# BallisticLA/RandLAPACK

Hardware: AMD Instinct MI355X
Metric: GFLOP/s (sketch+factor) for RSVD rank-256 on m x n dense fp64 (higher is better)
Workload: dtype f64; 1 GPU; RSVD 200000x20000 fp64 rank 256, one QB block, p=0, CholQRQ (BASELINE configs[1]); m=200000, n=20000, k=256, parallelism=row-block x1, collectives=none, ranks_seen=1, comm_kind=none, qb_return=3, k_out=256

## Files before the change

### include/RandLAPACK_amd/rl_blaspp.hh

```
#pragma once
#include <cstdint>
#include <cmath>
#include <stdexcept>
#include <string>
#include <vector>
#include "../rlhip.h"

namespace blas {

enum class Layout : char { ColMajor = 'C', RowMajor = 'R' };
enum class Op : char { NoTrans = 'N', Trans = 'T', ConjTrans = 'C' };
enum class Side : char { Left = 'L', Right = 'R' };
enum class Diag : char { NonUnit = 'N', Unit = 'U' };
enum class Uplo : char { Upper = 'U', Lower = 'L', General = 'G' };

inline char to_char(Op v) { return (char)v; }
inline char to_char(Side v) { return (char)v; }
inline char to_char(Diag v) { return (char)v; }
inline char to_char(Uplo v) { return (char)v; }
inline char to_char(Layout v) { return (char)v; }

class Error : public std::runtime_error {
public:
    explicit Error(std::string const& m) : std::runtime_error(m) {}
};

inline void check(int rc, const char* what) {
    if (rc < 0) throw Error(std::string(what) + " failed with code " + std::to_string(rc));
}

class Queue {
    rlhip_ctx* ctx_ = nullptr;
    bool owned_ = false;
public:
    explicit Queue(int device = 0) {
        check(rlhip_create(&ctx_, device, nullptr, 1), "rlhip_create");
        owned_ = true;
    }
    explicit Queue(rlhip_ctx* ctx) : ctx_(ctx), owned_(false) {}
    struct Side {};
    Queue(Queue& parent, Side) {
        check(rlhip_create_side(parent.ctx_, &ctx_), "rlhip_create_side");
        owned_ = true;
    }
    struct CachedSide {};
    Queue(Queue& parent, CachedSide) {
        check(rlhip_side_of(parent.ctx_, &ctx_), "rlhip_side_of");
        owned_ = false;
    }
    void wait_for(Queue& other) { check(rlhip_order_after(ctx_, other.ctx_), "rlhip_order_after"); }
    void set_qrcp_cols(int cols) { check(rlhip_set_qrcp_cols(ctx_, cols), "rlhip_set_qrcp_cols"); }
    Queue(Queue const&) = delete;
    Queue& operator=(Queue const&) = delete;
    ~Queue() { if (owned_ && ctx_) rlhip_destroy(ctx_); }
    void sync() { check(rlhip_sync(ctx_), "rlhip_sync"); }

    int world() const { return local_only ? 1 : rlhip_comm_size(ctx_); }
    int rank() const { return local_only ? 0 : rlhip_comm_rank(ctx_); }
    int local_only = 0;
    struct NormRequest { const void* ptr = nullptr; int64_t rows = 0, cols = 0, ld = 0; bool done = false; double value = 0; bool defer = false, pending = false; };
    NormRequest norm_req;
    double collect_norm(bool over_ranks) {
        if (norm_req.pending) { check(rlhip_norma_collect_f64(ctx_, over_ranks ? 1 : 0, &norm_req.value), "norma_collect"); norm_req.pending = false; }
        else if (over_ranks && world() > 1) { double ssq = norm_req.value * norm_req.value; allreduce_sum_host(&ssq, 1); norm_req.value = std::sqrt(ssq); }
        return norm_req.value;
    }
    bool rows_sharded = false;
    bool reduce_over_rows() const { return rows_sharded && world() > 1; }
    void allreduce_sum(double* buf, int64_t count) { check(rlhip_allreduce_sum_f64(ctx_, buf, count), "allreduce"); }
    void allreduce_sum(float* buf, int64_t count) { check(rlhip_allreduce_sum_f32(ctx_, buf, count), "allreduce"); }
    void allreduce_sum_host(double* x, int64_t n) { check(rlhip_allreduce_sum_host_f64(ctx_, x, n), "allreduce_host"); }
    void shard_extent(int64_t m_local, int64_t& m_global, int64_t& row0) {
        const int w = world(), r = rank();
        if (w <= 1) { m_global = m_local; row0 = 0; return; }
        std::vector<double> len((size_t)w, 0.0);
        len[(size_t)r] = (double)m_local;
        allreduce_sum_host(len.data(), w);
        m_global = 0; row0 = 0;
        for (int i = 0; i < w; ++i) { if (i < r) row0 += (int64_t)len[(size_t)i]; m_global += (int64_t)len[(size_t)i]; }
    }
    void* stream() const { return rlhip_stream(ctx_); }
    rlhip_ctx* ctx() const { return ctx_; }
};

inline Queue& default_queue() {
    static Queue q0(0);
    return q0;
}

template <typename T>
T* device_malloc(int64_t n, Queue& q = blas::default_queue()) {
    void* p = nullptr;
    check(rlhip_malloc(q.ctx(), &p, (size_t)(n > 0 ? n : 1) * sizeof(T)), "device_malloc");
    return (T*)p;
}
inline void device_free(void* p, Queue& q = blas::default_queue()) { check(rlhip_free(q.ctx(), p), "device_free"); }
template <typename T>
void device_memset(T* p, int byte, int64_t n, Queue& q = blas::default_queue()) { check(rlhip_memset(q.ctx(), p, byte, (size_t)n * sizeof(T)), "memset"); }
template <typename T>
void device_copy_vector(int64_t n, T const* src, T* dst, Queue& q = blas::default_queue()) {
    check(rlhip_memcpy_d2d(q.ctx(), dst, src, (size_t)n * sizeof(T)), "device_copy_vector");
}
template <typename T>
void copy_to_host(int64_t n, T const* dev, T* host, Queue& q = blas::default_queue()) { check(rlhip_memcpy_d2h(q.ctx(), host, dev, (size_t)n * sizeof(T)), "d2h"); }
template <typename T>
void copy_to_device(int64_t n, T const* host, T* dev, Queue& q = blas::default_queue()) { check(rlhip_memcpy_h2d(q.ctx(), dev, host, (size_t)n * sizeof(T)), "h2d"); }

template <typename T>
void copy(int64_t n, T const* x, int64_t incx, T* y, int64_t incy, Queue& q = default_queue()) {
    if (incx != 1 || incy != 1) throw Error("blas::copy: unit strides only");
    device_copy_vector(n, x, y, q);
}

class RowsSharded {
    Queue& q_;
    bool prev_;
public:
    RowsSharded(Queue& q, bool on) : q_(q), prev_(q.rows_sharded) { q.rows_sharded = on; }
    ~RowsSharded() { q_.rows_sharded = prev_; }
};

class LocalOnly {
    Queue& q_;
public:
    explicit LocalOnly(Queue& q) : q_(q) { ++q.local_only; }
    ~LocalOnly() { --q_.local_only; }
};

class Range {
public:
    explicit Range(const char* name) { rlhip_range_push(name); }
    ~Range() { rlhip_range_pop(); }
    Range(Range const&) = delete;
    Range& operator=(Range const&) = delete;
};

class Phases {
    bool open_ = false;
public:
    void operator()(const char* name) { end(); rlhip_range_push(name); open_ = true; }
    void end() { if (open_) { rlhip_range_pop(); open_ = false; } }
    ~Phases() { end(); }
};

class GiveWay {
    Queue& q_;
    int prev_;
public:
    explicit GiveWay(Queue& q) : q_(q), prev_(rlhip_avoid_persistent(q.ctx(), 1)) {}
    ~GiveWay() { rlhip_avoid_persistent(q_.ctx(), prev_ > 0 ? 1 : 0); }
};

class Scratch {
    Queue& q_;
    size_t mark_;
public:
    explicit Scratch(Queue& q) : q_(q), mark_(rlhip_scratch_mark(q.ctx())) {}
    ~Scratch() { rlhip_scratch_release(q_.ctx(), mark_); }
    template <typename T>
    T* alloc(int64_t n) {
        void* p = nullptr;
        check(rlhip_scratch_alloc(q_.ctx(), &p, (size_t)(n > 0 ? n : 1) * sizeof(T)), "scratch_alloc");
        return (T*)p;
    }
    template <typename T>
    T* try_alloc(int64_t n) {
        void* p = nullptr;
        if (rlhip_scratch_alloc(q_.ctx(), &p, (size_t)(n > 0 ? n : 1) * sizeof(T)) < 0) return nullptr;
        return (T*)p;
    }
};

inline void gemm(Layout, Op ta, Op tb, int64_t m, int64_t n, int64_t k, double alpha, double const* A, int64_t lda,
                 double const* B, int64_t ldb, double beta, double* C, int64_t ldc, Queue& q = blas::default_queue()) {
    auto& nr = q.norm_req;
    if (nr.ptr == (const void*)A && !nr.done && nr.ld == lda &&
        ((ta == Op::NoTrans && nr.rows == m && nr.cols == k) || (ta != Op::NoTrans && nr.rows == k && nr.cols == m))) {
        double nrm = 0;
        check(rlhip_gemm_norma_f64(q.ctx(), (char)ta, (char)tb, m, n, k, alpha, A, lda, B, ldb, beta, C, ldc, nr.defer ? nullptr : &nrm,
                                   nullptr), "gemm_norma");
        nr.done = true;
        nr.pending = nr.defer;
        nr.value = nrm;
        return;
    }
    check(rlhip_gemm_f64(q.ctx(), (char)ta, (char)tb, m, n, k, alpha, A, lda, B, ldb, beta, C, ldc), "gemm");
}
inline void gemm(Layout, Op ta, Op tb, int64_t m, int64_t n, int64_t k, float alpha, float const* A, int64_t lda,
                 float const* B, int64_t ldb, float beta, float* C, int64_t ldc, Queue& q = blas::default_queue()) {
    check(rlhip_gemm_f32(q.ctx(), (char)ta, (char)tb, m, n, k, alpha, A, lda, B, ldb, beta, C, ldc), "gemm");
}
inline void syrk(Layout, Uplo u, Op t, int64_t n, int64_t k, double alpha, double const* A, int64_t lda, double beta,
                 double* C, int64_t ldc, Queue& q = blas::default_queue()) {
    check(rlhip_syrk_f64(q.ctx(), (char)u, (char)t, n, k, alpha, A, lda, beta, C, ldc), "syrk");
}
inline void syrk(Layout, Uplo u, Op t, int64_t n, int64_t k, float alpha, float const* A, int64_t lda, float beta,
                 float* C, int64_t ldc, Queue& q = blas::default_queue()) {
    check(rlhip_syrk_f32(q.ctx(), (char)u, (char)t, n, k, alpha, A, lda, beta, C, ldc), "syrk");
}
inline void trsm(Layout, Side s, Uplo u, Op t, Diag d, int64_t m, int64_t n, double alpha, double const* A, int64_t lda,
                 double* B, int64_t ldb, Queue& q = blas::default_queue()) {
    check(rlhip_trsm_f64(q.ctx(), (char)s, (char)u, (char)t, (char)d, m, n, alpha, A, lda, B, ldb), "trsm");
}
inline void trsm(Layout, Side s, Uplo u, Op t, Diag d, int64_t m, int64_t n, float alpha, float const* A, int64_t lda,
                 float* B, int64_t ldb, Queue& q = blas::default_queue()) {
    check(rlhip_trsm_f32(q.ctx(), (char)s, (char)u, (char)t, (char)d, m, n, alpha, A, lda, B, ldb), "trsm");
}
inline void trsm_gather(Diag d, int64_t m, int64_t n, double alpha, double const* A, int64_t lda, double const* Bsrc, int64_t ldsrc,
                        int64_t const* jpvt, double* B, int64_t ldb, Queue& q = blas::default_queue()) {
    check(rlhip_trsm_gather_f64(q.ctx(), (char)d, m, n, alpha, A, lda, Bsrc, ldsrc, jpvt, B, ldb), "trsm_gather");
}
inline void trsm_gather(Diag d, int64_t m, int64_t n, float alpha, float const* A, int64_t lda, float const* Bsrc, int64_t ldsrc,
                        int64_t const* jpvt, float* B, int64_t ldb, Queue& q = blas::default_queue()) {
    check(rlhip_trsm_gather_f32(q.ctx(), (char)d, m, n, alpha, A, lda, Bsrc, ldsrc, jpvt, B, ldb), "trsm_gather");
}
inline bool trsm_gather_range(Diag d, int64_t m, int64_t nsrc, double alpha, double const* A, int64_t lda, double const* Bsrc, int64_t ldsrc,
                              int64_t const* jpvt, double* B, int64_t ldb, int64_t col0, int64_t col1, Queue& q = blas::default_queue()) {
    const int rc = rlhip_trsm_gather_range_f64(q.ctx(), (char)d, m, nsrc, alpha, A, lda, Bsrc, ldsrc, jpvt, B, ldb, col0, col1);
    if (rc == 1) return false;
    check(rc, "trsm_gather_range");
    return true;
}
inline bool trsm_gather_range(Diag d, int64_t m, int64_t nsrc, float alpha, float const* A, int64_t lda, float const* Bsrc, int64_t ldsrc,
                              int64_t const* jpvt, float* B, int64_t ldb, int64_t col0, int64_t col1, Queue& q = blas::default_queue()) {
    const int rc = rlhip_trsm_gather_range_f32(q.ctx(), (char)d, m, nsrc, alpha, A, lda, Bsrc, ldsrc, jpvt, B, ldb, col0, col1);
    if (rc == 1) return false;
    check(rc, "trsm_gather_range");
    return true;
}
inline void trmm(Layout, Side s, Uplo u, Op t, Diag d, int64_t m, int64_t n, double alpha, double const* A, int64_t lda,
                 double* B, int64_t ldb, Queue& q = blas::default_queue()) {
    check(rlhip_trmm_f64(q.ctx(), (char)s, (char)u, (char)t, (char)d, m, n, alpha, A, lda, B, ldb), "trmm");
}
inline void trmm(Layout, Side s, Uplo u, Op t, Diag d, int64_t m, int64_t n, float alpha, float const* A, int64_t lda,
                 float* B, int64_t ldb, Queue& q = blas::default_queue()) {
    check(rlhip_trmm_f32(q.ctx(), (char)s, (char)u, (char)t, (char)d, m, n, alpha, A, lda, B, ldb), "trmm");
}

}

namespace RandLAPACK {
using blas::Layout;
using blas::Op;
using blas::Side;
using blas::Diag;
using blas::Uplo;
}
```

### include/RandLAPACK_amd/rl_lapackpp.hh

```
#pragma once
#include <cmath>
#include "rl_blaspp.hh"

namespace lapack {

using blas::Queue;
enum class Job : char { NoVec = 'N', Vec = 'V', SomeVec = 'S', AllVec = 'A' };
enum class Norm : char { One = '1', Inf = 'I', Fro = 'F', Max = 'M' };
enum class MatrixType : char { General = 'G', Lower = 'L', Upper = 'U' };
inline char to_char(Job v) { return (char)v; }
inline char to_char(Norm v) { return (char)v; }
inline char to_char(MatrixType v) { return (char)v; }

inline int64_t potrf(blas::Uplo u, int64_t n, double* A, int64_t lda, Queue& q = blas::default_queue()) {
    int rc = rlhip_potrf_f64(q.ctx(), (char)u, n, A, lda); blas::check(rc, "potrf"); return rc;
}
inline int64_t potrf(blas::Uplo u, int64_t n, float* A, int64_t lda, Queue& q = blas::default_queue()) {
    int rc = rlhip_potrf_f32(q.ctx(), (char)u, n, A, lda); blas::check(rc, "potrf"); return rc;
}
inline int cholqrq(int64_t m, int64_t k, double* A, int64_t lda, double* R, bool reduce_gram, int& info, Queue& q = blas::default_queue()) {
    const int rc = rlhip_cholqrq_f64(q.ctx(), m, k, A, lda, R, reduce_gram ? 1 : 0, &info);
    blas::check(rc, "cholqrq");
    return rc;
}
inline int cholqrq(int64_t m, int64_t k, float* A, int64_t lda, float* R, bool reduce_gram, int& info, Queue& q = blas::default_queue()) {
    const int rc = rlhip_cholqrq_f32(q.ctx(), m, k, A, lda, R, reduce_gram ? 1 : 0, &info);
    blas::check(rc, "cholqrq");
    return rc;
}
inline double lange(Norm nt, int64_t m, int64_t n, double const* A, int64_t lda, Queue& q = blas::default_queue()) {
    if (nt != Norm::Fro) throw blas::Error("lange: only Norm::Fro is on the path");
    double r = 0; blas::check(rlhip_lange_fro_f64(q.ctx(), m, n, A, lda, &r), "lange"); return r;
}
inline float lange(Norm nt, int64_t m, int64_t n, float const* A, int64_t lda, Queue& q = blas::default_queue()) {
    if (nt != Norm::Fro) throw blas::Error("lange: only Norm::Fro is on the path");
    float r = 0; blas::check(rlhip_lange_fro_f32(q.ctx(), m, n, A, lda, &r), "lange"); return r;
}
inline void lacpy(MatrixType t, int64_t m, int64_t n, double const* A, int64_t lda, double* B, int64_t ldb, Queue& q = blas::default_queue()) {
    blas::check(rlhip_lacpy_f64(q.ctx(), (char)t, m, n, A, lda, B, ldb), "lacpy");
}
inline void lacpy(MatrixType t, int64_t m, int64_t n, float const* A, int64_t lda, float* B, int64_t ldb, Queue& q = blas::default_queue()) {
    blas::check(rlhip_lacpy_f32(q.ctx(), (char)t, m, n, A, lda, B, ldb), "lacpy");
}
inline void laset(MatrixType t, int64_t m, int64_t n, double offd, double diag, double* A, int64_t lda, Queue& q = blas::default_queue()) {
    blas::check(rlhip_laset_f64(q.ctx(), (char)t, m, n, offd, diag, A, lda), "laset");
}
inline void laset(MatrixType t, int64_t m, int64_t n, float offd, float diag, float* A, int64_t lda, Queue& q = blas::default_queue()) {
    blas::check(rlhip_laset_f32(q.ctx(), (char)t, m, n, offd, diag, A, lda), "laset");
}
inline void add_diag(int64_t n, double alpha, double* A, int64_t lda, Queue& q = blas::default_queue()) {
    blas::check(rlhip_add_diag_f64(q.ctx(), n, alpha, A, lda), "add_diag");
}
inline void add_diag(int64_t n, float alpha, float* A, int64_t lda, Queue& q = blas::default_queue()) {
    blas::check(rlhip_add_diag_f32(q.ctx(), n, alpha, A, lda), "add_diag");
}
inline int64_t geqp3(int64_t m, int64_t n, double* A, int64_t lda, int64_t* jpvt, double* tau, Queue& q = blas::default_queue()) {
    int rc = rlhip_geqp3_f64(q.ctx(), m, n, A, lda, jpvt, tau); blas::check(rc, "geqp3"); return rc;
}
inline int64_t geqp3(int64_t m, int64_t n, float* A, int64_t lda, int64_t* jpvt, float* tau, Queue& q = blas::default_queue()) {
    int rc = rlhip_geqp3_f32(q.ctx(), m, n, A, lda, jpvt, tau); blas::check(rc, "geqp3"); return rc;
}
inline void get_diag(int64_t n, double const* A, int64_t lda, double* diag_host, Queue& q = blas::default_queue()) {
    blas::check(rlhip_get_diag_f64(q.ctx(), n, A, lda, diag_host), "get_diag");
}
inline void get_diag(int64_t n, float const* A, int64_t lda, float* diag_host, Queue& q = blas::default_queue()) {
    blas::check(rlhip_get_diag_f32(q.ctx(), n, A, lda, diag_host), "get_diag");
}
inline bool any_abs_gt(int64_t n, double const* x, double thr, Queue& q = blas::default_queue()) { int a = 0; blas::check(rlhip_any_abs_gt_f64(q.ctx(), n, x, thr, &a), "any_abs_gt"); return a != 0; }
inline bool any_abs_gt(int64_t n, float const* x, float thr, Queue& q = blas::default_queue()) { int a = 0; blas::check(rlhip_any_abs_gt_f32(q.ctx(), n, x, thr, &a), "any_abs_gt"); return a != 0; }
inline void orhr_col(int64_t m, int64_t n, int64_t nb, double* A, int64_t lda, double* T, int64_t ldt, double* D, Queue& q = blas::default_queue()) { blas::check(rlhip_orhr_col_f64(q.ctx(), m, n, nb, A, lda, T, ldt, D), "orhr_col"); }
inline void orhr_col(int64_t m, int64_t n, int64_t nb, float* A, int64_t lda, float* T, int64_t ldt, float* D, Queue& q = blas::default_queue()) { blas::check(rlhip_orhr_col_f32(q.ctx(), m, n, nb, A, lda, T, ldt, D), "orhr_col"); }
inline void gemqrt(blas::Side s, blas::Op t, int64_t m, int64_t n, int64_t k, int64_t nb, double const* V, int64_t ldv, double const* T, int64_t ldt, double* C, int64_t ldc, Queue& q = blas::default_queue()) { blas::check(rlhip_gemqrt_f64(q.ctx(), (char)s, (char)t, m, n, k, nb, V, ldv, T, ldt, C, ldc), "gemqrt"); }
inline void gemqrt(blas::Side s, blas::Op t, int64_t m, int64_t n, int64_t k, int64_t nb, float const* V, int64_t ldv, float const* T, int64_t ldt, float* C, int64_t ldc, Queue& q = blas::default_queue()) { blas::check(rlhip_gemqrt_f32(q.ctx(), (char)s, (char)t, m, n, k, nb, V, ldv, T, ldt, C, ldc), "gemqrt"); }
inline void gemqrt_head(int64_t m, int64_t n, int64_t k, double const* V, int64_t ldv, double const* T, int64_t ldt, double* C, int64_t ldc, double* W2, Queue& q = blas::default_queue()) { blas::check(rlhip_gemqrt_head_f64(q.ctx(), m, n, k, V, ldv, T, ldt, C, ldc, W2), "gemqrt_head"); }
inline void gemqrt_head(int64_t m, int64_t n, int64_t k, float const* V, int64_t ldv, float const* T, int64_t ldt, float* C, int64_t ldc, float* W2, Queue& q = blas::default_queue()) { blas::check(rlhip_gemqrt_head_f32(q.ctx(), m, n, k, V, ldv, T, ldt, C, ldc, W2), "gemqrt_head"); }
inline void gemqrt_tail(int64_t m, int64_t n, int64_t k, double const* V, int64_t ldv, double const* W2, double* C, int64_t ldc, Queue& q = blas::default_queue()) { blas::check(rlhip_gemqrt_tail_f64(q.ctx(), m, n, k, V, ldv, W2, C, ldc), "gemqrt_tail"); }
inline void gemqrt_tail(int64_t m, int64_t n, int64_t k, float const* V, int64_t ldv, float const* W2, float* C, int64_t ldc, Queue& q = blas::default_queue()) { blas::check(rlhip_gemqrt_tail_f32(q.ctx(), m, n, k, V, ldv, W2, C, ldc), "gemqrt_tail"); }
inline void larft(int64_t m, int64_t k, double const* V, int64_t ldv, double const* tau, double* T, int64_t ldt, Queue& q = blas::default_queue()) { blas::check(rlhip_larft_f64(q.ctx(), m, k, V, ldv, tau, T, ldt), "larft"); }
inline void larft(int64_t m, int64_t k, float const* V, int64_t ldv, float const* tau, float* T, int64_t ldt, Queue& q = blas::default_queue()) { blas::check(rlhip_larft_f32(q.ctx(), m, k, V, ldv, tau, T, ldt), "larft"); }
inline void row_sign(int64_t n, double* R, int64_t ldr, double const* D, Queue& q = blas::default_queue()) { blas::check(rlhip_row_sign_f64(q.ctx(), n, R, ldr, D), "row_sign"); }
inline void row_sign(int64_t n, float* R, int64_t ldr, float const* D, Queue& q = blas::default_queue()) { blas::check(rlhip_row_sign_f32(q.ctx(), n, R, ldr, D), "row_sign"); }
inline void tau_from_t(int64_t k, int64_t nb, double const* T, int64_t ldt, double* tau, Queue& q = blas::default_queue()) { blas::check(rlhip_tau_from_t_f64(q.ctx(), k, nb, T, ldt, tau), "tau_from_t"); }
inline void tau_from_t(int64_t k, int64_t nb, float const* T, int64_t ldt, float* tau, Queue& q = blas::default_queue()) { blas::check(rlhip_tau_from_t_f32(q.ctx(), k, nb, T, ldt, tau), "tau_from_t"); }
inline int64_t geqrf(int64_t m, int64_t n, double* A, int64_t lda, double* tau, Queue& q = blas::default_queue()) { int rc = rlhip_geqrf_f64(q.ctx(), m, n, A, lda, tau); blas::check(rc, "geqrf"); return rc; }
inline int64_t geqrf(int64_t m, int64_t n, float* A, int64_t lda, float* tau, Queue& q = blas::default_queue()) { int rc = rlhip_geqrf_f32(q.ctx(), m, n, A, lda, tau); blas::check(rc, "geqrf"); return rc; }
inline bool geqrf_q(int64_t m, int64_t n, double* A, int64_t lda, double* R, int64_t ldr, Queue& q = blas::default_queue()) { int rc = rlhip_geqrf_q_f64(q.ctx(), m, n, A, lda, R, ldr); blas::check(rc, "geqrf_q"); return rc == 0; }
inline bool geqrf_q(int64_t m, int64_t n, float* A, int64_t lda, float* R, int64_t ldr, Queue& q = blas::default_queue()) { int rc = rlhip_geqrf_q_f32(q.ctx(), m, n, A, lda, R, ldr); blas::check(rc, "geqrf_q"); return rc == 0; }
inline void ungqr(int64_t m, int64_t n, int64_t k, double* A, int64_t lda, double const* tau, Queue& q = blas::default_queue()) { blas::check(rlhip_ungqr_f64(q.ctx(), m, n, k, A, lda, tau), "ungqr"); }
inline void ungqr(int64_t m, int64_t n, int64_t k, float* A, int64_t lda, float const* tau, Queue& q = blas::default_queue()) { blas::check(rlhip_ungqr_f32(q.ctx(), m, n, k, A, lda, tau), "ungqr"); }
inline int64_t getrf(int64_t m, int64_t n, double* A, int64_t lda, int64_t* ipiv, Queue& q = blas::default_queue()) { int rc = rlhip_getrf_f64(q.ctx(), m, n, A, lda, ipiv); blas::check(rc, "getrf"); return rc; }
inline int64_t getrf(int64_t m, int64_t n, float* A, int64_t lda, int64_t* ipiv, Queue& q = blas::default_queue()) { int rc = rlhip_getrf_f32(q.ctx(), m, n, A, lda, ipiv); blas::check(rc, "getrf"); return rc; }
inline int64_t getrf_pivots(int64_t m, int64_t n, double* A, int64_t lda, int64_t* ipiv, Queue& q = blas::default_queue()) { int rc = rlhip_getrf_piv_f64(q.ctx(), m, n, A, lda, ipiv); blas::check(rc, "getrf_piv"); return rc; }
inline int64_t getrf_pivots(int64_t m, int64_t n, float* A, int64_t lda, int64_t* ipiv, Queue& q = blas::default_queue()) { int rc = rlhip_getrf_piv_f32(q.ctx(), m, n, A, lda, ipiv); blas::check(rc, "getrf_piv"); return rc; }
inline void laswp(int64_t n, double* A, int64_t lda, int64_t k1, int64_t k2, int64_t const* ipiv, int64_t incx, Queue& q = blas::default_queue()) {
    if (incx != 1) throw blas::Error("laswp: only incx = 1 is on the path");
    blas::check(rlhip_laswp_f64(q.ctx(), n, A, lda, k1, k2, ipiv), "laswp");
}
inline void laswp(int64_t n, float* A, int64_t lda, int64_t k1, int64_t k2, int64_t const* ipiv, int64_t incx, Queue& q = blas::default_queue()) {
    if (incx != 1) throw blas::Error("laswp: only incx = 1 is on the path");
    blas::check(rlhip_laswp_f32(q.ctx(), n, A, lda, k1, k2, ipiv), "laswp");
}
template <typename T>
inline void geqrt(int64_t m, int64_t n, int64_t nb, T* A, int64_t lda, T* Tm, int64_t ldt, T* tau_scratch, Queue& q = blas::default_queue()) {
    geqrf(m, n, A, lda, tau_scratch, q);
    for (int64_t i = 0; i < n; i += nb) {
        const int64_t ib = std::min(nb, n - i);
        larft(m - i, ib, A + i + i * lda, lda, tau_scratch + i, Tm + i * ldt, ldt, q);
    }
}
template <typename T>
inline void ormqr(blas::Side s, blas::Op t, int64_t m, int64_t n, int64_t k, T const* V, int64_t ldv, T const* tau, T* C, int64_t ldc, T* T_scratch, Queue& q = blas::default_queue()) {
    if (k == 0 || n == 0) return;
    larft(m, k, V, ldv, tau, T_scratch, k, q);
    gemqrt(s, t, m, n, k, k, V, ldv, T_scratch, k, C, ldc, q);
}
template <typename T>
inline T lansy(Norm nt, blas::Uplo u, int64_t n, T const* A, int64_t lda, Queue& q = blas::default_queue()) {
    if (nt != Norm::Fro) throw blas::Error("lansy: only Norm::Fro is on the path");
    if (n <= 0) return (T)0;
    blas::Scratch ws(q);
    T* W = ws.alloc<T>(n * n);
    laset(MatrixType::General, n, n, (T)0, (T)0, W, n, q);
    lacpy(u == blas::Uplo::Upper ? MatrixType::Upper : MatrixType::Lower, n, n, A, lda, W, n, q);
    const T tri = lange(Norm::Fro, n, n, W, n, q);
    std::vector<T> dg((size_t)n);
    get_diag(n, A, lda, dg.data(), q);
    double dd = 0;
    for (T v : dg) dd += (double)v * (double)v;
    const double s2 = 2.0 * (double)tri * (double)tri - dd;
    return (T)std::sqrt(s2 > 0 ? s2 : 0.0);
}
inline void qrp_partial(int64_t m, int64_t n, int64_t steps, double* A, int64_t lda, int64_t* jpvt, double* tau, Queue& q = blas::default_queue()) { blas::check(rlhip_qrp_partial_f64(q.ctx(), m, n, steps, A, lda, jpvt, tau), "qrp_partial"); }
inline void qrp_partial(int64_t m, int64_t n, int64_t steps, float* A, int64_t lda, int64_t* jpvt, float* tau, Queue& q = blas::default_queue()) { blas::check(rlhip_qrp_partial_f32(q.ctx(), m, n, steps, A, lda, jpvt, tau), "qrp_partial"); }
inline void geqp3_steps(int64_t m, int64_t n, int64_t steps, double* A, int64_t lda, int64_t* jpvt, double* tau, Queue& q = blas::default_queue()) { blas::check(rlhip_geqp3_steps_f64(q.ctx(), m, n, steps, A, lda, jpvt, tau), "geqp3_steps"); }
inline void geqp3_steps(int64_t m, int64_t n, int64_t steps, float* A, int64_t lda, int64_t* jpvt, float* tau, Queue& q = blas::default_queue()) { blas::check(rlhip_geqp3_steps_f32(q.ctx(), m, n, steps, A, lda, jpvt, tau), "geqp3_steps"); }
inline void vrows_explicit(int64_t br, int64_t toff, int64_t tcnt, double const* Vtop, int64_t ldv, double* out, int64_t ldo, Queue& q = blas::default_queue()) { blas::check(rlhip_vrows_explicit_f64(q.ctx(), br, toff, tcnt, Vtop, ldv, out, ldo), "vrows_explicit"); }
inline void vrows_explicit(int64_t br, int64_t toff, int64_t tcnt, float const* Vtop, int64_t ldv, float* out, int64_t ldo, Queue& q = blas::default_queue()) { blas::check(rlhip_vrows_explicit_f32(q.ctx(), br, toff, tcnt, Vtop, ldv, out, ldo), "vrows_explicit"); }
inline void luqrcp_piv(int64_t sd, int64_t cols, int64_t const* ipiv, int64_t* J, Queue& q = blas::default_queue()) { blas::check(rlhip_luqrcp_piv(q.ctx(), sd, cols, ipiv, J), "luqrcp_piv"); }
inline int64_t gesdd(Job job, int64_t m, int64_t n, double* A, int64_t lda, double* S, double* U, int64_t ldu,
                     double* VT, int64_t ldvt, Queue& q = blas::default_queue()) {
    if (job != Job::SomeVec) throw blas::Error("gesdd: only Job::SomeVec is on the path");
    int rc = rlhip_gesdd_f64(q.ctx(), m, n, A, lda, S, U, ldu, VT, ldvt, nullptr); blas::check(rc, "gesdd"); return rc;
}
inline int64_t gesdd(Job job, int64_t m, int64_t n, float* A, int64_t lda, float* S, float* U, int64_t ldu,
                     float* VT, int64_t ldvt, Queue& q = blas::default_queue()) {
    if (job != Job::SomeVec) throw blas::Error("gesdd: only Job::SomeVec is on the path");
    int rc = rlhip_gesdd_f32(q.ctx(), m, n, A, lda, S, U, ldu, VT, ldvt, nullptr); blas::check(rc, "gesdd"); return rc;
}
inline int64_t gesvdj(int64_t m, int64_t n, double* A, int64_t lda, double* S, double* VT, int64_t ldvt, Queue& q = blas::default_queue()) {
    int rc = rlhip_gesvdj_f64(q.ctx(), m, n, A, lda, S, VT, ldvt, nullptr); blas::check(rc, "gesvdj"); return rc;
}
inline int64_t gesvdj(int64_t m, int64_t n, float* A, int64_t lda, float* S, float* VT, int64_t ldvt, Queue& q = blas::default_queue()) {
    int rc = rlhip_gesvdj_f32(q.ctx(), m, n, A, lda, S, VT, ldvt, nullptr); blas::check(rc, "gesvdj"); return rc;
}

}

namespace RandLAPACK {
using lapack::Job;
using lapack::MatrixType;
using lapack::Norm;
}
```

### include/RandLAPACK_amd/rl_qb.hh

```
#pragma once
#include <algorithm>
#include <cmath>
#include <limits>
#include "rl_rf.hh"

namespace RandLAPACK {

template <typename T, typename RNG>
class QBalg {
public:
    virtual ~QBalg() {}
    virtual int call(int64_t m, int64_t n, T* A, int64_t& k, int64_t b_sz, T tol, T*& Q, T*& BT,
                     RandBLAS::RNGState<RNG>& state) = 0;
};

template <typename T, typename RNG>
class QB : public QBalg<T, RNG> {
public:
    QB(RangeFinder<T, RNG>& rf_obj, Stabilization<T>& orth_obj, bool verb, bool orth) : QB(blas::default_queue(), rf_obj, orth_obj, verb, orth) {}
    QB(blas::Queue& queue, RangeFinder<T, RNG>& rf_obj, Stabilization<T>& orth_obj, bool verb, bool orth)
        : q(queue), rf(rf_obj), orth(orth_obj) {
        verbose = verb;
        orth_check = orth;
    }

    int call(int64_t m, int64_t n, T* A, int64_t& k, int64_t b_sz, T tol, T*& Q, T*& BT,
             RandBLAS::RNGState<RNG>& state) override {
        int64_t curr_sz = 0, next_sz = 0;
        tol = std::max(tol, 100 * std::numeric_limits<T>::epsilon());
        T norm_B = 0, prev_err = 0, approx_err = 0;
        if (Q) blas::device_free(Q, q);
        if (BT) blas::device_free(BT, q);
        const int64_t k_in = k;
        Q = blas::device_malloc<T>(m * k_in, q);
        BT = blas::device_malloc<T>(n * k_in, q);
        blas::Scratch ws(q);
        T* QtQi = ws.alloc<T>(k_in * std::max<int64_t>(1, std::min(b_sz, k_in)));
        const bool single_block = (b_sz >= k_in);
        T* A_cpy = A;
        T* A_own = nullptr;
        T norm_A = 0;
        bool have_norm = false;
        if (!single_block) {
            A_own = blas::device_malloc<T>(m * n, q);
            lapack::lacpy(MatrixType::General, m, n, A, m, A_own, m, q);
            A_cpy = A_own;
        }
        if constexpr (sizeof(T) == 8) {
            q.norm_req = blas::Queue::NormRequest();
            q.norm_req.ptr = A_cpy; q.norm_req.rows = m; q.norm_req.cols = n; q.norm_req.ld = m;
            q.norm_req.defer = true;
        }
        blas::RowsSharded sh(q, true);
        auto done = [&](int code) {
            q.norm_req = blas::Queue::NormRequest();
            if (A_own) blas::device_free(A_own, q);
            const int64_t kept = std::max<int64_t>(std::min(k, k_in), 0);
            if (kept < k_in) {
                blas::device_memset(Q + m * kept, 0, m * (k_in - kept), q);
                blas::device_memset(BT + n * kept, 0, n * (k_in - kept), q);
            }
            return code;
        };

        while (curr_sz < k) {
            b_sz = std::min(b_sz, k - curr_sz);
            next_sz = curr_sz + b_sz;
            T* Q_i = Q + m * curr_sz;
            T* BT_i = BT + n * curr_sz;
            if (rf.call(m, n, A_cpy, b_sz, Q_i, state)) { k = curr_sz; q.norm_req = blas::Queue::NormRequest(); return done(6); }
            const bool norm_rides = !have_norm && q.norm_req.done;
            if (!have_norm && !norm_rides) norm_A = lapack::lange(Norm::Fro, m, n, A_cpy, m, q);
            if (orth_check && util::orthogonality_check(m, b_sz, Q_i, verbose, q)) { k = curr_sz; return done(4); }
            if (curr_sz != 0) {
                blas::gemm(Layout::ColMajor, Op::Trans, Op::NoTrans, curr_sz, b_sz, m, T(1), Q, m, Q_i, m, T(0), QtQi, next_sz, q);
                if (q.world() > 1) q.allreduce_sum(QtQi, next_sz * b_sz);
                blas::gemm(Layout::ColMajor, Op::NoTrans, Op::NoTrans, m, b_sz, curr_sz, T(-1), Q, m, QtQi, next_sz, T(1), Q_i, m, q);
                orth.call(m, b_sz, Q_i);
            }
            blas::gemm(Layout::ColMajor, Op::Trans, Op::NoTrans, n, b_sz, m, T(1), A_cpy, m, Q_i, m, T(0), BT_i, n, q);
            if (q.world() > 1) q.allreduce_sum(BT_i, n * b_sz);
            T norm_B_i = lapack::lange(Norm::Fro, n, b_sz, BT_i, n, q);
            if (!have_norm) {
                if (norm_rides) norm_A = (T)q.collect_norm(true);
                else if (q.world() > 1) {
                    double ssq = (double)norm_A * (double)norm_A;
                    q.allreduce_sum_host(&ssq, 1);
                    norm_A = (T)std::sqrt(ssq);
                }
                q.norm_req = blas::Queue::NormRequest();
                have_norm = true;
            }
            norm_B = std::hypot(norm_B, norm_B_i);
            prev_err = approx_err;
            approx_err = std::sqrt(std::abs(norm_A - norm_B)) * (std::sqrt(norm_A + norm_B) / norm_A);
            if ((curr_sz > 0) && (approx_err > prev_err)) { k = curr_sz; return done(2); }
            if (orth_check && util::orthogonality_check(m, next_sz, Q, verbose, q)) { k = curr_sz; return done(5); }
            curr_sz += b_sz;
            if (approx_err < tol) { k = curr_sz; return done(0); }
            if (curr_sz < k)
                blas::gemm(Layout::ColMajor, Op::NoTrans, Op::Trans, m, n, b_sz, T(-1), Q_i, m, BT_i, n, T(1), A_cpy, m, q);
        }
        return done(3);
    }

    blas::Queue& q;
    RangeFinder<T, RNG>& rf;
    Stabilization<T>& orth;
    bool verbose;
    bool orth_check;
};

}
```

### include/RandLAPACK_amd/rl_rsvd.hh

```
#pragma once
#include "rl_exceptions.hh"
#include "rl_qb.hh"

namespace RandLAPACK {

template <typename T, typename RNG>
class RSVDalg {
public:
    virtual ~RSVDalg() {}
    virtual int call(int64_t m, int64_t n, T* A, int64_t& k, T tol, T*& U, T*& S, T*& V,
                     RandBLAS::RNGState<RNG>& state) = 0;
};

template <typename T, typename RNG>
class RSVD : public RSVDalg<T, RNG> {
public:
    RSVD(QBalg<T, RNG>& qb_obj, int64_t b_sz) : RSVD(blas::default_queue(), qb_obj, b_sz) {}
    RSVD(blas::Queue& queue, QBalg<T, RNG>& qb_obj, int64_t b_sz) : q(queue), QB_Obj(qb_obj) { block_sz = b_sz; }

    int call(int64_t m, int64_t n, T* A, int64_t& k, T tol, T*& U, T*& S, T*& V,
             RandBLAS::RNGState<RNG>& state) override {
        randlapack_require(m >= 0) << "m=" << m << " must be >= 0";
        randlapack_require(n >= 0) << "n=" << n << " must be >= 0";
        randlapack_require(k > 0) << "target rank k=" << k << " must be > 0";
        randlapack_require(tol >= (T)0) << "tol=" << tol << " must be >= 0";
        randlapack_require(!(A == nullptr && m > 0 && n > 0))
            << "A buffer is null but m=" << m << " and n=" << n << " imply a nonempty matrix";

        T* Q = nullptr;
        T* BT = nullptr;
        qb_return = QB_Obj.call(m, n, A, k, block_sz, tol, Q, BT, state);

        const int64_t kk = std::max<int64_t>(k, 1);
        U = blas::device_malloc<T>(m * kk, q);
        S = blas::device_malloc<T>(kk, q);
        V = blas::device_malloc<T>(n * kk, q);
        if (k > 0) {
            blas::Scratch ws(q);
            T* UT_buf = ws.alloc<T>(k * k);
            svd_info = lapack::gesdd(Job::SomeVec, n, k, BT, n, S, V, n, UT_buf, k, q);
            blas::gemm(Layout::ColMajor, Op::NoTrans, Op::Trans, m, k, k, T(1), Q, m, UT_buf, k, T(0), U, m, q);
        }
        blas::device_free(Q, q);
        blas::device_free(BT, q);
        return 0;
    }

    blas::Queue& q;
    QBalg<T, RNG>& QB_Obj;
    int64_t block_sz;
    int qb_return = 0;
    int64_t svd_info = 0;
};

}
```

### include/rlhip.h

```cpp
#ifndef RLHIP_H
#define RLHIP_H
#include <stddef.h>
#include <stdint.h>

#ifdef __cplusplus
extern "C" {
#endif

typedef struct rlhip_ctx rlhip_ctx;

int rlhip_create(rlhip_ctx** ctx, int device, void* hip_stream, int own_stream);
int rlhip_create_side(rlhip_ctx* parent, rlhip_ctx** out);
int rlhip_order_after(rlhip_ctx* waiter, rlhip_ctx* signaler);
int rlhip_destroy(rlhip_ctx* ctx);
enum rlhip_option {
    RLHIP_OPT_CHOLQRQ_ONE_STREAM = 0,
    RLHIP_OPT_GESDD_GRAM = 1,
    RLHIP_OPT_JACOBI_PERSIST = 2,
    RLHIP_OPT_TRSM_XASM = 3,
    RLHIP_OPT_SASO_MODE = 4,
    RLHIP_OPT_HQRRP_TALL_PANEL = 5,
    RLHIP_OPT_DRV_BQRRP_LOOKAHEAD_MIN_ELEMS = 6,
    RLHIP_OPT_DRV_BQRRP_CHOLQR_FALLBACK = 7,
    RLHIP_OPT_DRV_CQRRPT_FOLD_PIVOTING = 8,
    RLHIP_OPT_DRV_CQRRPT_SPLIT_QRCP = 9,
    RLHIP_OPT_DRV_SPARSE_SKETCH_DENSIFY = 10,
    RLHIP_OPT_JACOBI_CLOCK_HOLDERS = 11,
    RLHIP_OPT_LSQ_NORMAL_FUSED = 12,
    RLHIP_OPT_SPMV_LANES = 13,
    RLHIP_OPT_RBF_FUSED = 14,
    RLHIP_OPT_COUNT = 15
};
int rlhip_set_option(rlhip_ctx* ctx, int option, int64_t value);
int64_t rlhip_get_option(rlhip_ctx* ctx, int option);
int rlhip_sync(rlhip_ctx* ctx);
void* rlhip_stream(rlhip_ctx* ctx);
int rlhip_malloc(rlhip_ctx* ctx, void** dev_ptr, size_t bytes);
int rlhip_free(rlhip_ctx* ctx, void* dev_ptr);
int rlhip_trim(rlhip_ctx* ctx);
int rlhip_malloc_host(rlhip_ctx* ctx, void** host_ptr, size_t bytes);
int rlhip_free_host(rlhip_ctx* ctx, void* host_ptr);
int rlhip_memcpy_h2d(rlhip_ctx* ctx, void* dst_dev, const void* src_host, size_t bytes);
int rlhip_memcpy_d2h(rlhip_ctx* ctx, void* dst_host, const void* src_dev, size_t bytes);
int rlhip_memcpy_d2d(rlhip_ctx* ctx, void* dst_dev, const void* src_dev, size_t bytes);
int rlhip_memset(rlhip_ctx* ctx, void* dst_dev, int byte, size_t bytes);
int rlhip_reserve_workspace(rlhip_ctx* ctx, size_t bytes);
size_t rlhip_workspace_highwater(rlhip_ctx* ctx);
const char* rlhip_version(void);

size_t rlhip_scratch_mark(rlhip_ctx* ctx);
int rlhip_scratch_alloc(rlhip_ctx* ctx, void** dev_ptr, size_t bytes);
int rlhip_scratch_release(rlhip_ctx* ctx, size_t mark);

int rlhip_timer_start(rlhip_ctx* ctx);
int rlhip_timer_stop_ms(rlhip_ctx* ctx, float* ms_host);

int rlhip_philox4x32_10(rlhip_ctx* ctx, int64_t nblocks, uint32_t* out_dev, const uint32_t ctr_host[4],
                        const uint32_t key_host[2]);
int rlhip_fill_dense_f64(rlhip_ctx* ctx, int dist, int64_t rows, int64_t cols, double* buf,
                         const uint32_t ctr_host[4], const uint32_t key_host[2], uint32_t next_ctr_host[4]);
int rlhip_fill_dense_f32(rlhip_ctx* ctx, int dist, int64_t rows, int64_t cols, float* buf,
                         const uint32_t ctr_host[4], const uint32_t key_host[2], uint32_t next_ctr_host[4]);
int rlhip_fill_dense_rows_f64(rlhip_ctx* ctx, int dist, int64_t glob_rows, int64_t cols, int64_t row0, int64_t loc_rows,
                              double* buf, int64_t ld, const uint32_t ctr[4], const uint32_t key[2], uint32_t next_ctr[4]);
int rlhip_fill_dense_rows_f32(rlhip_ctx* ctx, int dist, int64_t glob_rows, int64_t cols, int64_t row0, int64_t loc_rows,
                              float* buf, int64_t ld, const uint32_t ctr[4], const uint32_t key[2], uint32_t next_ctr[4]);

int rlhip_gemm_f64(rlhip_ctx* ctx, char transa, char transb, int64_t m, int64_t n, int64_t k, double alpha,
                   const double* A, int64_t lda, const double* B, int64_t ldb, double beta, double* C,
                   int64_t ldc);
int rlhip_gemm_f32(rlhip_ctx* ctx, char transa, char transb, int64_t m, int64_t n, int64_t k, float alpha,
                   const float* A, int64_t lda, const float* B, int64_t ldb, float beta, float* C,
                   int64_t ldc);
int rlhip_gemm_norma_f64(rlhip_ctx* ctx, char transa, char transb, int64_t m, int64_t n, int64_t k, double alpha,
                         const double* A, int64_t lda, const double* B, int64_t ldb, double beta, double* C,
                         int64_t ldc, double* norm_a_host, int* fused_host);
int rlhip_norma_collect_f64(rlhip_ctx* ctx, int over_ranks, double* norm_a_host);
int rlhip_syrk_f64(rlhip_ctx* ctx, char uplo, char trans, int64_t n, int64_t k, double alpha, const double* A,
                   int64_t lda, double beta, double* C, int64_t ldc);
int rlhip_syrk_f32(rlhip_ctx* ctx, char uplo, char trans, int64_t n, int64_t k, float alpha, const float* A,
                   int64_t lda, float beta, float* C, int64_t ldc);
int rlhip_trsm_f64(rlhip_ctx* ctx, char side, char uplo, char trans, char diag, int64_t m, int64_t n,
                   double alpha, const double* A, int64_t lda, double* B, int64_t ldb);
int rlhip_trsm_f32(rlhip_ctx* ctx, char side, char uplo, char trans, char diag, int64_t m, int64_t n,
                   float alpha, const float* A, int64_t lda, float* B, int64_t ldb);
int rlhip_trsm_gather_f64(rlhip_ctx* ctx, char diag, int64_t m, int64_t n, double alpha, const double* A, int64_t lda,
                          const double* Bsrc, int64_t ldsrc, const int64_t* jpvt_dev, double* B, int64_t ldb);
int rlhip_trsm_gather_f32(rlhip_ctx* ctx, char diag, int64_t m, int64_t n, float alpha, const float* A, int64_t lda,
                          const float* Bsrc, int64_t ldsrc, const int64_t* jpvt_dev, float* B, int64_t ldb);
int rlhip_trsm_gather_range_f64(rlhip_ctx* ctx, char diag, int64_t m, int64_t nsrc, double alpha, const double* A, int64_t lda,
                                const double* Bsrc, int64_t ldsrc, const int64_t* jpvt, double* B, int64_t ldb, int64_t col0, int64_t col1);
int rlhip_trsm_gather_range_f32(rlhip_ctx* ctx, char diag, int64_t m, int64_t nsrc, float alpha, const float* A, int64_t lda,
                                const float* Bsrc, int64_t ldsrc, const int64_t* jpvt, float* B, int64_t ldb, int64_t col0, int64_t col1);
int rlhip_trmm_f64(rlhip_ctx* ctx, char side, char uplo, char trans, char diag, int64_t m, int64_t n,
                   double alpha, const double* A, int64_t lda, double* B, int64_t ldb);
int rlhip_trmm_f32(rlhip_ctx* ctx, char side, char uplo, char trans, char diag, int64_t m, int64_t n,
                   float alpha, const float* A, int64_t lda, float* B, int64_t ldb);

int rlhip_potrf_f64(rlhip_ctx* ctx, char uplo, int64_t n, double* A, int64_t lda);
int rlhip_potrf_f32(rlhip_ctx* ctx, char uplo, int64_t n, float* A, int64_t lda);
int rlhip_cholqrq_f64(rlhip_ctx* ctx, int64_t m, int64_t k, double* A, int64_t lda, double* R, int reduce_gram, int* info_host);
int rlhip_cholqrq_f32(rlhip_ctx* ctx, int64_t m, int64_t k, float* A, int64_t lda, float* R, int reduce_gram, int* info_host);
int rlhip_lange_fro_f64(rlhip_ctx* ctx, int64_t m, int64_t n, const double* A, int64_t lda, double* result_host);
int rlhip_lange_fro_f32(rlhip_ctx* ctx, int64_t m, int64_t n, const float* A, int64_t lda, float* result_host);
int rlhip_lacpy_f64(rlhip_ctx* ctx, char uplo, int64_t m, int64_t n, const double* A, int64_t lda, double* B,
                    int64_t ldb);
int rlhip_lacpy_f32(rlhip_ctx* ctx, char uplo, int64_t m, int64_t n, const float* A, int64_t lda, float* B,
                    int64_t ldb);
int rlhip_laset_f64(rlhip_ctx* ctx, char uplo, int64_t m, int64_t n, double offdiag, double diag, double* A,
                    int64_t lda);
int rlhip_laset_f32(rlhip_ctx* ctx, char uplo, int64_t m, int64_t n, float offdiag, float diag, float* A,
                    int64_t lda);
int rlhip_gesvdj_f64(rlhip_ctx* ctx, int64_t m, int64_t n, double* A, int64_t lda, double* S, double* VT,
                     int64_t ldvt, int* sweeps_host);
int rlhip_gesvdj_f32(rlhip_ctx* ctx, int64_t m, int64_t n, float* A, int64_t lda, float* S, float* VT,
                     int64_t ldvt, int* sweeps_host);

int rlhip_add_diag_f64(rlhip_ctx* ctx, int64_t n, double alpha, double* A, int64_t lda);
int rlhip_add_diag_f32(rlhip_ctx* ctx, int64_t n, float alpha, float* A, int64_t lda);
int rlhip_gesdd_f64(rlhip_ctx* ctx, int64_t m, int64_t n, double* A, int64_t lda, double* S, double* U, int64_t ldu,
                    double* VT, int64_t ldvt, int* sweeps_host);
int rlhip_gesdd_f32(rlhip_ctx* ctx, int64_t m, int64_t n, float* A, int64_t lda, float* S, float* U, int64_t ldu,
                    float* VT, int64_t ldvt, int* sweeps_host);
int rlhip_transpose_f64(rlhip_ctx* ctx, int64_t m, int64_t n, const double* A, int64_t lda, double* AT,
                        int64_t ldat, int upper_only);
int rlhip_transpose_f32(rlhip_ctx* ctx, int64_t m, int64_t n, const float* A, int64_t lda, float* AT, int64_t ldat,
                        int upper_only);

typedef struct rlhip_saso rlhip_saso;
int rlhip_saso_create(rlhip_ctx* ctx, int64_t d, int64_t m, int nnz, const uint32_t ctr_host[4],
                      const uint32_t key_host[2], uint32_t next_ctr_host[4], rlhip_saso** S);
int rlhip_saso_create_mode(rlhip_ctx* ctx, int64_t d, int64_t m, int nnz, int mode, const uint32_t ctr_host[4],
                           const uint32_t key_host[2], uint32_t next_ctr_host[4], rlhip_saso** S);
int rlhip_saso_destroy(rlhip_ctx* ctx, rlhip_saso* S);
int rlhip_saso_apply_f64(rlhip_ctx* ctx, const rlhip_saso* S, int64_t n, double alpha, const double* A, int64_t lda,
                         double beta, double* B, int64_t ldb);
int rlhip_saso_apply_f32(rlhip_ctx* ctx, const rlhip_saso* S, int64_t n, float alpha, const float* A, int64_t lda,
                         float beta, float* B, int64_t ldb);
int rlhip_saso_apply_rows_f64(rlhip_ctx* ctx, const rlhip_saso* S, int64_t n, double alpha, const double* A_loc, int64_t lda,
                              int64_t row0, int64_t mloc, double beta, double* B, int64_t ldb);
int rlhip_saso_apply_rows_f32(rlhip_ctx* ctx, const rlhip_saso* S, int64_t n, float alpha, const float* A_loc, int64_t lda,
                              int64_t row0, int64_t mloc, float beta, float* B, int64_t ldb);
int rlhip_saso_apply_csr_f64(rlhip_ctx* ctx, const rlhip_saso* S, int64_t n, double alpha, const int64_t* rowptrT, const int64_t* colidxT,
                             const double* valsT, double beta, double* B, int64_t ldb, int64_t row0);
int rlhip_saso_apply_csr_f32(rlhip_ctx* ctx, const rlhip_saso* S, int64_t n, float alpha, const int64_t* rowptrT, const int64_t* colidxT,
                             const float* valsT, float beta, float* B, int64_t ldb, int64_t row0);
int rlhip_saso_apply_csr_ordered_f64(rlhip_ctx* ctx, const rlhip_saso* S, int64_t n, double alpha, const int64_t* rowptrT, const int64_t* colidxT,
                                     const double* valsT, double beta, double* B, int64_t ldb);
int rlhip_saso_apply_csr_ordered_f32(rlhip_ctx* ctx, const rlhip_saso* S, int64_t n, float alpha, const int64_t* rowptrT, const int64_t* colidxT,
                                     const float* valsT, float beta, float* B, int64_t ldb);
int rlhip_saso_dense_f64(rlhip_ctx* ctx, const rlhip_saso* S, double* dense_d_by_m);
int rlhip_saso_dense_f32(rlhip_ctx* ctx, const rlhip_saso* S, float* dense_d_by_m);
int rlhip_col_swap_f64(rlhip_ctx* ctx, int64_t m, int64_t n, int64_t k, double* A, int64_t lda, const int64_t* idx);
int rlhip_col_swap_f32(rlhip_ctx* ctx, int64_t m, int64_t n, int64_t k, float* A, int64_t lda, const int64_t* idx);
int rlhip_col_swap_i64(rlhip_ctx* ctx, int64_t n, int64_t k, int64_t* A, const int64_t* idx);
int rlhip_geqp3_f64(rlhip_ctx* ctx, int64_t m, int64_t n, double* A, int64_t lda, int64_t* jpvt, double* tau);
int rlhip_geqp3_f32(rlhip_ctx* ctx, int64_t m, int64_t n, float* A, int64_t lda, int64_t* jpvt, float* tau);
int rlhip_get_diag_f64(rlhip_ctx* ctx, int64_t n, const double* A, int64_t lda, double* diag_host);
int rlhip_get_diag_f32(rlhip_ctx* ctx, int64_t n, const float* A, int64_t lda, float* diag_host);

int rlhip_getrf_f64(rlhip_ctx* ctx, int64_t m, int64_t n, double* A, int64_t lda, int64_t* ipiv);
int rlhip_getrf_piv_f64(rlhip_ctx* ctx, int64_t m, int64_t n, double* A, int64_t lda, int64_t* ipiv);
int rlhip_getrf_piv_f32(rlhip_ctx* ctx, int64_t m, int64_t n, float* A, int64_t lda, int64_t* ipiv);
int rlhip_getrf_f32(rlhip_ctx* ctx, int64_t m, int64_t n, float* A, int64_t lda, int64_t* ipiv);
int rlhip_geqrf_q_f64(rlhip_ctx* ctx, int64_t m, int64_t n, double* A, int64_t lda, double* R, int64_t ldr);
int rlhip_geqrf_q_f32(rlhip_ctx* ctx, int64_t m, int64_t n, float* A, int64_t lda, float* R, int64_t ldr);
int rlhip_geqrf_f64(rlhip_ctx* ctx, int64_t m, int64_t n, double* A, int64_t lda, double* tau);
int rlhip_geqrf_f32(rlhip_ctx* ctx, int64_t m, int64_t n, float* A, int64_t lda, float* tau);
int rlhip_ungqr_f64(rlhip_ctx* ctx, int64_t m, int64_t n, int64_t k, double* A, int64_t lda, const double* tau);
int rlhip_ungqr_f32(rlhip_ctx* ctx, int64_t m, int64_t n, int64_t k, float* A, int64_t lda, const float* tau);
int rlhip_laswp_f64(rlhip_ctx* ctx, int64_t n, double* A, int64_t lda, int64_t k1, int64_t k2, const int64_t* ipiv);
int rlhip_laswp_f32(rlhip_ctx* ctx, int64_t n, float* A, int64_t lda, int64_t k1, int64_t k2, const int64_t* ipiv);
int rlhip_luqrcp_piv(rlhip_ctx* ctx, int64_t sd, int64_t cols, const int64_t* ipiv, int64_t* J);

int rlhip_orhr_col_f64(rlhip_ctx* ctx, int64_t m, int64_t n, int64_t nb, double* A, int64_t lda, double* T, int64_t ldt,
                       double* D);
int rlhip_orhr_col_f32(rlhip_ctx* ctx, int64_t m, int64_t n, int64_t nb, float* A, int64_t lda, float* T, int64_t ldt,
                       float* D);
int rlhip_gemqrt_f64(rlhip_ctx* ctx, char side, char trans, int64_t m, int64_t n, int64_t k, int64_t nb, const double* V,
                     int64_t ldv, const double* T, int64_t ldt, double* C, int64_t ldc);
int rlhip_gemqrt_f32(rlhip_ctx* ctx, char side, char trans, int64_t m, int64_t n, int64_t k, int64_t nb, const float* V,
                     int64_t ldv, const float* T, int64_t ldt, float* C, int64_t ldc);
int rlhip_gemqrt_head_f64(rlhip_ctx* ctx, int64_t m, int64_t n, int64_t k, const double* V, int64_t ldv, const double* T, int64_t ldt, double* C, int64_t ldc, double* W2);
int rlhip_gemqrt_head_f32(rlhip_ctx* ctx, int64_t m, int64_t n, int64_t k, const float* V, int64_t ldv, const float* T, int64_t ldt, float* C, int64_t ldc, float* W2);
int rlhip_gemqrt_tail_f64(rlhip_ctx* ctx, int64_t m, int64_t n, int64_t k, const double* V, int64_t ldv, const double* W2, double* C, int64_t ldc);
int rlhip_gemqrt_tail_f32(rlhip_ctx* ctx, int64_t m, int64_t n, int64_t k, const float* V, int64_t ldv, const float* W2, float* C, int64_t ldc);
int rlhip_qrp_partial_f64(rlhip_ctx* ctx, int64_t m, int64_t n, int64_t steps, double* A, int64_t lda, int64_t* jpvt, double* tau);
int rlhip_qrp_partial_f32(rlhip_ctx* ctx, int64_t m, int64_t n, int64_t steps, float* A, int64_t lda, int64_t* jpvt, float* tau);
int rlhip_geqp3_steps_f64(rlhip_ctx* ctx, int64_t m, int64_t n, int64_t steps, double* A, int64_t lda, int64_t* jpvt, double* tau);
int rlhip_geqp3_steps_f32(rlhip_ctx* ctx, int64_t m, int64_t n, int64_t steps, float* A, int64_t lda, int64_t* jpvt, float* tau);
int rlhip_side_of(rlhip_ctx* parent, rlhip_ctx** out);
int rlhip_set_qrcp_cols(rlhip_ctx* ctx, int cols);
int rlhip_vrows_explicit_f64(rlhip_ctx* ctx, int64_t br, int64_t toff, int64_t tcnt, const double* Vtop, int64_t ldv, double* out, int64_t ldo);
int rlhip_vrows_explicit_f32(rlhip_ctx* ctx, int64_t br, int64_t toff, int64_t tcnt, const float* Vtop, int64_t ldv, float* out, int64_t ldo);
int rlhip_larft_f64(rlhip_ctx* ctx, int64_t m, int64_t k, const double* V, int64_t ldv, const double* tau, double* T, int64_t ldt);
int rlhip_larft_f32(rlhip_ctx* ctx, int64_t m, int64_t k, const float* V, int64_t ldv, const float* tau, float* T, int64_t ldt);
int rlhip_row_sign_f64(rlhip_ctx* ctx, int64_t n, double* R, int64_t ldr, const double* D);
int rlhip_row_sign_f32(rlhip_ctx* ctx, int64_t n, float* R, int64_t ldr, const float* D);
int rlhip_tau_from_t_f64(rlhip_ctx* ctx, int64_t k, int64_t nb, const double* T, int64_t ldt, double* tau);
int rlhip_tau_from_t_f32(rlhip_ctx* ctx, int64_t k, int64_t nb, const float* T, int64_t ldt, float* tau);
int rlhip_any_abs_gt_f64(rlhip_ctx* ctx, int64_t n, const double* x, double thr, int* any_host);
int rlhip_any_abs_gt_f32(rlhip_ctx* ctx, int64_t n, const float* x, float thr, int* any_host);

int rlhip_scal_cols_f64(rlhip_ctx* ctx, int64_t m, int64_t n, double* A, int64_t lda, const double* s_dev);
int rlhip_scal_cols_f32(rlhip_ctx* ctx, int64_t m, int64_t n, float* A, int64_t lda, const float* s_dev);
int rlhip_scal_rows_idx_f64(rlhip_ctx* ctx, int64_t cnt, const int64_t* idx_dev, int64_t n, double* A, int64_t lda, double alpha);
int rlhip_scal_rows_idx_f32(rlhip_ctx* ctx, int64_t cnt, const int64_t* idx_dev, int64_t n, float* A, int64_t lda, float alpha);
int rlhip_gen_kahan_f64(rlhip_ctx* ctx, int64_t m, int64_t n, double* A, int64_t lda, double theta, double perturb);
int rlhip_gen_kahan_f32(rlhip_ctx* ctx, int64_t m, int64_t n, float* A, int64_t lda, float theta, float perturb);

int rlhip_symmetrize_f64(rlhip_ctx* ctx, char uplo, int64_t n, const double* A, int64_t lda, double* F, int64_t ldf);
int rlhip_symmetrize_f32(rlhip_ctx* ctx, char uplo, int64_t n, const float* A, int64_t lda, float* F, int64_t ldf);
int rlhip_axpby_f64(rlhip_ctx* ctx, int64_t n, double alpha, const double* x, double beta, double* y);
int rlhip_axpby_f32(rlhip_ctx* ctx, int64_t n, float alpha, const float* x, float beta, float* y);

int rlhip_csr_spmm_f64(rlhip_ctx* ctx, char layout, int64_t m, int64_t n, int64_t k, double alpha, const int64_t* rowptr,
                       const int64_t* colidx, const double* vals, const double* B, int64_t ldb, double beta, double* C, int64_t ldc);
int rlhip_csr_spmm_f32(rlhip_ctx* ctx, char layout, int64_t m, int64_t n, int64_t k, float alpha, const int64_t* rowptr,
                       const int64_t* colidx, const float* vals, const float* B, int64_t ldb, float beta, float* C, int64_t ldc);
int rlhip_csr_transpose_f64(rlhip_ctx* ctx, int64_t m, int64_t k, const int64_t* rowptr, const int64_t* colidx, const double* vals,
                            int64_t* rowptrT, int64_t* colidxT, double* valsT);
int rlhip_csr_transpose_f32(rlhip_ctx* ctx, int64_t m, int64_t k, const int64_t* rowptr, const int64_t* colidx, const float* vals,
                            int64_t* rowptrT, int64_t* colidxT, float* valsT);
int rlhip_csr_densify_cols_f64(rlhip_ctx* ctx, int64_t m, const int64_t* rowptrT, const int64_t* colidxT, const double* valsT,
                               int64_t c0, int64_t b, double* out, int64_t ldo);
int rlhip_csr_densify_cols_f32(rlhip_ctx* ctx, int64_t m, const int64_t* rowptrT, const int64_t* colidxT, const float* valsT,
                               int64_t c0, int64_t b, float* out, int64_t ldo);

int rlhip_sqexp_columns_f64(rlhip_ctx* ctx, int64_t rows_x, int64_t n, const double* X, int64_t ldx, int64_t nidx, const int64_t* idx_dev,
                            double bandwidth, double reg, double* out, int64_t ldo);
int rlhip_sqexp_columns_f32(rlhip_ctx* ctx, int64_t rows_x, int64_t n, const float* X, int64_t ldx, int64_t nidx, const int64_t* idx_dev,
                            float bandwidth, float reg, float* out, int64_t ldo);
int rlhip_sq_colnorms_f64(rlhip_ctx* ctx, int64_t rows_x, int64_t cols_x, const double* X, int64_t ldx, double* sq_colnorms_x);
int rlhip_sq_colnorms_f32(rlhip_ctx* ctx, int64_t rows_x, int64_t cols_x, const float* X, int64_t ldx, float* sq_colnorms_x);
int rlhip_sqexp_submatrix_f64(rlhip_ctx* ctx, int64_t rows_x, int64_t cols_x, const double* X, int64_t ldx, const double* sq_colnorms_x,
                              int64_t rows_ksub, int64_t cols_ksub, double* Ksub, int64_t ldk, int64_t ro_ksub, int64_t co_ksub, double bandwidth);
int rlhip_sqexp_submatrix_f32(rlhip_ctx* ctx, int64_t rows_x, int64_t cols_x, const float* X, int64_t ldx, const float* sq_colnorms_x,
                              int64_t rows_ksub, int64_t cols_ksub, float* Ksub, int64_t ldk, int64_t ro_ksub, int64_t co_ksub, float bandwidth);
int rlhip_rbf_apply_f64(rlhip_ctx* ctx, int64_t rows_x, int64_t dim, const double* X, int64_t ldx, double bandwidth, const double* regs_host,
                        int64_t num_ops, int eval_includes_reg, int64_t n, double alpha, const double* B, int64_t ldb, double beta, double* C,
                        int64_t ldc);
int rlhip_rbf_apply_f32(rlhip_ctx* ctx, int64_t rows_x, int64_t dim, const float* X, int64_t ldx, float bandwidth, const float* regs_host,
                        int64_t num_ops, int eval_includes_reg, int64_t n, float alpha, const float* B, int64_t ldb, float beta, float* C,
                        int64_t ldc);
#define RLHIP_PDK_SQEXP 0
#define RLHIP_PDK_MATERN32 1
#define RLHIP_PDK_MATERN52 2
int rlhip_pdk_columns_f64(rlhip_ctx* ctx, int64_t rows_x, int64_t n, const double* X, int64_t ldx, int64_t nidx, const int64_t* idx_dev, int kernel,
                          double bandwidth, double reg, double* out, int64_t ldo);
int rlhip_pdk_columns_f32(rlhip_ctx* ctx, int64_t rows_x, int64_t n, const float* X, int64_t ldx, int64_t nidx, const int64_t* idx_dev, int kernel,
                          float bandwidth, float reg, float* out, int64_t ldo);
int rlhip_pdk_submatrix_f64(rlhip_ctx* ctx, int64_t rows_x, int64_t cols_x, const double* X, int64_t ldx, const double* sq_colnorms_x,
                            int64_t rows_ksub, int64_t cols_ksub, double* Ksub, int64_t ldk, int64_t ro_ksub, int64_t co_ksub, int kernel,
                            double bandwidth);
int rlhip_pdk_submatrix_f32(rlhip_ctx* ctx, int64_t rows_x, int64_t cols_x, const float* X, int64_t ldx, const float* sq_colnorms_x,
// ... 167 lines not shown
```

### randlapack_amd/_lib.py

```python
from __future__ import annotations

import ctypes as C
import os
from pathlib import Path

_HERE = Path(__file__).resolve().parent
LIB_PATH = _HERE / "librlhip.so"

c_i64 = C.c_int64
c_int = C.c_int
c_char = C.c_char
c_dbl = C.c_double
c_flt = C.c_float
c_vp = C.c_void_p
c_sz = C.c_size_t
u32p = C.POINTER(C.c_uint32)


def _blas3(T):
    return {
        "gemm": [c_vp, c_char, c_char, c_i64, c_i64, c_i64, T, c_vp, c_i64, c_vp, c_i64, T, c_vp, c_i64],
        "syrk": [c_vp, c_char, c_char, c_i64, c_i64, T, c_vp, c_i64, T, c_vp, c_i64],
        "trsm": [c_vp, c_char, c_char, c_char, c_char, c_i64, c_i64, T, c_vp, c_i64, c_vp, c_i64],
        "trmm": [c_vp, c_char, c_char, c_char, c_char, c_i64, c_i64, T, c_vp, c_i64, c_vp, c_i64],
# ... 154 lines not shown
    "rlhip_drv_abrik_linop_timed_f64": (c_int, [c_vp, _ldp, c_i64, c_dbl, c_i64, dpp, dpp, dpp, u32p, C.POINTER(c_i64), C.POINTER(c_i64),
                                                C.POINTER(c_dbl), c_int, C.POINTER(C.c_long)]),
    "rlhip_linop_apply_f64": (c_int, [c_vp, _ldp, _ldp, c_char, c_char, c_i64, c_i64, c_i64, c_dbl, c_vp, c_i64, c_dbl, c_vp, c_i64]),
    "rlhip_linop_apply_view_f64": (c_int, [c_vp, _ldp, _ldp, c_int, C.POINTER(c_i64), c_char, c_char, c_i64, c_i64, c_i64, c_dbl, c_vp, c_i64, c_dbl, c_vp, c_i64]),
    "rlhip_regsym_apply_f64": (c_int, [c_vp, c_i64, c_vp, c_i64, C.POINTER(c_dbl), c_i64, c_int, c_i64, c_dbl, c_vp, c_i64, c_dbl, c_vp, c_i64]),
})
SIGNATURES["rlhip_drv_revd2_f64"] = (c_int, [c_vp, c_char, c_i64, c_vp, C.POINTER(c_i64), c_dbl, c_i64, c_i64, c_int, c_int, dpp, dpp, u32p,
                                               C.POINTER(c_dbl)])
SIGNATURES["rlhip_drv_syrf_f64"] = (c_int, [c_vp, c_char, c_i64, c_vp, c_i64, c_i64, c_i64, c_int, c_vp, u32p])
SIGNATURES["rlhip_drv_mat_gen_f64"] = (c_int, [c_vp, c_int, c_i64, c_i64, c_i64, c_dbl, c_dbl, c_dbl, c_int, c_dbl, c_dbl, c_dbl, c_int, c_vp, u32p,
                                                 C.POINTER(c_i64)])
for _name in ("stab", "rsvd", "cqrrpt", "hqrrp", "bqrrp", "qr_linops", "mat_gen"):
    _rt, _args = SIGNATURES[f"rlhip_drv_{_name}_f64"]
    SIGNATURES[f"rlhip_drv_{_name}_f32"] = (_rt, [c_flt if a is c_dbl else a for a in _args])
for _suf, _T in (("f64", c_dbl), ("f32", c_flt)):
    for _name, _args in _blas3(_T).items():
        SIGNATURES[f"rlhip_{_name}_{_suf}"] = (c_int, _args)

i64p = C.POINTER(c_i64)
intp = C.POINTER(c_int)
for _suf, _T in (("f64", c_dbl), ("f32", c_flt)):
    SIGNATURES.update({
        f"rlhip_sqexp_columns_{_suf}": (c_int, [c_vp, c_i64, c_i64, c_vp, c_i64, c_i64, c_vp, _T, _T, c_vp, c_i64]),
        f"rlhip_sq_colnorms_{_suf}": (c_int, [c_vp, c_i64, c_i64, c_vp, c_i64, c_vp]),
        f"rlhip_sqexp_submatrix_{_suf}": (c_int, [c_vp, c_i64, c_i64, c_vp, c_i64, c_vp, c_i64, c_i64, c_vp, c_i64, c_i64, c_i64, _T]),
        f"rlhip_rbf_apply_{_suf}": (c_int, [c_vp, c_i64, c_i64, c_vp, c_i64, _T, C.POINTER(_T), c_i64, c_int, c_i64, _T, c_vp, c_i64, _T, c_vp,
                                            c_i64]),
        f"rlhip_sample_indices_iid_{_suf}": (c_int, [c_vp, c_i64, c_vp, c_i64, c_int, u32p, u32p, u32p, c_vp, i64p, i64p, intp]),
        f"rlhip_rpchol_panel_finish_{_suf}": (c_int, [c_vp, c_i64, c_i64, c_vp, c_i64, c_vp, c_i64, c_vp, c_vp]),
        f"rlhip_gather_rows_{_suf}": (c_int, [c_vp, c_i64, c_vp, c_i64, c_vp, c_i64, c_vp, c_i64]),
        f"rlhip_gather_cols_{_suf}": (c_int, [c_vp, c_i64, c_i64, c_vp, c_vp, c_i64, c_vp, c_i64]),
        f"rlhip_drv_rpchol_rbf_{_suf}": (c_int, [c_vp, c_vp, c_i64, c_i64, c_i64, _T, _T, i64p, c_i64, i64p, c_vp, c_i64, u32p, intp]),
        f"rlhip_drv_rpchol_dense_{_suf}": (c_int, [c_vp, c_i64, c_vp, c_i64, i64p, c_i64, i64p, c_vp, c_i64, u32p, intp]),
        f"rlhip_drv_rpchol_pc_data_rbf_{_suf}": (c_int, [c_vp, c_vp, c_i64, c_i64, c_i64, _T, _T, i64p, c_i64, c_vp, c_vp, u32p]),
    })

f64p = C.POINTER(c_dbl)
SIGNATURES["rlhip_pcg_path_count"] = (c_i64, [c_vp, c_int])
for _suf, _T in (("f64", c_dbl), ("f32", c_flt)):
    _Tp = C.POINTER(_T)
    SIGNATURES.update({
        f"rlhip_posm_square_{_suf}": (c_int, [c_vp, c_i64, c_vp, c_vp, c_int, c_vp]),
        f"rlhip_pcg_update_xr_{_suf}": (c_int, [c_vp, c_i64, c_i64, c_vp, c_vp, c_i64, c_vp, c_i64, c_vp, c_i64, c_vp, c_i64, c_vp]),
        f"rlhip_pcg_update_p_{_suf}": (c_int, [c_vp, c_i64, c_i64, c_vp, c_vp, c_i64, c_vp, c_i64]),
        f"rlhip_pcg_colnorm2_{_suf}": (c_int, [c_vp, c_i64, c_i64, c_vp, c_i64, c_vp]),
        f"rlhip_spectral_precond_apply_{_suf}": (c_int, [c_vp, c_i64, c_i64, c_vp, c_i64, c_vp, c_i64, c_i64, _T, c_vp, c_i64, _T, c_vp, c_i64, c_vp,
                                                         c_vp]),
        f"rlhip_drv_pcg_dense_{_suf}": (c_int, [c_vp, c_i64, c_vp, c_i64, _Tp, c_i64, c_vp, c_i64, c_vp, c_i64, c_vp, c_vp, c_i64, _T, c_i64, i64p,
                                                _Tp]),
        f"rlhip_drv_pcg_rbf_{_suf}": (c_int, [c_vp, c_vp, c_i64, c_i64, c_i64, _T, _Tp, c_i64, c_vp, c_i64, c_vp, c_i64, c_vp, c_vp, c_i64, _T, c_i64,
                                              i64p, _Tp]),
        f"rlhip_drv_krill_full_rpchol_rbf_{_suf}": (c_int, [c_vp, c_vp, c_i64, c_i64, c_i64, _T, _Tp, c_i64, c_vp, c_vp, c_i64, _T, c_i64, i64p, c_i64,
                                                            u32p, i64p, _Tp]),
        f"rlhip_drv_posm_square_{_suf}": (c_int, [c_vp, c_i64, c_vp, c_vp, c_int, i64p]),
    })

SIGNATURES["rlhip_lsq_path_count"] = (c_i64, [c_vp, c_int])
for _suf, _T in (("f64", c_dbl), ("f32", c_flt)):
    SIGNATURES.update({
        f"rlhip_gemv_{_suf}": (c_int, [c_vp, c_char, c_i64, c_i64, _T, c_vp, c_i64, c_vp, _T, c_vp]),
        f"rlhip_normal_matvec_{_suf}": (c_int, [c_vp, c_i64, c_i64, c_vp, c_i64, c_vp, _T, c_vp, c_vp, c_vp, c_i64]),
        f"rlhip_pcg_saddle_step_xr_{_suf}": (c_int, [c_vp, c_i64, c_vp, c_vp, c_vp, c_vp, c_vp, c_vp]),
        f"rlhip_pcg_saddle_step_refresh_{_suf}": (c_int, [c_vp, c_i64, c_vp, c_vp, _T, c_vp, c_vp]),
        f"rlhip_pcg_saddle_step_d_{_suf}": (c_int, [c_vp, c_i64, c_vp, c_vp, c_vp, c_vp, c_vp]),
        f"rlhip_drv_pcg_saddle_{_suf}": (c_int, [c_vp, c_i64, c_i64, c_vp, c_i64, c_vp, c_vp, _T, c_i64, c_vp, _T, c_i64, c_vp, c_i64, c_vp, c_vp, c_vp,
                                                 i64p]),
        f"rlhip_drv_rpc_data_svd_saso_{_suf}": (c_int, [c_vp, c_i64, c_i64, c_i64, c_i64, c_vp, c_i64, c_vp, c_vp, u32p]),
        f"rlhip_drv_make_right_orthogonalizer_{_suf}": (c_int, [c_vp, c_i64, c_vp, c_vp, _T, c_i64, i64p]),
        f"rlhip_drv_sap_lstsq_{_suf}": (c_int, [c_vp, c_i64, c_i64, c_vp, c_i64, c_vp, c_vp, _T, _T, c_i64, _T, c_i64, c_vp, c_vp, c_vp, u32p, i64p,
                                                i64p]),
    })

SIGNATURES["rlhip_spmv_path_count"] = (c_i64, [c_vp, c_int])
for _suf, _T in (("f64", c_dbl), ("f32", c_flt)):
    SIGNATURES.update({
        f"rlhip_csr_spmv_{_suf}": (c_int, [c_vp, c_i64, c_i64, c_i64, c_vp, c_vp, c_vp, _T, c_vp, _T, c_vp]),
        f"rlhip_csr_normal_matvec_{_suf}": (c_int, [c_vp, c_i64, c_i64, c_i64, c_vp, c_vp, c_vp, c_vp, c_vp, c_vp, c_vp, _T, c_vp, c_vp, c_vp, c_i64]),
        f"rlhip_drv_pcg_saddle_linop_{_suf}": (c_int, [c_vp, _ldp, _ldp, c_vp, c_vp, _T, c_i64, c_vp, _T, c_i64, c_vp, c_i64, c_vp, c_vp, c_vp, i64p]),
        f"rlhip_drv_rpc_data_svd_saso_linop_{_suf}": (c_int, [c_vp, _ldp, _ldp, c_i64, c_i64, c_vp, c_vp, u32p]),
        f"rlhip_drv_sap_lstsq_linop_{_suf}": (c_int, [c_vp, _ldp, _ldp, c_vp, c_vp, _T, _T, c_i64, _T, c_i64, c_vp, c_vp, c_vp, u32p, i64p, i64p]),
    })

SIGNATURES["rlhip_rbf_path_count"] = (c_i64, [c_vp, c_int])
SIGNATURES["rlhip_rbf_split_chunks"] = (c_i64, [c_i64, c_i64])
SIGNATURES["rlhip_rbf_split_count"] = (c_i64, [c_vp])
for _suf, _T in (("f64", c_dbl), ("f32", c_flt)):
    SIGNATURES.update({
        f"rlhip_sqexp_cross_submatrix_{_suf}": (c_int, [c_vp, c_i64, c_i64, c_vp, c_i64, c_vp, c_i64, c_vp, c_i64, c_vp, c_i64, c_i64, c_vp, c_i64, c_i64,
                                                        c_i64, _T]),
        f"rlhip_rbf_cross_apply_{_suf}": (c_int, [c_vp, c_i64, c_i64, c_vp, c_i64, c_i64, c_vp, c_i64, _T, c_i64, _T, c_vp, c_i64, _T, c_vp, c_i64]),
        f"rlhip_drv_rbf_kernel_apply_{_suf}": (c_int, [c_vp, c_vp, c_i64, c_i64, c_i64, _T, C.POINTER(_T), c_i64, c_int, c_int, c_i64, _T, c_vp, c_i64, _T,
                                                       c_vp, c_i64]),
        f"rlhip_drv_krr_predict_{_suf}": (c_int, [c_vp, c_i64, c_i64, c_vp, c_i64, c_i64, c_vp, c_i64, _T, c_i64, c_vp, c_i64, c_vp, c_i64]),
    })

for _suf, _T in (("f64", c_dbl), ("f32", c_flt)):
    for _new, _old in (("rlhip_pdk_columns", "rlhip_sqexp_columns"), ("rlhip_pdk_submatrix", "rlhip_sqexp_submatrix"), ("rlhip_pdk_apply", "rlhip_rbf_apply"),
                       ("rlhip_pdk_cross_submatrix", "rlhip_sqexp_cross_submatrix"), ("rlhip_pdk_cross_apply", "rlhip_rbf_cross_apply"),
                       ("rlhip_drv_rpchol_pdk", "rlhip_drv_rpchol_rbf"), ("rlhip_drv_krill_full_rpchol_pdk", "rlhip_drv_krill_full_rpchol_rbf"),
                       ("rlhip_drv_krr_predict_pdk", "rlhip_drv_krr_predict"), ("rlhip_drv_pdk_kernel_apply", "rlhip_drv_rbf_kernel_apply")):
        _rt, _args = SIGNATURES[f"{_old}_{_suf}"]
        _at = _args.index(_T)
        SIGNATURES[f"{_new}_{_suf}"] = (_rt, _args[:_at] + [c_int] + _args[_at:])

for _suf, _T in (("f64", c_dbl), ("f32", c_flt)):
    _Tp = C.POINTER(_T)
    SIGNATURES.update({
        f"rlhip_ridge_filter_{_suf}": (c_int, [c_vp, c_i64, c_i64, c_vp, c_vp, c_i64, _T, c_vp, c_i64]),
        f"rlhip_drv_krill_restricted_rpchol_pdk_{_suf}": (c_int, [c_vp, c_vp, c_i64, c_i64, c_i64, c_int, _T, _Tp, c_i64, c_vp, c_i64, c_i64, i64p, c_i64,
                                                                  i64p, c_vp, c_i64, u32p, intp]),
        f"rlhip_drv_krill_restricted_pdk_{_suf}": (c_int, [c_vp, c_vp, c_i64, c_i64, c_i64, c_int, _T, _Tp, c_i64, c_vp, c_i64, c_i64, c_i64, i64p, c_vp,
                                                           c_i64, i64p]),
        f"rlhip_drv_krr_predict_restricted_pdk_{_suf}": (c_int, [c_vp, c_i64, c_i64, c_vp, c_i64, c_i64, c_vp, c_i64, c_int, _T, c_i64, i64p, c_i64, c_vp,
                                                                 c_i64, c_vp, c_i64]),
    })

for _suf, _T in (("f64", c_dbl), ("f32", c_flt)):
    _Tp, _dp = C.POINTER(_T), C.POINTER(c_dbl)
    SIGNATURES.update({
        f"rlhip_ridge_loo_{_suf}": (c_int, [c_vp, c_i64, c_i64, c_i64, c_i64, c_vp, c_i64, c_vp, c_vp, c_i64, c_vp, c_i64, c_vp, _T, c_vp, c_vp]),
        f"rlhip_drv_krill_restricted_rpchol_cv_pdk_{_suf}": (c_int, [c_vp, c_vp, c_i64, c_i64, c_i64, c_int, _T, _Tp, c_i64, c_int, c_vp, c_i64, c_i64, i64p,
                                                                     c_i64, i64p, c_vp, c_i64, u32p, intp, _dp, _dp, _dp, i64p, _dp]),
        f"rlhip_drv_krill_restricted_cv_pdk_{_suf}": (c_int, [c_vp, c_vp, c_i64, c_i64, c_i64, c_int, _T, _Tp, c_i64, c_int, c_vp, c_i64, c_i64, c_i64, i64p,
                                                              c_vp, c_i64, i64p, _dp, _dp, _dp, i64p, _dp]),
    })

SIGNATURES["rlhip_pdk_var_fused"] = (c_int, [c_i64, c_i64, c_i64])
SIGNATURES["rlhip_pdk_var_path_count"] = (c_i64, [c_vp, c_int])
SIGNATURES["rlhip_pdk_var_set_fused"] = (c_int, [c_vp, c_int])
for _suf, _T in (("f64", c_dbl), ("f32", c_flt)):
    _Tp = C.POINTER(_T)
    _fit, _given = (SIGNATURES[f"rlhip_drv_krill_restricted_{_n}pdk_{_suf}"] for _n in ("rpchol_", ""))
    SIGNATURES.update({
        f"rlhip_pdk_cross_var_{_suf}": (c_int, [c_vp, c_i64, c_i64, c_vp, c_i64, c_i64, c_vp, c_i64, c_int, _T, c_vp, c_i64, c_vp, c_i64, c_vp, c_i64, _T,
                                                c_vp, c_i64]),
        f"rlhip_drv_krill_restricted_rpchol_gp_pdk_{_suf}": (_fit[0], _fit[1] + [c_vp, c_i64, c_vp]),
        f"rlhip_drv_krill_restricted_gp_pdk_{_suf}": (_given[0], _given[1] + [c_vp, c_i64, c_vp]),
        f"rlhip_drv_krr_predict_restricted_var_pdk_{_suf}": (c_int, [c_vp, c_i64, c_i64, c_vp, c_i64, c_i64, c_vp, c_i64, c_int, _T, c_i64, i64p, c_vp,
                                                                     c_i64, c_vp, c_i64, _Tp, c_i64, c_vp, c_i64, c_int]),
    })

SIGNATURES["rlhip_pdk_grad_fused"] = (c_int, [c_i64, c_i64])
SIGNATURES["rlhip_pdk_grad_path_count"] = (c_i64, [c_vp, c_int])
SIGNATURES["rlhip_pdk_grad_set_fused"] = (c_int, [c_vp, c_int])
for _suf, _T in (("f64", c_dbl), ("f32", c_flt)):
    SIGNATURES.update({
        f"rlhip_pdk_cross_grad_{_suf}": (c_int, [c_vp, c_i64, c_i64, c_vp, c_i64, c_i64, c_vp, c_i64, c_int, _T, c_i64, _T, c_vp, c_i64, c_vp, c_i64]),
        f"rlhip_drv_krr_predict_grad_pdk_{_suf}": SIGNATURES[f"rlhip_drv_krr_predict_pdk_{_suf}"],
        f"rlhip_drv_krr_predict_restricted_grad_pdk_{_suf}": SIGNATURES[f"rlhip_drv_krr_predict_restricted_pdk_{_suf}"],
    })

SIGNATURES["rlhip_lu_path_count"] =(c_i64, [c_vp, c_int])
SIGNATURES["rlhip_tri_path_count"] = (c_i64, [c_vp, c_int])

_lib = None


def load():
    global _lib
    if _lib is not None:
        return _lib
    if not LIB_PATH.exists():
        raise RuntimeError(
            f"{LIB_PATH} is missing: build it with `python -c 'import __graft_entry__ as g; g.build()'` "
            "(hipcc --offload-arch=gfx950). randlapack_amd has no CPU fallback."
        )
    lib = C.CDLL(str(LIB_PATH), mode=os.RTLD_GLOBAL if hasattr(os, "RTLD_GLOBAL") else C.DEFAULT_MODE)
    for name, (res, args) in SIGNATURES.items():
        fn = getattr(lib, name)
        fn.restype = res
        fn.argtypes = args
    _lib = lib
    return lib


class RlhipError(RuntimeError):
    pass


def check(rc: int, what: str) -> int:
    if rc < 0:
        raise RlhipError(f"{what} failed with code {rc}")
    return rc


def lib_sha256() -> str:
    import hashlib

    h = hashlib.sha256()
    with open(LIB_PATH, "rb") as f:
        for chunk in iter(lambda: f.read(1 << 20), b""):
            h.update(chunk)
    return h.hexdigest()
```

### randlapack_amd/csrc/capi.hip

```cpp
#include "rlhip_internal.h"
#include <cstring>
#include <cstdlib>
#include <dlfcn.h>

static inline size_t align_up(size_t x, size_t a) { return (x + a - 1) / a * a; }

static size_t seg_vstart(const rlhip_ctx* c, int k) {
    size_t v = 0;
    for (int i = 0; i < k; ++i) v += c->segs[i].size;
    return v;
}

static int rlhip_poison() {
    static int v = -1;
    if (v < 0) { const char* e = getenv("RLHIP_POISON"); v = (e && e[0] == '1') ? 1 : 0; }
    return v;
}

void* rlhip_ws_alloc(rlhip_ctx* c, size_t bytes) {
    bytes = align_up(bytes ? bytes : 1, 256);
    for (;;) {
        if (c->cur_seg < c->nsegs && c->cur_used + bytes <= c->segs[c->cur_seg].size) {
            void* p = c->segs[c->cur_seg].base + c->cur_used;
            c->cur_used += bytes;
// ... 29 lines not shown
    void* p = nullptr;
    hipError_t e;
    if (kind == 1) e = hipExtMallocWithFlags(&p, bytes, hipDeviceMallocFinegrained);
    else if (kind == 2) e = hipExtMallocWithFlags(&p, bytes, hipDeviceMallocUncached);
    else e = hipMalloc(&p, bytes);
    if (e != hipSuccess && kind != 0) { (void)hipGetLastError(); e = hipMalloc(&p, bytes); }
    if (e != hipSuccess) { (void)hipGetLastError(); return nullptr; }
    c->xchg = p; c->xchg_bytes = bytes;
    return p;
}

void* rlhip_xloc_buffer(rlhip_ctx* c, size_t bytes) {
    if (bytes <= c->xloc_bytes) return c->xloc;
    if (c->xloc) { rlhip_stream_sync(c); hipFree(c->xloc); c->xloc = nullptr; c->xloc_bytes = 0; }
    bytes = (bytes + ((size_t)1 << 20) - 1) & ~(((size_t)1 << 20) - 1);
    void* p = nullptr;
    if (hipMalloc(&p, bytes) != hipSuccess) { (void)hipGetLastError(); return nullptr; }
    c->xloc = p; c->xloc_bytes = bytes;
    return p;
}

size_t rlhip_ws_mark(rlhip_ctx* c) { return c->nsegs ? seg_vstart(c, c->cur_seg) + c->cur_used : 0; }

void rlhip_ws_release(rlhip_ctx* c, size_t mark) {
    size_t v = 0;
    int k = 0;
    for (; k < c->nsegs; ++k) {
        if (mark <= v + c->segs[k].size) break;
        v += c->segs[k].size;
    }
    if (k >= c->nsegs) k = c->nsegs ? c->nsegs - 1 : 0;
    c->cur_seg = k;
    c->cur_used = (c->nsegs && mark >= v) ? (mark - v) : 0;
    if (mark == 0 && c->nsegs > 1) {
        rlhip_stream_sync(c);
        for (int i = 0; i < c->nsegs; ++i) hipFree(c->segs[i].base);
        c->nsegs = 0; c->cur_seg = 0; c->cur_used = 0;
        size_t want = align_up(c->ws_highwater + (c->ws_highwater >> 3), 1 << 20);
        char* p = nullptr;
        if (hipMalloc((void**)&p, want) == hipSuccess) { c->segs[0].base = p; c->segs[0].size = want; c->nsegs = 1; }
    }
}

__global__ void rlhip_zero_f64_kernel(double* p) { *p = 0.0; }

extern "C" {

const char* rlhip_version(void) { return "rlhip 0.1 (gfx950)"; }

int rlhip_create(rlhip_ctx** out, int device, void* hip_stream, int own_stream) {
    if (!out) return -1;
    int ndev = 0;
    hipError_t e = hipGetDeviceCount(&ndev);
    if (e != hipSuccess || ndev <= 0) {
        fprintf(stderr, "[rlhip] no HIP device visible (%s)\n", hipGetErrorString(e));
        return RLHIP_ERR_HIP(e == hipSuccess ? hipErrorNoDevice : e);
    }
    if (device < 0 || device >= ndev) return -2;
    RLHIP_CHECK(hipSetDevice(device));
    rlhip_ctx* c = new rlhip_ctx();
    c->device = device;
    {
        int ncu = 0;
        if (hipDeviceGetAttribute(&ncu, hipDeviceAttributeMultiprocessorCount, device) == hipSuccess && ncu > 0) c->num_cu = ncu;
    }
    if (!own_stream) {
        c->stream = (hipStream_t)hip_stream;
        c->owns_stream = false;
    } else {
        RLHIP_CHECK(hipStreamCreateWithFlags(&c->stream, hipStreamNonBlocking));
        c->owns_stream = true;
    }
    RLHIP_CHECK(hipHostMalloc((void**)&c->h_mail, MAIL_WORDS * sizeof(int64_t), hipHostMallocDefault));
    RLHIP_CHECK(hipMalloc((void**)&c->d_mail, MAIL_WORDS * sizeof(int64_t)));
    RLHIP_CHECK(hipEventCreate(&c->ev0));
    RLHIP_CHECK(hipEventCreate(&c->ev1));
    RLHIP_CHECK(hipEventCreateWithFlags(&c->ev_flag, hipEventDisableTiming));
    {
        char* p = nullptr;
        RLHIP_CHECK(hipMalloc((void**)&p, (size_t)64 << 20));
        c->segs[0].base = p; c->segs[0].size = (size_t)64 << 20; c->nsegs = 1;
    }
    {
        size_t fr = 0, tot = 0;
        c->pool_cap_bytes = (hipMemGetInfo(&fr, &tot) == hipSuccess) ? tot / 8 : ((size_t)8 << 30);
    }
    *out = c;
    return 0;
}

int rlhip_create_side(rlhip_ctx* parent, rlhip_ctx** out) {
    if (!parent || !out) return -1;
    RLHIP_CHECK(hipSetDevice(parent->device));
    int lo = 0, hi = 0;
    RLHIP_CHECK(hipDeviceGetStreamPriorityRange(&lo, &hi));
    hipStream_t st = nullptr;
    RLHIP_CHECK(hipStreamCreateWithPriority(&st, hipStreamNonBlocking, hi));
    const int rc = rlhip_create(out, parent->device, (void*)st, 0);
    if (rc) { hipStreamDestroy(st); return rc; }
    (*out)->owns_stream = true;
    for (int i = 0; i < RLHIP_OPT_COUNT; ++i) (*out)->opt[i] = parent->opt[i];
    (*out)->avoid_persistent = 1;
    return 0;
}

int rlhip_side_of(rlhip_ctx* parent, rlhip_ctx** out) {
    if (!parent || !out) return -1;
    if (!parent->side_ctx) {
        const int rc = rlhip_create_side(parent, &parent->side_ctx);
        if (rc) { parent->side_ctx = nullptr; return rc; }
    }
    *out = parent->side_ctx;
    return 0;
}

int rlhip_set_qrcp_cols(rlhip_ctx* c, int cols) {
    if (!c || cols < 0) return -1;
    c->qrcp_cols_per_wg = cols;
    return 0;
}

int rlhip_set_option(rlhip_ctx* c, int option, int64_t value) {
    if (!c || option < 0 || option >= RLHIP_OPT_COUNT) return -1;
    c->opt[option] = value;
    if (c->side_ctx) c->side_ctx->opt[option] = value;
    return 0;
}
int64_t rlhip_get_option(rlhip_ctx* c, int option) {
    if (!c || option < 0 || option >= RLHIP_OPT_COUNT) return INT64_MIN;
    return c->opt[option];
}

int rlhip_order_after(rlhip_ctx* waiter, rlhip_ctx* signaler) {
    if (!waiter || !signaler) return -1;
    if (waiter->stream == signaler->stream) return 0;
    hipEvent_t ev = nullptr;
    RLHIP_CHECK(hipEventCreateWithFlags(&ev, hipEventDisableTiming));
    hipError_t e = hipEventRecord(ev, signaler->stream);
    if (e == hipSuccess) e = hipStreamWaitEvent(waiter->stream, ev, 0);
    hipEventDestroy(ev);
    return e == hipSuccess ? 0 : RLHIP_ERR_HIP(e);
}

int rlhip_destroy(rlhip_ctx* c) {
    if (!c) return 0;
    rlhip_comm_destroy(c);
    hipSetDevice(c->device);
    rlhip_stream_sync(c);
    for (int i = 0; i < c->npool; ++i) hipFree(c->pool[i].p);
    for (int i = 0; i < c->nsegs; ++i) hipFree(c->segs[i].base);
    if (c->d_mail) hipFree(c->d_mail);
    if (c->xchg) hipFree(c->xchg);
    if (c->xloc) hipFree(c->xloc);
    if (c->h_mail) hipHostFree(c->h_mail);
    if (c->ev0) hipEventDestroy(c->ev0);
    if (c->ev1) hipEventDestroy(c->ev1);
    if (c->ev_flag) hipEventDestroy(c->ev_flag);
    if (c->side_ctx) { rlhip_destroy(c->side_ctx); c->side_ctx = nullptr; hipSetDevice(c->device); }
    if (c->side) hipStreamDestroy(c->side);
    if (c->owns_stream) hipStreamDestroy(c->stream);
    delete c;
    return 0;
}

int rlhip_sync(rlhip_ctx* c) { RLHIP_CHECK(rlhip_stream_sync(c)); return 0; }
void* rlhip_stream(rlhip_ctx* c) { return (void*)c->stream; }

static void pool_drop(rlhip_ctx* c, int i) {
    hipFree(c->pool[i].p);
    c->pool_idle_bytes -= c->pool[i].bytes;
    c->pool[i] = c->pool[--c->npool];
}
int rlhip_malloc_host(rlhip_ctx* c, void** p, size_t bytes) {
    RLHIP_CHECK(hipSetDevice(c->device));
    RLHIP_CHECK(hipHostMalloc(p, bytes ? bytes : 1, hipHostMallocMapped | hipHostMallocPortable));
    return 0;
}
int rlhip_free_host(rlhip_ctx* c, void* p) {
    if (!p) return 0;
    RLHIP_CHECK(rlhip_stream_sync(c));
    RLHIP_CHECK(hipHostFree(p));
    return 0;
}
int rlhip_trim(rlhip_ctx* c) {
    RLHIP_CHECK(rlhip_stream_sync(c));
    for (int i = c->npool - 1; i >= 0; --i)
        if (!c->pool[i].in_use) pool_drop(c, i);
    return 0;
}
int rlhip_malloc(rlhip_ctx* c, void** p, size_t bytes) {
    RLHIP_CHECK(hipSetDevice(c->device));
    bytes = bytes ? ((bytes + 255) & ~(size_t)255) : 256;
    for (int i = 0; i < c->npool; ++i)
        if (!c->pool[i].in_use && c->pool[i].bytes == bytes) {
            c->pool[i].in_use = true;
            c->pool_idle_bytes -= bytes;
            *p = c->pool[i].p;
            if (rlhip_poison()) (void)hipMemsetAsync(*p, 0xFF, bytes, c->stream);
            return 0;
        }
    static int trace = -1;
    if (trace < 0) { const char* t = getenv("RLHIP_POOL_TRACE"); trace = t ? atoi(t) : 0; }
    if (trace) fprintf(stderr, "[rlhip pool] miss: %zu bytes (%d blocks, %zu idle bytes)\n", bytes, c->npool, c->pool_idle_bytes);
    hipError_t e = hipMalloc(p, bytes);
    if (e != hipSuccess) {
        (void)hipGetLastError();
        rlhip_trim(c);
        e = hipMalloc(p, bytes);
        if (e != hipSuccess) { (void)hipGetLastError(); return RLHIP_ERR_HIP(e); }
    }
    if (c->npool >= 256) {
        int lru = -1;
        for (int j = 0; j < c->npool; ++j)
            if (!c->pool[j].in_use && (lru < 0 || c->pool[j].stamp < c->pool[lru].stamp)) lru = j;
        if (lru >= 0) { (void)rlhip_stream_sync(c); pool_drop(c, lru); }
    }
    if (c->npool < 256) c->pool[c->npool++] = {*p, bytes, true, 0};
    if (rlhip_poison()) (void)hipMemsetAsync(*p, 0xFF, bytes, c->stream);
    return 0;
}
int rlhip_free(rlhip_ctx* c, void* p) {
    if (!p) return 0;
    for (int i = 0; i < c->npool; ++i)
        if (c->pool[i].p == p) {
            c->pool[i].in_use = false;
            c->pool[i].stamp = ++c->pool_clock;
            c->pool_idle_bytes += c->pool[i].bytes;
            if (c->pool_idle_bytes > c->pool_cap_bytes) {
                RLHIP_CHECK(rlhip_stream_sync(c));
                while (c->pool_idle_bytes > c->pool_cap_bytes) {
                    int lru = -1;
                    for (int j = 0; j < c->npool; ++j)
                        if (!c->pool[j].in_use && (lru < 0 || c->pool[j].stamp < c->pool[lru].stamp)) lru = j;
                    if (lru < 0) break;
                    pool_drop(c, lru);
                }
            }
            return 0;
        }
    RLHIP_CHECK(rlhip_stream_sync(c));
    RLHIP_CHECK(hipFree(p));
    return 0;
}
int rlhip_memcpy_h2d(rlhip_ctx* c, void* dst, const void* src, size_t bytes) {
    RLHIP_CHECK(hipMemcpyAsync(dst, src, bytes, hipMemcpyHostToDevice, c->stream));
    RLHIP_CHECK(rlhip_stream_sync(c));
    return 0;
}
int rlhip_memcpy_d2h(rlhip_ctx* c, void* dst, const void* src, size_t bytes) {
    RLHIP_CHECK(hipMemcpyAsync(dst, src, bytes, hipMemcpyDeviceToHost, c->stream));
    RLHIP_CHECK(rlhip_stream_sync(c));
    return 0;
}
int rlhip_memcpy_d2d(rlhip_ctx* c, void* dst, const void* src, size_t bytes) {
    RLHIP_CHECK(hipMemcpyAsync(dst, src, bytes, hipMemcpyDeviceToDevice, c->stream));
    return 0;
}
int rlhip_memset(rlhip_ctx* c, void* dst, int byte, size_t bytes) {
    RLHIP_CHECK(hipMemsetAsync(dst, byte, bytes, c->stream));
    return 0;
}
int rlhip_reserve_workspace(rlhip_ctx* c, size_t bytes) {
    if (rlhip_ws_mark(c) != 0) return -2;
    size_t total = 0;
    for (int i = 0; i < c->nsegs; ++i) total += c->segs[i].size;
    if (c->nsegs == 1 && bytes <= total) return 0;
    RLHIP_CHECK(rlhip_stream_sync(c));
    for (int i = 0; i < c->nsegs; ++i) hipFree(c->segs[i].base);
    c->nsegs = 0; c->cur_seg = 0; c->cur_used = 0;
    bytes = align_up(bytes > total ? bytes : total, 1 << 20);
    char* p = nullptr;
    RLHIP_CHECK(hipMalloc((void**)&p, bytes));
    c->segs[0].base = p; c->segs[0].size = bytes; c->nsegs = 1;
    return 0;
}
size_t rlhip_workspace_highwater(rlhip_ctx* c) { return c->ws_highwater; }

size_t rlhip_scratch_mark(rlhip_ctx* c) { return rlhip_ws_mark(c); }
int rlhip_scratch_alloc(rlhip_ctx* c, void** p, size_t bytes) {
    *p = rlhip_ws_alloc(c, bytes);
    return *p ? 0 : RLHIP_ERR_HIP(hipErrorOutOfMemory);
}
int rlhip_scratch_release(rlhip_ctx* c, size_t mark) { rlhip_ws_release(c, mark); return 0; }

int rlhip_timer_start(rlhip_ctx* c) { RLHIP_CHECK(hipEventRecord(c->ev0, c->stream)); return 0; }
int rlhip_timer_stop_ms(rlhip_ctx* c, float* ms) {
    RLHIP_CHECK(hipEventRecord(c->ev1, c->stream));
    RLHIP_CHECK(hipEventSynchronize(c->ev1));
    RLHIP_CHECK(hipEventElapsedTime(ms, c->ev0, c->ev1));
    return 0;
}

int rlhip_philox4x32_10(rlhip_ctx* c, int64_t nblocks, uint32_t* out_dev, const uint32_t ctr[4],
                        const uint32_t key[2]) {
    return rlhip::philox_raw(c, nblocks, out_dev, ctr, key);
}
int rlhip_fill_dense_f64(rlhip_ctx* c, int dist, int64_t rows, int64_t cols, double* buf, const uint32_t ctr[4],
                         const uint32_t key[2], uint32_t next_ctr[4]) {
    return rlhip::fill_dense<double>(c, dist, rows, cols, buf, ctr, key, next_ctr);
}
int rlhip_fill_dense_rows_f64(rlhip_ctx* c, int dist, int64_t glob_rows, int64_t cols, int64_t row0, int64_t loc_rows, double* buf,
                              int64_t ld, const uint32_t ctr[4], const uint32_t key[2], uint32_t next_ctr[4]) {
    return rlhip::fill_dense_rows<double>(c, dist, glob_rows, cols, row0, loc_rows, buf, ld, ctr, key, next_ctr);
}
int rlhip_fill_dense_rows_f32(rlhip_ctx* c, int dist, int64_t glob_rows, int64_t cols, int64_t row0, int64_t loc_rows, float* buf,
                              int64_t ld, const uint32_t ctr[4], const uint32_t key[2], uint32_t next_ctr[4]) {
// ... 217 lines not shown
    if (op_flag(ta, &fa)) return -2;
    if (op_flag(tb, &fb)) return -3;
    double* d_ssq = (double*)(c->d_mail + MAIL_NORMA_SSQ);
    hipLaunchKernelGGL(rlhip_zero_f64_kernel, dim3(1), dim3(1), 0, c->stream, d_ssq);
    int done = 0;
    int rc = rlhip::gemm_impl<double>(c, fa, fb, m, n, k, alpha, A, lda, B, ldb, beta, C, ldc, 0, d_ssq, &done);
    if (rc) return rc;
    if (fused_host) *fused_host = done ? 1 : 0;
    const int64_t arows = fa ? k : m, acols = fa ? m : k;
    c->norma_state = 0;
    c->norma_reduced = 0;
    if (done == 2 && norm_a_host == nullptr) {
        RLHIP_CHECK(hipMemcpyAsync(c->h_mail + MAIL_NORMA_SSQ, d_ssq, sizeof(double), hipMemcpyDeviceToHost, c->stream));
        c->norma_state = 1;
        c->norma_epoch = c->sync_epoch;
        return 0;
    }
    double result = 0;
    if (!done) {
        rc = rlhip::lange_fro<double>(c, arows, acols, A, lda, &result);
        if (rc) return rc;
    } else {
        double ssq_main = 0, rest = 0;
        RLHIP_CHECK(hipMemcpyAsync(c->h_mail + MAIL_NORMA_SSQ, d_ssq, sizeof(double), hipMemcpyDeviceToHost, c->stream));
        RLHIP_CHECK(rlhip_stream_sync(c));
        ssq_main = *(double*)(c->h_mail + MAIL_NORMA_SSQ);
        const int64_t m_main = (m / 128) * 128;
        if (m_main < m && done != 2) {
            const double* A2 = fa ? (A + m_main * lda) : (A + m_main);
            rc = rlhip::lange_fro<double>(c, fa ? k : (m - m_main), fa ? (m - m_main) : k, A2, lda, &rest);
            if (rc) return rc;
        }
        result = sqrt(ssq_main + rest * rest);
    }
    if (norm_a_host) *norm_a_host = result;
    else { c->norma_value = result; c->norma_state = 2; }
    return 0;
}

int rlhip_norma_collect_f64(rlhip_ctx* c, int over_ranks, double* norm_a_host) {
    if (!norm_a_host) return -3;
    double ssq = 0;
    bool global = false;
    if (c->norma_state == 1) {
        if (c->sync_epoch == c->norma_epoch) RLHIP_CHECK(rlhip_stream_sync(c));
        if (over_ranks && c->norma_reduced) { ssq = *(double*)(c->h_mail + MAIL_NORMA_SSQ_RANKS); global = true; }
        else ssq = *(double*)(c->h_mail + MAIL_NORMA_SSQ);
    } else if (c->norma_state == 2) {
        ssq = c->norma_value * c->norma_value;
    } else {
        return -4;
    }
    c->norma_state = 0;
    c->norma_reduced = 0;
    if (over_ranks && !global && rlhip_comm_size(c) > 1) {
        const int rc = rlhip_allreduce_sum_host_f64(c, &ssq, 1);
        if (rc) return rc;
    }
    *norm_a_host = sqrt(ssq);
    return 0;
}

RLHIP_DEFINE_BLAS3(f64, double)
RLHIP_DEFINE_BLAS3(f32, float)

}

namespace {
typedef double d4_t __attribute__((ext_vector_type(4)));
typedef float f4_t __attribute__((ext_vector_type(4)));

__global__ __launch_bounds__(256) void mfma_peak_f64_kernel(int iters, double* out) {
    d4_t a0 = {0, 0, 0, 0}, a1 = a0, a2 = a0, a3 = a0, a4 = a0, a5 = a0, a6 = a0, a7 = a0;
    double x = 1.0 + threadIdx.x * 1e-9, y = 1.0 - threadIdx.x * 1e-9;
    for (int i = 0; i < iters; ++i) {
        a0 = __builtin_amdgcn_mfma_f64_16x16x4f64(x, y, a0, 0, 0, 0);
        a1 = __builtin_amdgcn_mfma_f64_16x16x4f64(x, y, a1, 0, 0, 0);
        a2 = __builtin_amdgcn_mfma_f64_16x16x4f64(x, y, a2, 0, 0, 0);
        a3 = __builtin_amdgcn_mfma_f64_16x16x4f64(x, y, a3, 0, 0, 0);
        a4 = __builtin_amdgcn_mfma_f64_16x16x4f64(x, y, a4, 0, 0, 0);
        a5 = __builtin_amdgcn_mfma_f64_16x16x4f64(x, y, a5, 0, 0, 0);
        a6 = __builtin_amdgcn_mfma_f64_16x16x4f64(x, y, a6, 0, 0, 0);
        a7 = __builtin_amdgcn_mfma_f64_16x16x4f64(x, y, a7, 0, 0, 0);
    }
    d4_t s = a0 + a1 + a2 + a3 + a4 + a5 + a6 + a7;
    if (s[0] == 12345.678) out[0] = s[1] + s[2] + s[3];
}
__global__ __launch_bounds__(256) void mfma_peak_f32_kernel(int iters, float* out) {
    f4_t a0 = {0, 0, 0, 0}, a1 = a0, a2 = a0, a3 = a0, a4 = a0, a5 = a0, a6 = a0, a7 = a0;
    float x = 1.0f + threadIdx.x * 1e-6f, y = 1.0f - threadIdx.x * 1e-6f;
    for (int i = 0; i < iters; ++i) {
        a0 = __builtin_amdgcn_mfma_f32_16x16x4f32(x, y, a0, 0, 0, 0);
        a1 = __builtin_amdgcn_mfma_f32_16x16x4f32(x, y, a1, 0, 0, 0);
        a2 = __builtin_amdgcn_mfma_f32_16x16x4f32(x, y, a2, 0, 0, 0);
        a3 = __builtin_amdgcn_mfma_f32_16x16x4f32(x, y, a3, 0, 0, 0);
        a4 = __builtin_amdgcn_mfma_f32_16x16x4f32(x, y, a4, 0, 0, 0);
        a5 = __builtin_amdgcn_mfma_f32_16x16x4f32(x, y, a5, 0, 0, 0);
        a6 = __builtin_amdgcn_mfma_f32_16x16x4f32(x, y, a6, 0, 0, 0);
        a7 = __builtin_amdgcn_mfma_f32_16x16x4f32(x, y, a7, 0, 0, 0);
    }
    f4_t s = a0 + a1 + a2 + a3 + a4 + a5 + a6 + a7;
    if (s[0] == 12345.678f) out[0] = s[1] + s[2] + s[3];
}
__global__ __launch_bounds__(256) void hbm_read_kernel(const double2* __restrict__ p, size_t n16, double* out) {
    double acc = 0;
    size_t stride = (size_t)gridDim.x * blockDim.x;
    for (size_t i = (size_t)blockIdx.x * blockDim.x + threadIdx.x; i < n16; i += stride) {
        double2 v = p[i];
        acc += v.x + v.y;
    }
    if (acc == 12345.678) out[0] = acc;
}
__global__ __launch_bounds__(256) void dvfs_burn_kernel(int mode, long long ticks, double* out) {
    const long long t0 = wall_clock64();
    d4_t a0 = {0, 0, 0, 0}, a1 = a0, a2 = a0, a3 = a0;
    double x = 1.0 + threadIdx.x * 1e-9, y = 1.0 - threadIdx.x * 1e-9, z = 0.5;
    while (wall_clock64() - t0 < ticks) {
        if (mode == 0) {
            __builtin_amdgcn_s_sleep(64);
        } else if (mode == 1) {
#pragma unroll
            for (int i = 0; i < 64; ++i) z = fma(z, x, y);
        } else {
#pragma unroll
            for (int i = 0; i < 8; ++i) {
                a0 = __builtin_amdgcn_mfma_f64_16x16x4f64(x, y, a0, 0, 0, 0);
                a1 = __builtin_amdgcn_mfma_f64_16x16x4f64(x, y, a1, 0, 0, 0);
                a2 = __builtin_amdgcn_mfma_f64_16x16x4f64(x, y, a2, 0, 0, 0);
                a3 = __builtin_amdgcn_mfma_f64_16x16x4f64(x, y, a3, 0, 0, 0);
            }
        }
    }
    d4_t s = a0 + a1 + a2 + a3;
    if (s[0] + z == 12345.678) out[0] = s[1];
}
}

extern "C" int rlhip_dvfs_burn(rlhip_ctx* c, int blocks, int mode, int usec, int side) {
    if (blocks <= 0 || usec <= 0) return 0;
    hipStream_t st = c->stream;
    if (side) {
        if (!c->side) RLHIP_CHECK(hipStreamCreateWithFlags(&c->side, hipStreamNonBlocking));
        st = c->side;
    }
    hipLaunchKernelGGL(dvfs_burn_kernel, dim3((unsigned)blocks), dim3(256), 0, st, mode, (long long)usec * 100, (double*)(c->d_mail + MAIL_DVFS_SINK));
    RLHIP_LAUNCH_CHECK();
    return 0;
}

extern "C" int64_t rlhip_path_count(rlhip_ctx* c, int which) {
    return (c && which >= 0 && which < RLHIP_NPATH) ? c->path_count[which] : -1;
}
extern "C" int64_t rlhip_lu_path_count(rlhip_ctx* c, int which) { return (c && which >= 60 && which <= 66) ? c->lu_path_count[which - 60] : -1; }
extern "C" int64_t rlhip_tri_path_count(rlhip_ctx* c, int which) { return (c && which >= 67 && which <= 73) ? c->tri_path_count[which - 67] : -1; }
extern "C" int rlhip_path_note(rlhip_ctx* c, int which, int64_t delta) {
    if (!c || which < 0 || which >= RLHIP_NPATH) return -1;
    c->path_count[which] += delta;
    return 0;
}

namespace {
typedef int (*fn_roctx_push)(const char*);
typedef int (*fn_roctx_pop)(void);
struct Roctx { int state = 0; fn_roctx_push push = nullptr; fn_roctx_pop pop = nullptr; };
Roctx g_roctx;
void roctx_bind() {
    g_roctx.state = -1;
    const char* names[] = {"librocprofiler-sdk-roctx.so.1", "librocprofiler-sdk-roctx.so", "libroctx64.so.4", "libroctx64.so"};
    void* h = nullptr;
    const char* want = getenv("RLHIP_ROCTX");
    if (want && want[0] == '0') return;
    for (const char* n : names) { h = dlopen(n, RTLD_NOW | RTLD_NOLOAD); if (h) break; }
    if (!h && want && want[0] == '1')
        for (const char* n : names) { h = dlopen(n, RTLD_NOW); if (h) break; }
    if (!h) return;
    g_roctx.push = (fn_roctx_push)dlsym(h, "roctxRangePushA");
    g_roctx.pop = (fn_roctx_pop)dlsym(h, "roctxRangePop");
    if (g_roctx.push && g_roctx.pop) g_roctx.state = 1;
}
}
extern "C" int rlhip_range_push(const char* name) {
    if (g_roctx.state == 0) roctx_bind();
    if (g_roctx.state == 1 && name) g_roctx.push(name);
    return 0;
}
extern "C" int rlhip_range_pop(void) {
    if (g_roctx.state == 1) g_roctx.pop();
    return 0;
}
extern "C" int rlhip_avoid_persistent(rlhip_ctx* c, int on) {
    if (!c) return -1;
    const int prev = c->avoid_persistent;
    c->avoid_persistent = on ? 1 : 0;
    return prev;
}

extern "C" int rlhip_mfma_peak(rlhip_ctx* c, int is_f64, int iters, double* tflops) {
    const int blocks = 256 * 8, threads = 256;
    double* d = (double*)(c->d_mail + MAIL_SCALAR);
    for (int rep = 0; rep < 2; ++rep) {
        RLHIP_CHECK(hipEventRecord(c->ev0, c->stream));
        if (is_f64)
            hipLaunchKernelGGL(mfma_peak_f64_kernel, dim3(blocks), dim3(threads), 0, c->stream, iters, d);
        else
            hipLaunchKernelGGL(mfma_peak_f32_kernel, dim3(blocks), dim3(threads), 0, c->stream, iters, (float*)d);
        RLHIP_LAUNCH_CHECK();
        RLHIP_CHECK(hipEventRecord(c->ev1, c->stream));
        RLHIP_CHECK(hipEventSynchronize(c->ev1));
    }
    float ms = 0;
    RLHIP_CHECK(hipEventElapsedTime(&ms, c->ev0, c->ev1));
    double flops = (double)blocks * (threads / 64) * (double)iters * 8.0 * (2.0 * 16 * 16 * 4);
    *tflops = flops / (ms * 1e-3) / 1e12;
    return 0;
}

extern "C" int rlhip_hbm_read_peak(rlhip_ctx* c, const void* buf, size_t bytes, double* gbps) {
    size_t n16 = bytes / 16;
    double* d = (double*)(c->d_mail + MAIL_SCALAR);
    for (int rep = 0; rep < 2; ++rep) {
        RLHIP_CHECK(hipEventRecord(c->ev0, c->stream));
        hipLaunchKernelGGL(hbm_read_kernel, dim3(256 * 16), dim3(256), 0, c->stream, (const double2*)buf, n16, d);
        RLHIP_LAUNCH_CHECK();
        RLHIP_CHECK(hipEventRecord(c->ev1, c->stream));
        RLHIP_CHECK(hipEventSynchronize(c->ev1));
    }
    float ms = 0;
    RLHIP_CHECK(hipEventElapsedTime(&ms, c->ev0, c->ev1));
    *gbps = (double)(n16 * 16) / (ms * 1e-3) / 1e9;
    return 0;
}
```

### randlapack_amd/csrc/rlhip_internal.h

```cpp
#pragma once
#include <mutex>
#include <utility>
#include <vector>
#include <hip/hip_runtime.h>
#include <cstdint>
#include <cstddef>
#include <cstdio>
#include "rlhip.h"

#define RLHIP_ERR_HIP(e) (-1000 - (int)(e))

#define RLHIP_CHECK(expr)                                                     \
    do {                                                                      \
        hipError_t _e = (expr);                                               \
        if (_e != hipSuccess) {                                               \
            fprintf(stderr, "[rlhip] %s:%d: %s -> %s\n", __FILE__, __LINE__,  \
                    #expr, hipGetErrorString(_e));                            \
            return RLHIP_ERR_HIP(_e);                                         \
        }                                                                     \
    } while (0)

#define RLHIP_LAUNCH_CHECK() RLHIP_CHECK(hipGetLastError())

#define RLHIP_FUNC_LDS(c, func, bytes)                                                                                     \
    do {                                                                                                                   \
        static bool _rlhip_lds_done[64] = {};                                                                              \
        const int _d = (c)->device & 63;                                                                                   \
        if (!_rlhip_lds_done[_d]) {                                                                                        \
            RLHIP_CHECK(hipSetDevice((c)->device));                                                                        \
            RLHIP_CHECK(hipFuncSetAttribute((const void*)(func), hipFuncAttributeMaxDynamicSharedMemorySize, (int)(bytes))); \
            _rlhip_lds_done[_d] = true;                                                                                    \
        }                                                                                                                  \
    } while (0)

#define RLHIP_FUNC_LDS_DYN(c, func, bytes)                                                                                 \
    do {                                                                                                                   \
        static std::mutex _rlhip_lds_mu;                                                                                   \
        static std::vector<std::pair<int, const void*>> _rlhip_lds_seen;                                                   \
        std::lock_guard<std::mutex> _rlhip_lds_lock(_rlhip_lds_mu);                                                        \
        const std::pair<int, const void*> _key((c)->device, (const void*)(func));                                          \
        bool _found = false;                                                                                               \
        for (auto const& _e : _rlhip_lds_seen) _found = _found || (_e == _key);                                            \
        if (!_found) {                                                                                                     \
            RLHIP_CHECK(hipSetDevice((c)->device));                                                                        \
            RLHIP_CHECK(hipFuncSetAttribute(_key.second, hipFuncAttributeMaxDynamicSharedMemorySize, (int)(bytes)));       \
            _rlhip_lds_seen.push_back(_key);                                                                               \
        }                                                                                                                  \
    } while (0)

constexpr int MAIL_WORDS = 64;
constexpr int MAIL_SCALAR = 0;
constexpr int MAIL_ABSMAX = 1;
constexpr int MAIL_POTRF_INFO = 8;
constexpr int MAIL_JACOBI = 16;
constexpr int MAIL_TRSM_VERDICT = 16;
constexpr int MAIL_TRSM_VERDICT_WORDS = 17;
constexpr int MAIL_SVD_RATIO = 24;
constexpr int MAIL_SVD_GRAM_DEV = 25;
constexpr int MAIL_SVD_GRAM = 32;
constexpr int MAIL_SVD_GRAM_WORDS = 5;
constexpr int MAIL_SVD_GRAM_DEFECT = MAIL_SVD_GRAM + 4;
constexpr int MAIL_HOST_REDUCE = 32;
constexpr int MAIL_HOST_REDUCE_WORDS = 16;
constexpr int MAIL_DVFS_SINK = 32;
constexpr int MAIL_NORMA_SSQ = 40;
constexpr int MAIL_NORMA_SSQ_RANKS = 41;
constexpr int MAIL_GEQRF_CHOLQR = 44;
constexpr int MAIL_CHOLQRQ = 44;
constexpr int MAIL_CHOLQRQ_WORDS = 20;
constexpr int MAIL_ANY_FLAG = 48;
constexpr int MAIL_CSR_NNZ = 50;
constexpr int MAIL_CSR_BAD = 51;
constexpr int MAIL_CSR_MAXLEN = MAIL_CSR_BAD + 1;
constexpr int MAIL_PANEL_INFO = 56;
constexpr int MAIL_SAMPLE_HDR = 60;
constexpr int MAIL_SAMPLE_HDR_WORDS = 4;
constexpr bool mail_disjoint(int a, int na, int b, int nb) { return a + na <= b || b + nb <= a; }
static_assert(MAIL_TRSM_VERDICT + MAIL_TRSM_VERDICT_WORDS <= MAIL_WORDS && MAIL_SVD_GRAM + MAIL_SVD_GRAM_WORDS <= MAIL_WORDS &&
              MAIL_HOST_REDUCE + MAIL_HOST_REDUCE_WORDS <= MAIL_WORDS && MAIL_CHOLQRQ + MAIL_CHOLQRQ_WORDS <= MAIL_WORDS &&
              MAIL_CSR_BAD + 2 <= MAIL_WORDS && MAIL_SAMPLE_HDR + MAIL_SAMPLE_HDR_WORDS <= MAIL_WORDS, "a mailbox extent ends within the mailbox");
static_assert(mail_disjoint(MAIL_TRSM_VERDICT, MAIL_TRSM_VERDICT_WORDS, MAIL_NORMA_SSQ, 2) && mail_disjoint(MAIL_SVD_GRAM, MAIL_SVD_GRAM_WORDS, MAIL_NORMA_SSQ, 2) &&
              mail_disjoint(MAIL_JACOBI, 4, MAIL_NORMA_SSQ, 2) && mail_disjoint(MAIL_CHOLQRQ, MAIL_CHOLQRQ_WORDS, MAIL_NORMA_SSQ, 2),
              "a transient h_mail range covers the deferred norm");

constexpr int RLHIP_NPATH = 43;
struct rlhip_ctx {
    int device = 0;
    int num_cu = 256;
    hipStream_t stream = nullptr;
    bool owns_stream = false;
    struct Seg { char* base; size_t size; };
    Seg segs[32];
    int nsegs = 0;
    int cur_seg = 0;
    size_t cur_used = 0;
    size_t ws_highwater = 0;
    int64_t* h_mail = nullptr;
    int64_t* d_mail = nullptr;
    void* xchg = nullptr;
    size_t xchg_bytes = 0;
    void* xloc = nullptr;
    size_t xloc_bytes = 0;
    hipEvent_t ev0 = nullptr, ev1 = nullptr;
    hipEvent_t ev_flag = nullptr;
    int norma_state = 0;
    double norma_value = 0;
    int norma_reduced = 0;
    unsigned long norma_epoch = 0;
    unsigned long sync_epoch = 0;
    int avoid_persistent = 0;
    int qrcp_cols_per_wg = 0;
    int64_t opt[RLHIP_OPT_COUNT] = {-1, -1, -1, -1, -1, -1, -1, -1, -1, -1, -1, -1, -1, -1, -1};
    rlhip_ctx* side_ctx = nullptr;
    hipStream_t side = nullptr;
    void* comm = nullptr;
    struct PoolBlk { void* p; size_t bytes; bool in_use; unsigned long stamp; };
    PoolBlk pool[256];
    int npool = 0;
    size_t pool_idle_bytes = 0, pool_cap_bytes = 0;
    unsigned long pool_clock = 0;
    int64_t path_count[RLHIP_NPATH] = {};
    int64_t pcg_path_count[3] = {};
    int64_t lsq_path_count[4] = {};
    int64_t spmv_path_count[5] = {};
    int64_t rbf_path_count[3] = {};
    int64_t rbf_split_count = 0;
    int64_t var_path_count[2] = {};
    int64_t lu_path_count[7] = {};
    int64_t tri_path_count[7] = {};
    int var_fused = 0;
    int64_t grad_path_count[2] = {};
    int grad_fused = 0;
};

static inline hipError_t rlhip_stream_sync(rlhip_ctx* c) {
    const hipError_t e = hipStreamSynchronize(c->stream);
    if (e == hipSuccess) ++c->sync_epoch;
    return e;
}

void* rlhip_ws_alloc(rlhip_ctx* c, size_t bytes);
size_t rlhip_ws_mark(rlhip_ctx* c);
void rlhip_ws_release(rlhip_ctx* c, size_t mark);

template <typename T>
static inline T* ws_alloc(rlhip_ctx* c, size_t n) { return (T*)rlhip_ws_alloc(c, n * sizeof(T)); }

struct ws_scope {
    rlhip_ctx* const c;
    const size_t mark;
    explicit ws_scope(rlhip_ctx* ctx) : c(ctx), mark(rlhip_ws_mark(ctx)) {}
    ~ws_scope() { rlhip_ws_release(c, mark); }
    ws_scope(const ws_scope&) = delete;
    ws_scope& operator=(const ws_scope&) = delete;
    template <typename T>
    T* alloc(size_t n) { return ws_alloc<T>(c, n); }
};
void* rlhip_xchg_buffer(rlhip_ctx* c, size_t bytes);
void* rlhip_xloc_buffer(rlhip_ctx* c, size_t bytes);

namespace rlhip {

enum Op : int { NoTrans = 0, Trans = 1 };
enum Uplo : int { Upper = 0, Lower = 1 };
enum Diag : int { NonUnit = 0, Unit = 1 };
enum Dist : int { Gaussian = 0, UniformPM1 = 1 };

template <typename T>
int gemm(rlhip_ctx* c, int transA, int transB, int64_t m, int64_t n, int64_t k, T alpha, const T* A,
         int64_t lda, const T* B, int64_t ldb, T beta, T* C, int64_t ldc);

template <typename T>
int syrk(rlhip_ctx* c, int uplo, int trans, int64_t n, int64_t k, T alpha, const T* A, int64_t lda,
         T beta, T* C, int64_t ldc);

template <typename T>
int potrf_upper(rlhip_ctx* c, int64_t n, T* A, int64_t lda, int* info_host);

template <typename T>
int trsm_right_upper_oop(rlhip_ctx* c, int diag, int64_t m, int64_t n, T alpha, const T* A, int64_t lda, const T* Bsrc, int64_t ldsrc,
                         const int64_t* perm_dev, T* B, int64_t ldb);
template <typename T>
int trsm_right_upper_oop_range(rlhip_ctx* c, int diag, int64_t m, int64_t nsrc, T alpha, const T* A, int64_t lda, const T* Bsrc, int64_t ldsrc,
                               const int64_t* perm_dev, T* B, int64_t ldb, int64_t col0, int64_t col1);
template <typename T>
int trsm_right_upper(rlhip_ctx* c, int diag, int64_t m, int64_t n, T alpha, const T* A, int64_t lda,
                     T* B, int64_t ldb);

template <typename T>
int trmm_right_upper(rlhip_ctx* c, int diag, int64_t m, int64_t n, T alpha, const T* A, int64_t lda,
                     T* B, int64_t ldb);

template <typename T>
int trmm_left_upper(rlhip_ctx* c, int trans, int diag, int64_t m, int64_t n, T alpha, const T* A, int64_t lda, T* B, int64_t ldb);

template <typename T>
int fill_dense(rlhip_ctx* c, int dist, int64_t rows, int64_t cols, T* buf, const uint32_t ctr[4],
               const uint32_t key[2], uint32_t next_ctr[4]);

template <typename T>
int lange_fro(rlhip_ctx* c, int64_t m, int64_t n, const T* A, int64_t lda, T* result_host);

template <typename T>
int lacpy(rlhip_ctx* c, int uplo , int64_t m, int64_t n, const T* A,
          int64_t lda, T* B, int64_t ldb);

template <typename T>
int laset(rlhip_ctx* c, int uplo , int64_t m, int64_t n, T offdiag, T diag,
          T* A, int64_t lda);

template <typename T>
int gesvdj(rlhip_ctx* c, int64_t m, int64_t n, T* A, int64_t lda, T* S, T* VT, int64_t ldvt,
           int* sweeps_host);


template <typename T>
int gesvdj_core(rlhip_ctx* c, int64_t m, int64_t n, T* A, int64_t lda, T* S, T* VT, int64_t ldvt, int* sweeps_host);
template <typename T>
int svd_guard_begin(rlhip_ctx* c, int64_t m, int64_t n, T* A, int64_t lda, unsigned long long* w);
template <typename T>
int svd_guard_end(rlhip_ctx* c, int64_t n, T* S, const unsigned long long* w);

template <typename T>
int add_diag(rlhip_ctx* c, int64_t n, T alpha, T* A, int64_t lda);

template <typename T>
int transpose(rlhip_ctx* c, int64_t m, int64_t n, const T* A, int64_t lda, T* AT, int64_t ldat, int upper_only);

template <typename T>
int gesdd_tall(rlhip_ctx* c, int64_t m, int64_t n, T* A, int64_t lda, T* S, T* U, int64_t ldu, T* VT,
               int64_t ldvt, int* sweeps_host);

template <typename T>
int gemm_impl(rlhip_ctx* c, int transA, int transB, int64_t m, int64_t n, int64_t k, T alpha, const T* A, int64_t lda,
              const T* B, int64_t ldb, T beta, T* C, int64_t ldc, int tri, double* ssqA_dev = nullptr, int* ssq_done = nullptr);

template <typename T>
int gemm_streamk(rlhip_ctx* c, int transA, int transB, int64_t m, int64_t n, int64_t k, T alpha, const T* A, int64_t lda, const T* B,
                 int64_t ldb, T beta, T* C, int64_t ldc, double* ssqA_dev, int tri);

template <typename T>
int fill_dense_rows(rlhip_ctx* c, int dist, int64_t glob_rows, int64_t cols, int64_t row0, int64_t loc_rows, T* buf, int64_t ld,
                    const uint32_t ctr[4], const uint32_t key[2], uint32_t next_ctr[4]);
int philox_raw(rlhip_ctx* c, int64_t nblk, uint32_t* out_dev, const uint32_t ctr[4], const uint32_t key[2]);

template <typename T>
int potrf_upper_enqueue(rlhip_ctx* c, int64_t n, T* A, int64_t lda, int* info_dev);

template <typename T>
int cholqrq(rlhip_ctx* c, int64_t m, int64_t k, T* A, int64_t lda, T* R, int reduce_gram, int* info_host);

template <typename T>
int jacobi_enqueue_rt(rlhip_ctx* c, int n, const T* R, int64_t ldr, int trans_upper, float norm_ratio_lim, const int* skip_dev, int* out_dev,
                      const T** X_out);

struct SasoOp;
int saso_build(rlhip_ctx* c, int64_t d, int64_t m, int nnz, int mode, const uint32_t ctr[4], const uint32_t key[2],
               uint32_t next_ctr[4], SasoOp** out);
int saso_destroy(rlhip_ctx* c, SasoOp* op);
template <typename T>
int saso_dense(rlhip_ctx* c, const SasoOp* op, T* S );
template <typename T>
int saso_apply_rows(rlhip_ctx* c, const SasoOp* op, int64_t n, T alpha, const T* A, int64_t lda, int64_t row0, int64_t mloc, T beta,
                    T* B, int64_t ldb);
template <typename T>
int saso_apply(rlhip_ctx* c, const SasoOp* op, int64_t n, T alpha, const T* A, int64_t lda, T beta, T* B, int64_t ldb);
template <typename T>
int saso_apply_csr(rlhip_ctx* c, const SasoOp* op, int64_t n, T alpha, const int64_t* rowptrT, const int64_t* colidxT, const T* valsT, T beta,
                   T* B, int64_t ldb, int64_t row0);
template <typename T>
int saso_apply_csr_ordered(rlhip_ctx* c, const SasoOp* op, int64_t n, T alpha, const int64_t* rowptrT, const int64_t* colidxT, const T* valsT, T beta,
                           T* B, int64_t ldb);
template <typename T>
int col_swap(rlhip_ctx* c, int64_t m, int64_t n, int64_t k, T* A, int64_t lda, const int64_t* idx_dev);
int col_swap_i64(rlhip_ctx* c, int64_t n, int64_t k, int64_t* A, const int64_t* idx_dev);

template <typename T>
int geqp3(rlhip_ctx* c, int64_t m, int64_t n, T* A, int64_t lda, int64_t* jpvt_dev, T* tau_dev);
template <typename T>
int qrp_partial(rlhip_ctx* c, int64_t m, int64_t n, int64_t steps, T* A, int64_t lda, int64_t* jpvt_dev, T* tau_dev);
template <typename T>
int geqp3_steps(rlhip_ctx* c, int64_t m, int64_t n, int64_t steps, T* A, int64_t lda, int64_t* jpvt_dev, T* tau_dev);
template <typename T>
int geqrf(rlhip_ctx* c, int64_t m, int64_t n, T* A, int64_t lda, T* tau_dev);
template <typename T>
int ungqr(rlhip_ctx* c, int64_t m, int64_t n, T* A, int64_t lda, const T* tau_dev);

template <typename T>
int geqrf_blk(rlhip_ctx* c, int64_t m, int64_t n, T* A, int64_t lda, T* tau_dev);
template <typename T>
int lunp_blk(rlhip_ctx* c, int64_t n, T* A, int64_t lda, T* D);

template <typename T>
int orhr_col(rlhip_ctx* c, int64_t m, int64_t n, int64_t nb, T* A, int64_t lda, T* Tm, int64_t ldt, T* D);
template <typename T>
int gemqrt_lt(rlhip_ctx* c, int64_t m, int64_t n, int64_t k, int64_t nb, const T* V, int64_t ldv, const T* Tm, int64_t ldt,
              T* C, int64_t ldc);
template <typename T>
int gemqrt_lt_head(rlhip_ctx* c, int64_t m, int64_t n, int64_t k, const T* V, int64_t ldv, const T* Tm, int64_t ldt, T* C, int64_t ldc, T* W2);
template <typename T>
int gemqrt_lt_tail(rlhip_ctx* c, int64_t m, int64_t n, int64_t k, const T* V, int64_t ldv, const T* W2, T* C, int64_t ldc);
template <typename T>
int gemqrt_rn(rlhip_ctx* c, int64_t m, int64_t n, int64_t k, const T* V, int64_t ldv, const T* Tm, int64_t ldt, T* C, int64_t ldc);
template <typename T>
int larft_gram(rlhip_ctx* c, int64_t m, int64_t k, const T* V, int64_t ldv, const T* tau, T* Tm, int64_t ldt);
template <typename T>
int row_sign(rlhip_ctx* c, int64_t n, T* R, int64_t ldr, const T* D);
template <typename T>
int tau_from_t(rlhip_ctx* c, int64_t k, int64_t nb, const T* Tm, int64_t ldt, T* tau);
template <typename T>
int any_abs_gt(rlhip_ctx* c, int64_t n, const T* x, T thr, int* any_host);
template <typename T>
int geqrf_cholqr(rlhip_ctx* c, int64_t m, int64_t n, T* A, int64_t lda, T* tau, int* done);
template <typename T>
int geqrf_q(rlhip_ctx* c, int64_t m, int64_t n, T* A, int64_t lda, T* R, int64_t ldr, int* done);
template <typename T>
int vrows_explicit(rlhip_ctx* c, int64_t br, int64_t toff, int64_t tcnt, const T* Vtop, int64_t ldv, T* out, int64_t ldo);

template <typename T>
int getrf(rlhip_ctx* c, int64_t m, int64_t n, T* A, int64_t lda, int64_t* ipiv_dev, int* info_host, int pivots_only);
template <typename T>
int laswp(rlhip_ctx* c, int64_t n, T* A, int64_t lda, int64_t k1, int64_t k2, const int64_t* ipiv_dev);
int luqrcp_piv(rlhip_ctx* c, int64_t sd, int64_t cols, const int64_t* ipiv_dev, int64_t* J_dev);

template <typename T>
int gemv(rlhip_ctx* c, int trans, int64_t m, int64_t n, T alpha, const T* A, int64_t lda, const T* x, T beta, T* y);
template <typename T>
int dot_dev(rlhip_ctx* c, int64_t n, const T* x, const T* y, T* out_dev);

template <typename T>
struct PdkFn {
    bool matern;
    T scale, third;
    bool weight = false;
};
inline bool pdk_kind_ok(int kernel) { return kernel >= RLHIP_PDK_SQEXP && kernel <= RLHIP_PDK_MATERN52; }
template <typename T>
PdkFn<T> pdk_fn(int kernel, T bandwidth) {
    const double l = (double)bandwidth;
    if (kernel == RLHIP_PDK_SQEXP) return {false, (T)(-1.0 / (2.0 * l * l)), T(0)};
    if (kernel == RLHIP_PDK_MATERN32) return {true, (T)(1.7320508075688772 / l), T(0)};
    return {true, (T)(2.23606797749979 / l), (T)(1.0 / 3.0)};
}
template <typename T>
PdkFn<T> pdk_weight_fn(int kernel, T bandwidth, T* w0) {
    const double l = (double)bandwidth;
    if (kernel == RLHIP_PDK_SQEXP) { *w0 = (T)(-1.0 / (l * l)); return {false, (T)(-1.0 / (2.0 * l * l)), T(0), false}; }
    if (kernel == RLHIP_PDK_MATERN32) { *w0 = (T)(-3.0 / (l * l)); return {true, (T)(1.7320508075688772 / l), T(0), true}; }
    *w0 = (T)(-5.0 / (3.0 * l * l));
    return {true, (T)(2.23606797749979 / l), T(1), true};
}
template <typename T>
int sqexp_colnorms(rlhip_ctx* c, int64_t rows_x, int64_t cols, const T* X, int64_t ldx, T* nr);
template <typename T>
int pdk_epilogue(rlhip_ctx* c, int64_t rows, int64_t cols, const T* nr_rows, const T* nr_cols, PdkFn<T> f, T* K, int64_t ldk);

template <typename T>
int pdk_cross_apply_fn(rlhip_ctx* c, int64_t rows_x, int64_t mz, const T* Z, int64_t ldz, int64_t nx, const T* X, int64_t ldx, PdkFn<T> f, int64_t n,
                       T alpha, const T* B, int64_t ldb, T beta, T* C, int64_t ldc);

}
```

### randlapack_amd/csrc/tri.hip

```cpp
#include <cstdlib>
#include "rlhip_device.h"
#include <cstdio>

namespace {

using namespace rlhip_dev;

constexpr int SB = 32;
constexpr int RW = 256;
constexpr int BW = 256;

template <typename T>
__global__ void pack_upper_rows_kernel(int nb, int ldp, int unit, const T* __restrict__ U, int64_t ldu,
                                       T* __restrict__ Ut) {
    int idx = blockIdx.x * blockDim.x + threadIdx.x;
    if (idx >= ldp * ldp) return;
    int c = idx % ldp, l = idx / ldp;
    T v = 0;
    if (l < nb && c < nb) {
        if (l < c) v = U[l + (int64_t)c * ldu];
        else if (l == c) v = unit ? T(1) : T(1) / U[l + (int64_t)c * ldu];
    } else if (l == c) {
        v = 1;
    }
// ... 463 lines not shown
#pragma unroll
                for (int r = 0; r < 4; ++r) {
                    T* dst = bj + (int64_t)(16 * (2 * s + u) + CS * r) * ldb + loff;
                    *(live ? dst : dl) = acc[2 * s + u][r];
                }
        };
        auto retire_load = [&](int s) {
            const int64_t cbn = has_next ? col0 + 256 : col0;
#pragma unroll
            for (int u = 0; u < 2; ++u)
#pragma unroll
                for (int r = 0; r < 4; ++r) acc[2 * s + u][r] = load_raw(cbn, 2 * s + u, r);
        };
        auto retire_tiles = [&](int s) { retire_store(s); retire_load(s); };
        {
            auto dpair = [&](auto s_c) {
                constexpr int s = decltype(s_c)::value;
                wait_vm<(s >= 2) ? DW : 0>();
                __builtin_amdgcn_s_barrier();
                const T* sU = reinterpret_cast<const T*>(tf_smem + ring * HPB);
                solve_sub(s);
                T y[NQ];
#pragma unroll
                for (int q = 0; q < NQ; ++q) y[q] = M::operand(acc[2 * s], 4 * q, lane);
                panel_mma(IntC<2 * s + 2>{}, acc, sU, y, [&]() {
                    if (s >= 1) retire_store(s - 1);
                    issue_panel((s + 1 < 7) ? panel_ptr(J, ntoff + 2 * (s + 1)) : (has_next ? panel_ptr(J + 1, 0) : panel_ptr(J, 0)), ring ^ 1);
                    issue_dinv((int64_t)J * 8 + s + 1);
                    if (s >= 1) retire_load(s - 1);
                });
#pragma unroll
                for (int q = 0; q < NQ; ++q) y[q] = M::operand(acc[2 * s + 1], 4 * q, lane);
                panel_mma(IntC<2 * s + 2>{}, acc, sU + 16 * FSTR, y, [&]() {});
                ring ^= 1;
                TF_MARK(1 + 2 * s)
            };
            dpair(IntC<0>{}); dpair(IntC<1>{}); dpair(IntC<2>{}); dpair(IntC<3>{}); dpair(IntC<4>{}); dpair(IntC<5>{}); dpair(IntC<6>{});
            wait_vm<DW>();
            __builtin_amdgcn_s_barrier();
            solve_sub(7);
            retire_tiles(6);
            retire_tiles(7);
            TF_MARK(15)
            if (has_next) {
                issue_dinv((int64_t)(J + 1) * 8);
                xissue(B + (int64_t)K0blk * 256 * ldb, xc);
            }
        }
    }
#ifdef RLHIP_TF_PROF
    if (blockIdx.x == gridDim.x / 2 && threadIdx.x == 0) for (int i = 0; i < 16; ++i) ((long long*)(dump + 512))[i] = tfp[i];
#endif
}

__global__ void perm_check_kernel(int64_t n, const int64_t* __restrict__ perm, int64_t pbase, unsigned* __restrict__ seen, int* __restrict__ bad, int64_t nsrc) {
    const int64_t i = (int64_t)blockIdx.x * blockDim.x + threadIdx.x;
    if (i >= n) return;
    const int64_t sidx = perm[i] - pbase;
    if (sidx < 0 || sidx >= nsrc) { atomicExch(bad, 1); return; }
    const unsigned bit = 1u << (sidx & 31);
    if (atomicOr(seen + (sidx >> 5), bit) & bit) atomicExch(bad, 1);
}

template <typename T>
__global__ __launch_bounds__(256) void gather_cols_kernel(int64_t m, int64_t n, const T* __restrict__ src, int64_t lds_, const int64_t* __restrict__ perm,
                                                          int64_t pbase, T* __restrict__ dst, int64_t ldd) {
    const int64_t c = blockIdx.y;
    const int64_t sc = perm ? perm[c] - pbase : c;
    for (int64_t i = (int64_t)blockIdx.x * 256 + threadIdx.x; i < m; i += (int64_t)gridDim.x * 256) dst[i + c * ldd] = src[i + sc * lds_];
}


#ifndef RLHIP_TF_XASM_DEFAULT
#define RLHIP_TF_XASM_DEFAULT 1
#endif
constexpr int64_t TF_MIN_ROWS = 16384;
inline bool tf_xasm(const rlhip_ctx* c) {
    const int64_t o = c->opt[RLHIP_OPT_TRSM_XASM];
    return o < 0 ? (RLHIP_TF_XASM_DEFAULT != 0) : (o != 0);
}
inline bool tf_offsets_fit(int64_t ld, int64_t m) { return (4 * ld + m) < ((int64_t)1 << 28); }

constexpr int TF_HPR = 32;
constexpr double TF_KAPPA2_LIMIT = 1.0e6;
constexpr int TF_MAX_BLOCKS = 32;
constexpr int TF_PIVOT_WORD = TF_MAX_BLOCKS;
constexpr int TF_VERDICT_WORDS = TF_PIVOT_WORD + 1;
constexpr int TF_VERDICT_ALLOC = 40;
static_assert(TF_VERDICT_WORDS <= TF_VERDICT_ALLOC && TF_VERDICT_WORDS * sizeof(int) <= MAIL_TRSM_VERDICT_WORDS * sizeof(int64_t) &&
              TF_VERDICT_ALLOC * sizeof(int) <= MAIL_CHOLQRQ_WORDS * sizeof(int64_t), "the verdict words fit their mailbox ranges");

template <typename T>
hipError_t tf_enqueue_blk_pack(rlhip_ctx* c, int64_t n, int64_t nblk, int diag, const T* A, int64_t lda, T* Upk_all, T* Dinv_all, int* bad) {
    hipLaunchKernelGGL(trsm_blk_pack_kernel<T>, dim3(BW / 32 + 24, (unsigned)nblk), dim3(256), 0, c->stream, n, diag, A, lda, Upk_all, Dinv_all, bad,
                       TF_KAPPA2_LIMIT);
    return hipGetLastError();
}
template <typename T>
hipError_t tf_enqueue_neg_pack(rlhip_ctx* c, int64_t n, int64_t n_pad, const T* A, int64_t lda, T* Uneg) {
    hipLaunchKernelGGL(trsm_neg_pack_kernel<T>, dim3((unsigned)(n_pad / 32), (unsigned)(n_pad / 32)), dim3(256), 0, c->stream, n, n_pad, A, lda, Uneg);
    return hipGetLastError();
}
inline hipError_t tf_enqueue_perm_check(rlhip_ctx* c, int64_t n, const int64_t* perm, int64_t nsrc, unsigned* seen, int* bad, bool clear_bad) {
    hipError_t e = hipMemsetAsync(seen, 0, ((size_t)nsrc + 31) / 32 * sizeof(unsigned), c->stream);
    if (e == hipSuccess && clear_bad) e = hipMemsetAsync(bad, 0, sizeof(int), c->stream);
    if (e != hipSuccess) return e;
    hipLaunchKernelGGL(perm_check_kernel, dim3((unsigned)((n + 255) / 256)), dim3(256), 0, c->stream, n, perm, (int64_t)1, seen, bad, nsrc);
    return hipGetLastError();
}

template <typename T>
struct TfArgs {
    int64_t m, n, n_pad;
    T alpha;
    const T* Uneg;
    const T* Dinv;
    T* B;
    int64_t ldb;
    int J0, J1, K0blk;
    T* dump;
    const T* Bsrc = nullptr;
    int64_t ldsrc = 0;
    const int64_t* perm = nullptr;
    int64_t pbase = 0;
    const int* gate = nullptr;
    int ngate = 0;
};

template <typename T, int NW, int OOP, bool XASM>
int tf_launch_one(rlhip_ctx* c, const TfArgs<T>& a) {
    constexpr int lds = fused_lds_bytes<T, TF_HPR>();
    RLHIP_FUNC_LDS(c, (trsm_fused_kernel<T, NW, TF_HPR, OOP, XASM>), lds);
    hipLaunchKernelGGL((trsm_fused_kernel<T, NW, TF_HPR, OOP, XASM>), dim3((unsigned)((a.m + 16 * NW - 1) / (16 * NW))), dim3(64 * NW), lds, c->stream, a.m, a.n,
                       a.n_pad, a.alpha, a.Uneg, a.Dinv, a.B, a.ldb, a.J0, a.J1, a.K0blk, a.dump, a.Bsrc, a.ldsrc, a.perm, a.pbase, a.gate, a.ngate);
    RLHIP_LAUNCH_CHECK();
    return 0;
}

template <typename T, int OOP>
int tf_launch(rlhip_ctx* c, const TfArgs<T>& a) {
    const bool xasm = tf_xasm(c);
    if constexpr (sizeof(T) == 4 && OOP == 0) {
        const int64_t ncu = c->num_cu > 0 ? c->num_cu : 256;
        auto cost = [&](int64_t nw) { const int64_t wg = (a.m + 16 * nw - 1) / (16 * nw); return ((wg + ncu - 1) / ncu) * nw; };
        if (cost(12) < cost(8)) {
            const int rc = xasm ? tf_launch_one<T, 12, OOP, true>(c, a) : tf_launch_one<T, 12, OOP, false>(c, a);
            if (!rc) c->tri_path_count[2]++;
            return rc;
        }
    }
    return xasm ? tf_launch_one<T, 8, OOP, true>(c, a) : tf_launch_one<T, 8, OOP, false>(c, a);
}

}

namespace rlhip {

template <typename T>
int trsm_right_upper(rlhip_ctx* c, int diag, int64_t m, int64_t n, T alpha, const T* A, int64_t lda, T* B,
                     int64_t ldb) {
    if (m < 0) return -6;
    if (n < 0) return -7;
    if (lda < (n > 1 ? n : 1)) return -10;
    if (ldb < (m > 1 ? m : 1)) return -12;
    if (m == 0 || n == 0) return 0;
    ws_scope ws(c);
    T* Ut = ws.alloc<T>((size_t)SB * SB);
    if (!Ut) return RLHIP_ERR_HIP(hipErrorOutOfMemory);
    const int64_t nblk = (n + BW - 1) / BW;
    const bool try_blk = m >= 16 && n >= 128 && nblk <= TF_MAX_BLOCKS;
    T* Upk_all = try_blk ? ws.alloc<T>((size_t)nblk * BW * BW) : nullptr;
    T* Dinv_all = try_blk ? ws.alloc<T>((size_t)nblk * (BW / 32) * 1024) : nullptr;
    int* bad_dev = try_blk ? ws.alloc<int>(TF_MAX_BLOCKS) : nullptr;
    int bad_host[TF_MAX_BLOCKS];
    for (int i = 0; i < TF_MAX_BLOCKS; ++i) bad_host[i] = 1;
    if (try_blk) {
        if (!Upk_all || !Dinv_all || !bad_dev) return RLHIP_ERR_HIP(hipErrorOutOfMemory);
        RLHIP_CHECK(hipMemsetAsync(bad_dev, 0, TF_MAX_BLOCKS * sizeof(int), c->stream));
        RLHIP_CHECK(tf_enqueue_blk_pack<T>(c, n, nblk, diag, A, lda, Upk_all, Dinv_all, bad_dev));
        RLHIP_CHECK(hipMemcpyAsync(c->h_mail + MAIL_TRSM_VERDICT, bad_dev, TF_MAX_BLOCKS * sizeof(int), hipMemcpyDeviceToHost, c->stream));
        RLHIP_CHECK(rlhip_stream_sync(c));
        for (int i = 0; i < TF_MAX_BLOCKS; ++i) bad_host[i] = ((const int*)(c->h_mail + MAIL_TRSM_VERDICT))[i];
    }
    const bool use_fused = try_blk && m >= TF_MIN_ROWS && n >= BW && tf_offsets_fit(ldb, m);
    const int64_t n_pad = nblk * BW;
    T* Uneg = nullptr;
    T* fdump = nullptr;
    if (use_fused) {
        bool any_good = false;
        for (int64_t b = 0; (b + 1) * BW <= n; ++b) any_good |= !bad_host[b];
        if (any_good) {
            Uneg = ws.alloc<T>((size_t)n_pad * n_pad);
            if (!Uneg) return RLHIP_ERR_HIP(hipErrorOutOfMemory);
            RLHIP_CHECK(tf_enqueue_neg_pack<T>(c, n, n_pad, A, lda, Uneg));
            fdump = ws.alloc<T>(512 + 64);
            if (!fdump) return RLHIP_ERR_HIP(hipErrorOutOfMemory);
        }
    }
    for (int64_t j0 = 0; j0 < n; j0 += BW) {
        const int nb = (int)((n - j0 < BW) ? (n - j0) : BW);
        T a = alpha;
        if (Uneg && !bad_host[j0 / BW] && j0 + BW <= n) {
            const int Jb = (int)(j0 / BW);
            int Je = Jb;
            while (Je < nblk && !bad_host[Je] && (int64_t)(Je + 1) * BW <= n) ++Je;
            const int64_t jend = (Je * (int64_t)BW < n) ? Je * (int64_t)BW : n;
            if (j0 > 0) {
                int rc = gemm_impl<T>(c, 0, 0, m, jend - j0, j0, T(-1), B, ldb, A + j0 * lda, lda, alpha, B + j0 * ldb, ldb, 0);
                if (rc) return rc;
                a = T(1);
            }
            {
                const int lrc = tf_launch<T, 0>(c, TfArgs<T>{m, n, n_pad, a, Uneg, Dinv_all, B, ldb, Jb, Je, Jb, fdump});
                if (lrc) return lrc;
            }
#ifdef RLHIP_TF_PROF
            {
                long long pf[16];
                rlhip_stream_sync(c);
                hipMemcpy(pf, fdump + 512, sizeof(pf), hipMemcpyDeviceToHost);
                fprintf(stderr, "[trsm prof, one workgroup, us over %d blocks] off-diagonal %.1f | diag steps", Je - Jb, pf[0] / 100.0);
                for (int i = 1; i <= 14; ++i) fprintf(stderr, " %.1f", pf[i] / 100.0);
                fprintf(stderr, " | tail %.1f\n", pf[15] / 100.0);
            }
#endif
            c->path_count[2]++;
            j0 = (int64_t)(Je - 1) * BW;
            continue;
        }
        if (j0 > 0) {
            int rc = gemm_impl<T>(c, 0, 0, m, nb, j0, T(-1), B, ldb, A + j0 * lda, lda, alpha, B + j0 * ldb, ldb, 0);
            if (rc) return rc;
            a = T(1);
        }
        if (try_blk && !bad_host[j0 / BW]) {
            const T* Upk_b = Upk_all + (j0 / BW) * (int64_t)BW * BW;
            const T* Dinv_b = Dinv_all + (j0 / BW) * (int64_t)(BW / 32) * 1024;
            if (m >= 65536)
                hipLaunchKernelGGL((trsm_blk_kernel<T, 2>), dim3((unsigned)((m + 127) / 128)), dim3(256), 0, c->stream, m, nb, a, Upk_b, Dinv_b, B + j0 * ldb, ldb, 0, 0);
            else
                hipLaunchKernelGGL((trsm_blk_kernel<T, 1>), dim3((unsigned)((m + 63) / 64)), dim3(256), 0, c->stream, m, nb, a, Upk_b, Dinv_b, B + j0 * ldb, ldb, 0, 0);
            RLHIP_LAUNCH_CHECK();
            c->tri_path_count[m >= 65536 ? 1 : 0]++;
            continue;
        }
        for (int s0 = 0; s0 < nb; s0 += SB) {
            const int sbw = (nb - s0 < SB) ? (nb - s0) : SB;
            const int64_t jc = j0 + s0;
            T a2 = a;
            if (s0 > 0) {
                int rc = gemm_impl<T>(c, 0, 0, m, sbw, s0, T(-1), B + j0 * ldb, ldb, A + j0 + jc * lda, lda, a, B + jc * ldb,
                                      ldb, 0);
                if (rc) return rc;
                a2 = T(1);
            }
            hipLaunchKernelGGL(pack_upper_rows_kernel<T>, dim3((SB * SB + 255) / 256), dim3(256), 0, c->stream, sbw, SB, diag,
                               A + jc + jc * lda, lda, Ut);
            hipLaunchKernelGGL(trsm_diag_kernel<T>, dim3((unsigned)((m + RW - 1) / RW)), dim3(RW), 0, c->stream, m, sbw, SB, a2,
                               Ut, B + jc * ldb, ldb);
            RLHIP_LAUNCH_CHECK();
            c->path_count[3]++;
        }
    }
    return 0;
}

template <typename T>
static int trsm_oop_fused(rlhip_ctx* c, int diag, int64_t m, int64_t nsrc, T alpha, const T* A, int64_t lda, const T* Bsrc, int64_t ldsrc,
                          const int64_t* perm_dev, T* B, int64_t ldb, int64_t col0, int64_t col1, bool may_ident, bool* perm_checked) {
    const int64_t n = col1, nblk = (n + BW - 1) / BW;
    if (m < TF_MIN_ROWS || n < BW || n % BW != 0 || nblk > TF_MAX_BLOCKS || !tf_offsets_fit(ldb, m)) return 1;
    ws_scope ws(c);
    T* Upk_all = ws.alloc<T>((size_t)nblk * BW * BW);
    T* Dinv_all = ws.alloc<T>((size_t)nblk * (BW / 32) * 1024);
    int* bad_dev = ws.alloc<int>(TF_VERDICT_ALLOC);
    unsigned* seen = ws.alloc<unsigned>((size_t)nsrc / 32 + 2);
    T* Uneg = ws.alloc<T>((size_t)n * n);
    T* fdump = ws.alloc<T>(512);
    if (!Upk_all || !Dinv_all || !bad_dev || !seen || !Uneg || !fdump) return RLHIP_ERR_HIP(hipErrorOutOfMemory);
    RLHIP_CHECK(hipMemsetAsync(bad_dev, 0, TF_VERDICT_WORDS * sizeof(int), c->stream));
    RLHIP_CHECK(tf_enqueue_blk_pack<T>(c, n, nblk, diag, A, lda, Upk_all, Dinv_all, bad_dev));
    if (perm_dev) {
        RLHIP_CHECK(tf_enqueue_perm_check(c, n, perm_dev, nsrc, seen, bad_dev + TF_PIVOT_WORD, false));
        *perm_checked = true;
    }
    const int* verdict = (const int*)(c->h_mail + MAIL_TRSM_VERDICT);
    RLHIP_CHECK(hipMemcpyAsync(c->h_mail + MAIL_TRSM_VERDICT, bad_dev, TF_VERDICT_WORDS * sizeof(int), hipMemcpyDeviceToHost, c->stream));
    RLHIP_CHECK(hipEventRecord(c->ev_flag, c->stream));
    RLHIP_CHECK(tf_enqueue_neg_pack<T>(c, n, n, A, lda, Uneg));
    bool ident = false;
    {
        TfArgs<T> a{m, n, n, alpha, Uneg, Dinv_all, B, ldb, (int)(col0 / BW), (int)nblk, 0, fdump};
        a.Bsrc = Bsrc; a.ldsrc = ldsrc;
        a.perm = perm_dev; a.pbase = 1;
        a.gate = bad_dev; a.ngate = TF_VERDICT_WORDS;
        ident = may_ident && !perm_dev && tf_offsets_fit(ldsrc, m);
        const int lrc = ident ? tf_launch<T, 2>(c, a) : tf_launch<T, 1>(c, a);
        if (lrc) return lrc;
    }
    RLHIP_CHECK(hipEventSynchronize(c->ev_flag));
    if (perm_dev && verdict[TF_PIVOT_WORD] != 0) return -7;
    for (int64_t b = 0; b < nblk; ++b)
        if (verdict[b] != 0) return 1;
    c->path_count[4]++;
    if (ident) c->tri_path_count[3]++;
    return 0;
}

template <typename T>
int trsm_right_upper_oop(rlhip_ctx* c, int diag, int64_t m, int64_t n, T alpha, const T* A, int64_t lda, const T* Bsrc, int64_t ldsrc,
                         const int64_t* perm_dev, T* B, int64_t ldb) {
    if (m < 0) return -6;
    if (n < 0) return -7;
    if (lda < (n > 1 ? n : 1)) return -10;
    if (ldsrc < (m > 1 ? m : 1)) return -12;
    if (ldb < (m > 1 ? m : 1)) return -15;
    if (m == 0 || n == 0) return 0;
    if ((const T*)B == Bsrc) { if (perm_dev) return -14; return trsm_right_upper<T>(c, diag, m, n, alpha, A, lda, B, ldb); }
    bool perm_checked = false;
    const int frc = trsm_oop_fused<T>(c, diag, m, n, alpha, A, lda, Bsrc, ldsrc, perm_dev, B, ldb, 0, n, true, &perm_checked);
    if (frc <= 0) return frc;
    if (perm_dev && !perm_checked) {
        ws_scope ws(c);
        unsigned* seen = ws.alloc<unsigned>((size_t)n / 32 + 2);
        int* bad = ws.alloc<int>(8);
        if (!seen || !bad) return RLHIP_ERR_HIP(hipErrorOutOfMemory);
        RLHIP_CHECK(tf_enqueue_perm_check(c, n, perm_dev, n, seen, bad, true));
        RLHIP_CHECK(hipMemcpyAsync(c->h_mail + MAIL_TRSM_VERDICT, bad, sizeof(int), hipMemcpyDeviceToHost, c->stream));
        RLHIP_CHECK(rlhip_stream_sync(c));
        if (*(const int*)(c->h_mail + MAIL_TRSM_VERDICT) != 0) return -7;
    }
    {
        unsigned gx = (unsigned)((m + 256 * 8 - 1) / (256 * 8));
        if (gx < 1) gx = 1;
        hipLaunchKernelGGL(gather_cols_kernel<T>, dim3(gx, (unsigned)n), dim3(256), 0, c->stream, m, n, Bsrc, ldsrc, perm_dev, (int64_t)1, B, ldb);
        RLHIP_LAUNCH_CHECK();
        c->tri_path_count[4]++;
    }
    return trsm_right_upper<T>(c, diag, m, n, alpha, A, lda, B, ldb);
}

template <typename T>
int trsm_right_upper_oop_range(rlhip_ctx* c, int diag, int64_t m, int64_t nsrc, T alpha, const T* A, int64_t lda, const T* Bsrc, int64_t ldsrc,
                               const int64_t* perm_dev, T* B, int64_t ldb, int64_t col0, int64_t col1) {
    if (m < 0) return -6;
    if (col0 < 0 || col1 <= col0 || col0 % BW || col1 % BW) return -7;
    if (nsrc < col1) return -7;
    if (lda < col1) return -10;
    if (ldsrc < (m > 1 ? m : 1)) return -12;
    if (ldb < (m > 1 ? m : 1)) return -15;
    if (m == 0) return 0;
    if ((const T*)B == Bsrc) return -14;
    bool perm_checked = false;
    return trsm_oop_fused<T>(c, diag, m, nsrc, alpha, A, lda, Bsrc, ldsrc, perm_dev, B, ldb, col0, col1, false, &perm_checked);
}

template <typename T>
int trmm_right_upper(rlhip_ctx* c, int diag, int64_t m, int64_t n, T alpha, const T* A, int64_t lda, T* B,
                     int64_t ldb) {
    if (m < 0) return -6;
    if (n < 0) return -7;
    if (lda < (n > 1 ? n : 1)) return -10;
    if (ldb < (m > 1 ? m : 1)) return -12;
    if (m == 0 || n == 0) return 0;
    ws_scope ws(c);
    T* W = ws.alloc<T>((size_t)n * n);
    T* Bc = ws.alloc<T>((size_t)m * n);
    if (!W || !Bc) return RLHIP_ERR_HIP(hipErrorOutOfMemory);
    hipLaunchKernelGGL(copy_triu_kernel<T>, dim3((unsigned)((n * n + 255) / 256)), dim3(256), 0, c->stream, n, diag, A,
                       lda, W);
    RLHIP_LAUNCH_CHECK();
    int rc = lacpy<T>(c, 2, m, n, B, ldb, Bc, m);
    if (!rc) rc = gemm_impl<T>(c, 0, 0, m, n, n, alpha, Bc, m, W, n, T(0), B, ldb, 0);
    if (!rc) c->tri_path_count[5]++;
    return rc;
}

template <typename T>
int trmm_left_upper(rlhip_ctx* c, int trans, int diag, int64_t m, int64_t n, T alpha, const T* A, int64_t lda, T* B, int64_t ldb) {
    if (m < 0) return -6;
    if (n < 0) return -7;
    if (lda < (m > 1 ? m : 1)) return -10;
    if (ldb < (m > 1 ? m : 1)) return -12;
    if (m == 0 || n == 0) return 0;
    ws_scope ws(c);
    T* W = ws.alloc<T>((size_t)m * m);
    T* Bc = ws.alloc<T>((size_t)m * n);
    if (!W || !Bc) return RLHIP_ERR_HIP(hipErrorOutOfMemory);
    hipLaunchKernelGGL(copy_triu_kernel<T>, dim3((unsigned)((m * m + 255) / 256)), dim3(256), 0, c->stream, m, diag, A, lda, W);
    RLHIP_LAUNCH_CHECK();
    int rc = lacpy<T>(c, 2, m, n, B, ldb, Bc, m);
    if (!rc) rc = gemm_impl<T>(c, trans ? 1 : 0, 0, m, n, m, alpha, W, m, Bc, m, T(0), B, ldb, 0);
    if (!rc) c->tri_path_count[6]++;
    return rc;
}
template int trmm_left_upper<double>(rlhip_ctx*, int, int, int64_t, int64_t, double, const double*, int64_t, double*, int64_t);
template int trmm_left_upper<float>(rlhip_ctx*, int, int, int64_t, int64_t, float, const float*, int64_t, float*, int64_t);

template <typename T>
int cholqrq(rlhip_ctx* c, int64_t m, int64_t k, T* A, int64_t lda, T* R, int reduce_gram, int* info_host) {
    const int64_t nblk = (k + BW - 1) / BW;
    if (c->opt[RLHIP_OPT_CHOLQRQ_ONE_STREAM] == 0 || k < BW || k % BW != 0 || k > 448 || nblk > TF_MAX_BLOCKS - 1 || lda < (m > 1 ? m : 1)) return 1;
    bool local_ok = m >= TF_MIN_ROWS && tf_offsets_fit(lda, m);
    if (!reduce_gram && !local_ok) return 1;
    *info_host = 0;
    hipError_t e1 = hipSuccess;
    {
        ws_scope ws(c);
        int* words = ws.alloc<int>(TF_VERDICT_ALLOC);
        if (!words) return reduce_gram ? RLHIP_ERR_HIP(hipErrorOutOfMemory) : 1;
        T *Upk_all = nullptr, *Dinv_all = nullptr, *Uneg = nullptr, *fdump = nullptr;
        if (local_ok) {
            Upk_all = ws.alloc<T>((size_t)nblk * BW * BW);
            Dinv_all = ws.alloc<T>((size_t)nblk * (BW / 32) * 1024);
            Uneg = ws.alloc<T>((size_t)k * k);
            fdump = ws.alloc<T>(512 + 64);
            if (!Upk_all || !Dinv_all || !Uneg || !fdump) {
                if (!reduce_gram) return 1;
                local_ok = false;
            }
        }
        hipError_t e0 = hipMemsetAsync(words, 0, TF_VERDICT_ALLOC * sizeof(int), c->stream);
        if (e0 != hipSuccess) return RLHIP_ERR_HIP(e0);
        int rc = laset<T>(c, 2, k, k, T(0), T(0), R, k);
        if (!rc && m > 0) rc = syrk<T>(c, Upper, 1, k, m, T(1), A, lda, T(0), R, k);
        if (!rc && reduce_gram) {
            if (sizeof(T) == 8 && c->norma_state == 1 && !c->norma_reduced) {
                double* G2 = ws.alloc<double>((size_t)k * k + 1);
                if (!G2) return RLHIP_ERR_HIP(hipErrorOutOfMemory);
                hipError_t e = hipMemcpyAsync(G2, R, (size_t)k * k * sizeof(double), hipMemcpyDeviceToDevice, c->stream);
                if (e == hipSuccess) e = hipMemcpyAsync(G2 + (size_t)k * k, (double*)(c->d_mail + MAIL_NORMA_SSQ), sizeof(double), hipMemcpyDeviceToDevice, c->stream);
                if (e != hipSuccess) return RLHIP_ERR_HIP(e);
                rc = rlhip_allreduce_sum_f64(c, G2, k * k + 1);
                if (!rc) {
                    e = hipMemcpyAsync(R, G2, (size_t)k * k * sizeof(double), hipMemcpyDeviceToDevice, c->stream);
                    if (e == hipSuccess) e = hipMemcpyAsync(c->h_mail + MAIL_NORMA_SSQ_RANKS, G2 + (size_t)k * k, sizeof(double), hipMemcpyDeviceToHost, c->stream);
                    if (e != hipSuccess) return RLHIP_ERR_HIP(e);
                    c->norma_reduced = 1;
                }
            } else {
                rc = (sizeof(T) == 8) ? rlhip_allreduce_sum_f64(c, (double*)R, k * k) : rlhip_allreduce_sum_f32(c, (float*)R, k * k);
            }
        }
        if (!rc) rc = potrf_upper_enqueue<T>(c, k, R, k, words);
        if (rc) return rc < 0 ? rc : RLHIP_ERR_HIP(hipErrorUnknown);
        if (local_ok) {
            RLHIP_CHECK(tf_enqueue_blk_pack<T>(c, k, nblk, (int)NonUnit, R, k, Upk_all, Dinv_all, words + 1));
            RLHIP_CHECK(tf_enqueue_neg_pack<T>(c, k, k, R, k, Uneg));
            TfArgs<T> a{m, k, k, T(1), Uneg, Dinv_all, A, lda, 0, (int)nblk, 0, fdump};
            a.gate = words; a.ngate = 1 + (int)nblk;
            rc = tf_launch<T, 0>(c, a);
            if (rc) return rc;
        }
        e1 = hipMemcpyAsync(c->h_mail + MAIL_CHOLQRQ, words, TF_VERDICT_ALLOC * sizeof(int), hipMemcpyDeviceToHost, c->stream);
        if (e1 == hipSuccess) e1 = rlhip_stream_sync(c);
    }
    if (e1 != hipSuccess) return RLHIP_ERR_HIP(e1);
    const int* w = (const int*)(c->h_mail + MAIL_CHOLQRQ);
    *info_host = w[0];
    if (w[0] != 0) return 0;
    bool guard = !local_ok;
    for (int64_t b = 0; b < nblk; ++b) guard = guard || (w[1 + b] != 0);
    if (guard) return trsm_right_upper<T>(c, NonUnit, m, k, T(1), R, k, A, lda);
    c->path_count[2]++;
    c->path_count[11]++;
    return 0;
}
template int cholqrq<double>(rlhip_ctx*, int64_t, int64_t, double*, int64_t, double*, int, int*);
template int cholqrq<float>(rlhip_ctx*, int64_t, int64_t, float*, int64_t, float*, int, int*);

template int trsm_right_upper<double>(rlhip_ctx*, int, int64_t, int64_t, double, const double*, int64_t, double*, int64_t);
template int trsm_right_upper_oop<double>(rlhip_ctx*, int, int64_t, int64_t, double, const double*, int64_t, const double*, int64_t, const int64_t*, double*, int64_t);
template int trsm_right_upper_oop<float>(rlhip_ctx*, int, int64_t, int64_t, float, const float*, int64_t, const float*, int64_t, const int64_t*, float*, int64_t);
template int trsm_right_upper_oop_range<double>(rlhip_ctx*, int, int64_t, int64_t, double, const double*, int64_t, const double*, int64_t, const int64_t*, double*, int64_t, int64_t, int64_t);
template int trsm_right_upper_oop_range<float>(rlhip_ctx*, int, int64_t, int64_t, float, const float*, int64_t, const float*, int64_t, const int64_t*, float*, int64_t, int64_t, int64_t);
template int trsm_right_upper<float>(rlhip_ctx*, int, int64_t, int64_t, float, const float*, int64_t, float*, int64_t);
template int trmm_right_upper<double>(rlhip_ctx*, int, int64_t, int64_t, double, const double*, int64_t, double*, int64_t);
template int trmm_right_upper<float>(rlhip_ctx*, int, int64_t, int64_t, float, const float*, int64_t, float*, int64_t);

}
```

### randlapack_amd/device.py

```python
from __future__ import annotations

import ctypes as C

import numpy as np

from . import _lib

_TORCH_DT = None


def _torch():
    import torch

    return torch


def _suffix(t):
    torch = _torch()
    if t.dtype == torch.float64:
        return "f64", C.c_double
    if t.dtype == torch.float32:
        return "f32", C.c_float
    raise TypeError(f"unsupported dtype {t.dtype}")

# ... 53 lines not shown
    def timer_stop_ms(self) -> float:
        ms = C.c_float()
        _lib.check(self.lib.rlhip_timer_stop_ms(self.h, C.byref(ms)), "timer_stop")
        return float(ms.value)

    def reserve_workspace(self, nbytes: int):
        _lib.check(self.lib.rlhip_reserve_workspace(self.h, nbytes), "reserve_workspace")

    @staticmethod
    def _u32(vals):
        arr = (C.c_uint32 * len(vals))(*[int(v) & 0xFFFFFFFF for v in vals])
        return arr

    def philox(self, nblocks: int, ctr, key):
        torch = _torch()
        out = torch.empty(4 * nblocks, dtype=torch.int32, device=f"cuda:{self.device}")
        _lib.check(
            self.lib.rlhip_philox4x32_10(self.h, nblocks, out.data_ptr(), self._u32(ctr), self._u32(key)), "philox"
        )
        return out.cpu().numpy().view(np.uint32)

    def fill_dense(self, buf, rows: int, cols: int, ctr=(0, 0, 0, 0), key=(0, 0), dist: int = 0):
        suf, _ = _suffix(buf)
        nxt = (C.c_uint32 * 4)()
        fn = getattr(self.lib, f"rlhip_fill_dense_{suf}")
        _lib.check(fn(self.h, dist, rows, cols, buf.data_ptr(), self._u32(ctr), self._u32(key), nxt), "fill_dense")
        return tuple(int(x) for x in nxt)

    def gemm(self, ta, tb, m, n, k, alpha, A, lda, B, ldb, beta, Cm, ldc):
        suf, T = _suffix(Cm)
        fn = getattr(self.lib, f"rlhip_gemm_{suf}")
        return _lib.check(
            fn(self.h, ta.encode(), tb.encode(), m, n, k, T(alpha), A.data_ptr(), lda, B.data_ptr(), ldb, T(beta),
               Cm.data_ptr(), ldc),
            "gemm",
        )

    def syrk(self, uplo, trans, n, k, alpha, A, lda, beta, Cm, ldc):
        suf, T = _suffix(Cm)
        fn = getattr(self.lib, f"rlhip_syrk_{suf}")
        return _lib.check(
            fn(self.h, uplo.encode(), trans.encode(), n, k, T(alpha), A.data_ptr(), lda, T(beta), Cm.data_ptr(), ldc),
            "syrk",
        )

    def trsm(self, m, n, alpha, A, lda, B, ldb, diag="N"):
        suf, T = _suffix(B)
        fn = getattr(self.lib, f"rlhip_trsm_{suf}")
        return _lib.check(
            fn(self.h, b"R", b"U", b"N", diag.encode(), m, n, T(alpha), A.data_ptr(), lda, B.data_ptr(), ldb), "trsm"
        )

    def trsm_gather(self, m, n, alpha, A, lda, Bsrc, ldsrc, jpvt, B, ldb, diag="N"):
        suf, T = _suffix(B)
        fn = getattr(self.lib, f"rlhip_trsm_gather_{suf}")
        return _lib.check(
            fn(self.h, diag.encode(), m, n, T(alpha), A.data_ptr(), lda, Bsrc.data_ptr(), ldsrc, jpvt.data_ptr() if jpvt is not None else None,
               B.data_ptr(), ldb), "trsm_gather")

    def trmm(self, m, n, alpha, A, lda, B, ldb, diag="N"):
        suf, T = _suffix(B)
        fn = getattr(self.lib, f"rlhip_trmm_{suf}")
        return _lib.check(
            fn(self.h, b"R", b"U", b"N", diag.encode(), m, n, T(alpha), A.data_ptr(), lda, B.data_ptr(), ldb), "trmm"
        )

    def potrf(self, n, A, lda) -> int:
        suf, _ = _suffix(A)
        fn = getattr(self.lib, f"rlhip_potrf_{suf}")
        return _lib.check(fn(self.h, b"U", n, A.data_ptr(), lda), "potrf")

    def lange_fro(self, m, n, A, lda) -> float:
        suf, T = _suffix(A)
        res = T()
        fn = getattr(self.lib, f"rlhip_lange_fro_{suf}")
        _lib.check(fn(self.h, m, n, A.data_ptr(), lda, C.byref(res)), "lange")
        return float(res.value)

    def lacpy(self, uplo, m, n, A, lda, B, ldb):
        suf, _ = _suffix(A)
        fn = getattr(self.lib, f"rlhip_lacpy_{suf}")
        return _lib.check(fn(self.h, uplo.encode(), m, n, A.data_ptr(), lda, B.data_ptr(), ldb), "lacpy")

    def laset(self, uplo, m, n, offd, diag, A, lda):
        suf, T = _suffix(A)
        fn = getattr(self.lib, f"rlhip_laset_{suf}")
        return _lib.check(fn(self.h, uplo.encode(), m, n, T(offd), T(diag), A.data_ptr(), lda), "laset")

    def gesvdj(self, m, n, A, lda, S, VT, ldvt):
        suf, _ = _suffix(A)
        sweeps = C.c_int()
        fn = getattr(self.lib, f"rlhip_gesvdj_{suf}")
        info = _lib.check(fn(self.h, m, n, A.data_ptr(), lda, S.data_ptr(), VT.data_ptr(), ldvt, C.byref(sweeps)),
                          "gesvdj")
        return info, int(sweeps.value)

    def path_count(self, which: int) -> int:
        return int(self.lib.rlhip_path_count(self.h, which))

    def pcg_path_count(self, which: int) -> int:
        return int(self.lib.rlhip_pcg_path_count(self.h, which))

    def lsq_path_count(self, which: int) -> int:
        return int(self.lib.rlhip_lsq_path_count(self.h, which))

    def spmv_path_count(self, which: int) -> int:
        return int(self.lib.rlhip_spmv_path_count(self.h, which))

    def rbf_path_count(self, which: int) -> int:
        return int(self.lib.rlhip_rbf_path_count(self.h, which))

    def rbf_split_count(self) -> int:
        return int(self.lib.rlhip_rbf_split_count(self.h))

    def var_path_count(self, which: int) -> int:
        return int(self.lib.rlhip_pdk_var_path_count(self.h, which))

    def grad_path_count(self, which: int) -> int:
        return int(self.lib.rlhip_pdk_grad_path_count(self.h, which))

    def grad_fused(self, on: bool = True):
        import contextlib

        @contextlib.contextmanager
        def _cm():
            was = int(self.lib.rlhip_pdk_grad_set_fused(self.h, int(bool(on))))
            try:
                yield self
            finally:
                self.lib.rlhip_pdk_grad_set_fused(self.h, was)
        return _cm()

    def lu_path_count(self, which: int) -> int:
        return int(self.lib.rlhip_lu_path_count(self.h, which))

    def tri_path_count(self, which: int) -> int:
        return int(self.lib.rlhip_tri_path_count(self.h, which))

    def var_fused(self, on: bool = True):
        import contextlib

        @contextlib.contextmanager
        def _cm():
            was = int(self.lib.rlhip_pdk_var_set_fused(self.h, int(bool(on))))
            try:
                yield self
            finally:
                self.lib.rlhip_pdk_var_set_fused(self.h, was)
        return _cm()

    OPT = dict(cholqrq_one_stream=0, gesdd_gram=1, jacobi_persist=2, trsm_xasm=3, saso_mode=4, hqrrp_tall_panel=5,
               bqrrp_lookahead_min_elems=6, bqrrp_cholqr_fallback=7, cqrrpt_fold_pivoting=8, cqrrpt_split_qrcp=9, sparse_sketch_densify=10, jacobi_clock_holders=11,
               lsq_normal_fused=12, spmv_lanes=13, rbf_fused=14)

    def set_option(self, name: str, value: int) -> None:
        _lib.check(self.lib.rlhip_set_option(self.h, self.OPT[name], int(value)), "set_option")

    def get_option(self, name: str) -> int:
        return int(self.lib.rlhip_get_option(self.h, self.OPT[name]))

    def options(self, **kw):
        import contextlib

        @contextlib.contextmanager
        def _cm():
            old = {k: self.get_option(k) for k in kw}
            try:
                for k, v in kw.items():
                    self.set_option(k, v)
                yield self
            finally:
                for k, v in old.items():
                    self.set_option(k, v)
        return _cm()

    def gemm_norma(self, ta, tb, m, n, k, alpha, A, lda, B, ldb, beta, Cm, ldc):
        nrm, fused = C.c_double(), C.c_int()
        _lib.check(self.lib.rlhip_gemm_norma_f64(self.h, ta.encode(), tb.encode(), m, n, k, alpha, A.data_ptr(), lda, B.data_ptr(), ldb,
                                                 beta, Cm.data_ptr(), ldc, C.byref(nrm), C.byref(fused)), "gemm_norma")
        return float(nrm.value), int(fused.value)

    def mfma_peak(self, is_f64=True, iters=20000) -> float:
        tf = C.c_double()
        _lib.check(self.lib.rlhip_mfma_peak(self.h, 1 if is_f64 else 0, iters, C.byref(tf)), "mfma_peak")
        return float(tf.value)

    def hbm_read_peak(self, buf) -> float:
        g = C.c_double()
        nbytes = buf.numel() * buf.element_size()
        _lib.check(self.lib.rlhip_hbm_read_peak(self.h, buf.data_ptr(), nbytes, C.byref(g)), "hbm_read_peak")
        return float(g.value)


def _state_arr(ctr, key):
    return (C.c_uint32 * 6)(*[int(v) & 0xFFFFFFFF for v in list(ctr) + list(key)])


class _Owned:

    def __init__(self, ctx: "Context", ptr: int, shape, typestr: str):
        self._ctx, self._ptr = ctx, ptr
        self.__cuda_array_interface__ = {"shape": tuple(shape), "typestr": typestr, "data": (ptr, False), "version": 2, "strides": None}

    def __del__(self):
        try:
            if self._ptr and getattr(self._ctx, "h", None):
                self._ctx.lib.rlhip_free(self._ctx.h, C.c_void_p(self._ptr))
        except Exception:
            pass
        self._ptr = 0


def _adopt(ctx: "Context", ptr: C.c_void_p, rows: int, cols: int, dtype=None):
    torch = _torch()
    dtype = dtype or torch.float64
    if rows * cols <= 0 or not ptr.value:
        if ptr.value:
            _lib.check(ctx.lib.rlhip_free(ctx.h, ptr), "rlhip_free")
        return torch.empty((cols, rows), dtype=dtype, device=f"cuda:{ctx.device}")
    owner = _Owned(ctx, int(ptr.value), (cols, rows), "<f8" if dtype == torch.float64 else "<f4")
    return torch.as_tensor(owner, device=f"cuda:{ctx.device}")


def _drv_check(ctx, rc, what):
    if rc <= -100:
        raise _lib.RlhipError(f"{what}: {ctx.lib.rlhip_last_error().decode()} (code {rc})")
    return rc


def drv_stab(ctx: Context, kind: int, A, m: int, k: int, cond_check: bool = False):
    cf = C.c_int(0)
    rc = getattr(ctx.lib, f"rlhip_drv_stab_{_suffix(A)[0]}")(ctx.h, kind, int(cond_check), m, k, A.data_ptr(), C.byref(cf))
    return _drv_check(ctx, rc, "stab"), bool(cf.value)


def drv_rs(ctx: Context, A, m, n, k, p, q, stab_kind=0, ctr=(0, 0, 0, 0), key=(0, 0)):
    Om = cm_empty(n, k, device=f"cuda:{ctx.device}")
    st = _state_arr(ctr, key)
    rc = ctx.lib.rlhip_drv_rs_f64(ctx.h, m, n, A.data_ptr(), k, p, q, stab_kind, Om.data_ptr(), st)
    return _drv_check(ctx, rc, "rs"), Om, tuple(int(x) for x in st[:4])


def drv_rf(ctx: Context, A, m, n, k, p, q, rs_stab=0, orth_kind=0, ctr=(0, 0, 0, 0), key=(0, 0)):
    Q = cm_empty(m, k, device=f"cuda:{ctx.device}")
    st = _state_arr(ctr, key)
    rc = ctx.lib.rlhip_drv_rf_f64(ctx.h, m, n, A.data_ptr(), k, p, q, rs_stab, orth_kind, Q.data_ptr(), st)
    return _drv_check(ctx, rc, "rf"), Q, tuple(int(x) for x in st[:4])


def drv_qb(ctx: Context, A, m, n, k, b_sz, tol, p, q, rs_stab=0, rf_orth=0, qb_orth=0, orth_check=False,
           ctr=(0, 0, 0, 0), key=(0, 0)):
    kk = C.c_int64(k)
    Qp, Bp = C.c_void_p(), C.c_void_p()
    st = _state_arr(ctr, key)
    rc = ctx.lib.rlhip_drv_qb_f64(ctx.h, m, n, A.data_ptr(), C.byref(kk), b_sz, tol, p, q, rs_stab, rf_orth, qb_orth,
                                  int(orth_check), C.byref(Qp), C.byref(Bp), st)
    _drv_check(ctx, rc, "qb")
    Q = _adopt(ctx, Qp, m, k)
    BT = _adopt(ctx, Bp, n, k)
    kf = int(kk.value)
    return rc, kf, Q[:kf], BT[:kf], tuple(int(x) for x in st[:4])


def drv_rsvd(ctx: Context, A, m, n, k, b_sz, tol, p, q, rs_stab=0, rf_orth=0, qb_orth=0, orth_check=False,
             ctr=(0, 0, 0, 0), key=(0, 0), keep_on_device=True):
    kk = C.c_int64(k)
    Up, Sp, Vp = C.c_void_p(), C.c_void_p(), C.c_void_p()
    qrc = C.c_int(0)
    st = _state_arr(ctr, key)
    suf, _ = _suffix(A)
    rc = getattr(ctx.lib, f"rlhip_drv_rsvd_{suf}")(ctx.h, m, n, A.data_ptr(), C.byref(kk), b_sz, tol, p, q, rs_stab, rf_orth, qb_orth,
                                                   int(orth_check), C.byref(Up), C.byref(Sp), C.byref(Vp), st, C.byref(qrc))
    _drv_check(ctx, rc, "rsvd")
    kf = int(kk.value)
    kal = max(kf, 1)
    U = _adopt(ctx, Up, m, kal, A.dtype)
    S = _adopt(ctx, Sp, kal, 1, A.dtype).reshape(-1)
    V = _adopt(ctx, Vp, n, kal, A.dtype)
    return dict(rc=rc, qb_rc=int(qrc.value), k=kf, U=U[:kf], S=S[:kf], V=V[:kf], next_ctr=tuple(int(x) for x in st[:4]))


def drv_cqrrt(ctx: Context, A, m, n, d_factor=1.25, nnz=2, eps=None, ctr=(0, 0, 0, 0), key=(0, 0), sketch_in=None, want_sketch=False):
    dev = f"cuda:{ctx.device}"
    if eps is None:
        eps = float(np.finfo(np.float64).eps ** 0.85)
    d = int(d_factor * n)
    R = cm_zeros(n, n, device=dev)
    sk_out = cm_empty(d, n, device=dev) if want_sketch else None
    st = _state_arr(ctr, key)
    rc = ctx.lib.rlhip_drv_cqrrt_f64(ctx.h, m, n, A.data_ptr(), m, R.data_ptr(), n, d_factor, nnz, eps, st,
                                     sketch_in.data_ptr() if sketch_in is not None else None,
                                     sk_out.data_ptr() if sk_out is not None else None)
    _drv_check(ctx, rc, "cqrrt")
    out = dict(rc=rc, R=R, next_ctr=tuple(int(x) for x in st[:4]))
    if want_sketch:
        out["sketch"] = sk_out
    return out


def drv_abrik(ctx: Context, A, m, n, k, tol, max_krylov_iters=0, ctr=(0, 0, 0, 0), key=(0, 0), qr_exp=-1):
    Up, Sp, Vp = C.c_void_p(), C.c_void_p(), C.c_void_p()
    trip, iters = C.c_int64(0), C.c_int64(0)
    nre = C.c_double(0)
    st = _state_arr(ctr, key)
    rc = ctx.lib.rlhip_drv_abrik_f64(ctx.h, m, n, A.data_ptr(), m, k, tol, max_krylov_iters, C.byref(Up), C.byref(Sp), C.byref(Vp), st,
                                     C.byref(trip), C.byref(iters), C.byref(nre), qr_exp)
    _drv_check(ctx, rc, "abrik")
    t = int(trip.value)
    U = _adopt(ctx, Up, m, t)
    S = _adopt(ctx, Sp, t, 1).reshape(-1)
    V = _adopt(ctx, Vp, n, t)
    return dict(rc=rc, U=U, S=S, V=V, triplets=t, iters=int(iters.value), norm_R_end=float(nre.value),
# ... 1071 lines not shown
```

Before: 65200 GFLOP/s.

## Defer CholQR triangular solve on Q into downstream GEMMs in single-block RSVD

In single-block fp64 RSVD, the CholQRQ step skips the m×k triangular solve that forms Q and keeps Y plus R^{-1} instead. The later A^T Q product becomes A^T Y followed by a small k-row blocked solve, and the Q B^T product folds R^{-1} into B first. A condition-number gate (kappa² below 1e6) decides at runtime whether deferral is allowed, and any other use of Q materialises it with the original solve. The aim is to remove a full pass over the tall m×k panel, at the cost of some numerical-stability risk and extra bookkeeping state.

```diff
diff --git a/include/RandLAPACK_amd/rl_blaspp.hh b/include/RandLAPACK_amd/rl_blaspp.hh
--- a/include/RandLAPACK_amd/rl_blaspp.hh
+++ b/include/RandLAPACK_amd/rl_blaspp.hh
@@ -64,6 +64,12 @@
         if (norm_req.pending) { check(rlhip_norma_collect_f64(ctx_, over_ranks ? 1 : 0, &norm_req.value), "norma_collect"); norm_req.pending = false; }
         else if (over_ranks && world() > 1) { double ssq = norm_req.value * norm_req.value; allreduce_sum_host(&ssq, 1); norm_req.value = std::sqrt(ssq); }
         return norm_req.value;
+    }
+    struct SolveRequest { const void* ptr = nullptr; int64_t rows = 0, cols = 0; bool opt_in = false, armed = false, pending = false; };
+    SolveRequest solve_req;
+    bool solve_pending_on(const void* p) const { return solve_req.pending && p == solve_req.ptr; }
+    void materialise_pending() {
+        if (solve_req.pending) { solve_req.pending = false; check(rlhip_deferred_materialise(ctx_), "deferred_materialise"); }
     }
     bool rows_sharded = false;
     bool reduce_over_rows() const { return rows_sharded && world() > 1; }
@@ -120,6 +126,18 @@
     ~RowsSharded() { q_.rows_sharded = prev_; }
 };
 
+class DeferredSolveScope {
+    Queue& q_;
+public:
+    explicit DeferredSolveScope(Queue& q) : q_(q) { q.solve_req = Queue::SolveRequest(); q.solve_req.opt_in = (q.world() == 1); }
+    ~DeferredSolveScope() {
+        if (q_.solve_req.pending) rlhip_deferred_clear(q_.ctx());
+        q_.solve_req = Queue::SolveRequest();
+    }
+    DeferredSolveScope(DeferredSolveScope const&) = delete;
+    DeferredSolveScope& operator=(DeferredSolveScope const&) = delete;
+};
+
 class LocalOnly {
     Queue& q_;
 public:
@@ -174,8 +192,20 @@
 inline void gemm(Layout, Op ta, Op tb, int64_t m, int64_t n, int64_t k, double alpha, double const* A, int64_t lda,
                  double const* B, int64_t ldb, double beta, double* C, int64_t ldc, Queue& q = blas::default_queue()) {
     auto& nr = q.norm_req;
-    if (nr.ptr == (const void*)A && !nr.done && nr.ld == lda &&
-        ((ta == Op::NoTrans && nr.rows == m && nr.cols == k) || (ta != Op::NoTrans && nr.rows == k && nr.cols == m))) {
+    const bool with_norm = nr.ptr == (const void*)A && !nr.done && nr.ld == lda &&
+        ((ta == Op::NoTrans && nr.rows == m && nr.cols == k) || (ta != Op::NoTrans && nr.rows == k && nr.cols == m));
+    if (q.solve_req.pending) {
+        auto& sr = q.solve_req;
+        const bool atq = ta != Op::NoTrans && tb == Op::NoTrans && (const void*)B == sr.ptr && k == sr.rows && n == sr.cols && ldb == sr.rows;
+        const bool qbt = ta == Op::NoTrans && tb != Op::NoTrans && (const void*)A == sr.ptr && m == sr.rows && k == sr.cols && lda == sr.rows;
+        if ((atq || qbt) && !with_norm && (const void*)C != sr.ptr) {
+            const int rc = rlhip_deferred_gemm_f64(q.ctx(), (char)ta, (char)tb, m, n, k, alpha, A, lda, B, ldb, beta, C, ldc);
+            check(rc, "deferred_gemm");
+            if (rc == 0) { if (qbt) sr.pending = false; return; }
+        }
+        if ((const void*)A == sr.ptr || (const void*)B == sr.ptr || (const void*)C == sr.ptr) q.materialise_pending();
+    }
+    if (with_norm) {
         double nrm = 0;
         check(rlhip_gemm_norma_f64(q.ctx(), (char)ta, (char)tb, m, n, k, alpha, A, lda, B, ldb, beta, C, ldc, nr.defer ? nullptr : &nrm,
                                    nullptr), "gemm_norma");
diff --git a/include/RandLAPACK_amd/rl_lapackpp.hh b/include/RandLAPACK_amd/rl_lapackpp.hh
--- a/include/RandLAPACK_amd/rl_lapackpp.hh
+++ b/include/RandLAPACK_amd/rl_lapackpp.hh
@@ -19,6 +19,15 @@
     int rc = rlhip_potrf_f32(q.ctx(), (char)u, n, A, lda); blas::check(rc, "potrf"); return rc;
 }
 inline int cholqrq(int64_t m, int64_t k, double* A, int64_t lda, double* R, bool reduce_gram, int& info, Queue& q = blas::default_queue()) {
+    auto& sr = q.solve_req;
+    if (sr.armed && sr.ptr == (const void*)A && sr.rows == m && sr.cols == k && lda == m && !reduce_gram) {
+        sr.armed = false;
+        int deferred = 0;
+        const int drc = rlhip_cholqrq_defer_f64(q.ctx(), m, k, A, lda, R, &info, &deferred);
+        blas::check(drc, "cholqrq_defer");
+        sr.pending = (drc == 0 && deferred != 0);
+        return drc;
+    }
     const int rc = rlhip_cholqrq_f64(q.ctx(), m, k, A, lda, R, reduce_gram ? 1 : 0, &info);
     blas::check(rc, "cholqrq");
     return rc;
diff --git a/include/RandLAPACK_amd/rl_qb.hh b/include/RandLAPACK_amd/rl_qb.hh
--- a/include/RandLAPACK_amd/rl_qb.hh
+++ b/include/RandLAPACK_amd/rl_qb.hh
@@ -51,6 +51,7 @@
             q.norm_req.ptr = A_cpy; q.norm_req.rows = m; q.norm_req.cols = n; q.norm_req.ld = m;
             q.norm_req.defer = true;
         }
+        const bool may_defer = sizeof(T) == 8 && q.solve_req.opt_in && single_block && !orth_check && q.world() == 1;
         blas::RowsSharded sh(q, true);
         auto done = [&](int code) {
             q.norm_req = blas::Queue::NormRequest();
@@ -68,7 +69,10 @@
             next_sz = curr_sz + b_sz;
             T* Q_i = Q + m * curr_sz;
             T* BT_i = BT + n * curr_sz;
-            if (rf.call(m, n, A_cpy, b_sz, Q_i, state)) { k = curr_sz; q.norm_req = blas::Queue::NormRequest(); return done(6); }
+            if (may_defer) { q.solve_req.ptr = Q_i; q.solve_req.rows = m; q.solve_req.cols = b_sz; q.solve_req.armed = true; }
+            const int rf_rc = rf.call(m, n, A_cpy, b_sz, Q_i, state);
+            q.solve_req.armed = false;
+            if (rf_rc) { k = curr_sz; q.norm_req = blas::Queue::NormRequest(); return done(6); }
             const bool norm_rides = !have_norm && q.norm_req.done;
             if (!have_norm && !norm_rides) norm_A = lapack::lange(Norm::Fro, m, n, A_cpy, m, q);
             if (orth_check && util::orthogonality_check(m, b_sz, Q_i, verbose, q)) { k = curr_sz; return done(4); }
diff --git a/include/RandLAPACK_amd/rl_rsvd.hh b/include/RandLAPACK_amd/rl_rsvd.hh
--- a/include/RandLAPACK_amd/rl_rsvd.hh
+++ b/include/RandLAPACK_amd/rl_rsvd.hh
@@ -29,6 +29,7 @@
 
         T* Q = nullptr;
         T* BT = nullptr;
+        blas::DeferredSolveScope defer_scope(q);
         qb_return = QB_Obj.call(m, n, A, k, block_sz, tol, Q, BT, state);
 
         const int64_t kk = std::max<int64_t>(k, 1);
diff --git a/include/rlhip.h b/include/rlhip.h
--- a/include/rlhip.h
+++ b/include/rlhip.h
@@ -29,7 +29,8 @@
     RLHIP_OPT_LSQ_NORMAL_FUSED = 12,
     RLHIP_OPT_SPMV_LANES = 13,
     RLHIP_OPT_RBF_FUSED = 14,
-    RLHIP_OPT_COUNT = 15
+    RLHIP_OPT_RSVD_DEFER_SOLVE = 15,
+    RLHIP_OPT_COUNT = 16
 };
 int rlhip_set_option(rlhip_ctx* ctx, int option, int64_t value);
 int64_t rlhip_get_option(rlhip_ctx* ctx, int option);
@@ -101,6 +102,11 @@
 int rlhip_potrf_f32(rlhip_ctx* ctx, char uplo, int64_t n, float* A, int64_t lda);
 int rlhip_cholqrq_f64(rlhip_ctx* ctx, int64_t m, int64_t k, double* A, int64_t lda, double* R, int reduce_gram, int* info_host);
 int rlhip_cholqrq_f32(rlhip_ctx* ctx, int64_t m, int64_t k, float* A, int64_t lda, float* R, int reduce_gram, int* info_host);
+int rlhip_cholqrq_defer_f64(rlhip_ctx* ctx, int64_t m, int64_t k, double* A, int64_t lda, double* R, int* info_host, int* deferred_host);
+int rlhip_deferred_gemm_f64(rlhip_ctx* ctx, char transa, char transb, int64_t m, int64_t n, int64_t k, double alpha, const double* A, int64_t lda,
+                            const double* B, int64_t ldb, double beta, double* C, int64_t ldc);
+int rlhip_deferred_materialise(rlhip_ctx* ctx);
+int rlhip_deferred_clear(rlhip_ctx* ctx);
 int rlhip_lange_fro_f64(rlhip_ctx* ctx, int64_t m, int64_t n, const double* A, int64_t lda, double* result_host);
 int rlhip_lange_fro_f32(rlhip_ctx* ctx, int64_t m, int64_t n, const float* A, int64_t lda, float* result_host);
 int rlhip_lacpy_f64(rlhip_ctx* ctx, char uplo, int64_t m, int64_t n, const double* A, int64_t lda, double* B,
diff --git a/randlapack_amd/_lib.py b/randlapack_amd/_lib.py
--- a/randlapack_amd/_lib.py
+++ b/randlapack_amd/_lib.py
@@ -330,6 +330,10 @@
 
 SIGNATURES["rlhip_lu_path_count"] =(c_i64, [c_vp, c_int])
 SIGNATURES["rlhip_tri_path_count"] = (c_i64, [c_vp, c_int])
+SIGNATURES["rlhip_cholqrq_defer_f64"] = (c_int, [c_vp, c_i64, c_i64, c_vp, c_i64, c_vp, C.POINTER(c_int), C.POINTER(c_int)])
+SIGNATURES["rlhip_deferred_gemm_f64"] = (c_int, [c_vp, C.c_char, C.c_char, c_i64, c_i64, c_i64, c_dbl, c_vp, c_i64, c_vp, c_i64, c_dbl, c_vp, c_i64])
+SIGNATURES["rlhip_deferred_materialise"] = (c_int, [c_vp])
+SIGNATURES["rlhip_deferred_clear"] = (c_int, [c_vp])
 
 _lib = None
 
diff --git a/randlapack_amd/csrc/capi.hip b/randlapack_amd/csrc/capi.hip
--- a/randlapack_amd/csrc/capi.hip
+++ b/randlapack_amd/csrc/capi.hip
@@ -205,6 +205,7 @@
     if (c->d_mail) hipFree(c->d_mail);
     if (c->xchg) hipFree(c->xchg);
     if (c->xloc) hipFree(c->xloc);
+    if (c->defer.buf) hipFree(c->defer.buf);
     if (c->h_mail) hipHostFree(c->h_mail);
     if (c->ev0) hipEventDestroy(c->ev0);
     if (c->ev1) hipEventDestroy(c->ev1);
@@ -728,7 +729,28 @@
     return (c && which >= 0 && which < RLHIP_NPATH) ? c->path_count[which] : -1;
 }
 extern "C" int64_t rlhip_lu_path_count(rlhip_ctx* c, int which) { return (c && which >= 60 && which <= 66) ? c->lu_path_count[which - 60] : -1; }
-extern "C" int64_t rlhip_tri_path_count(rlhip_ctx* c, int which) { return (c && which >= 67 && which <= 73) ? c->tri_path_count[which - 67] : -1; }
+extern "C" int64_t rlhip_tri_path_count(rlhip_ctx* c, int which) {
+    if (c && which == 76) return c->tri_path_count[7];
+    return (c && which >= 67 && which <= 73) ? c->tri_path_count[which - 67] : -1;
+}
+extern "C" int rlhip_cholqrq_defer_f64(rlhip_ctx* c, int64_t m, int64_t k, double* A, int64_t lda, double* R, int* info_host, int* deferred_host) {
+    if (!c || !info_host || !deferred_host) return -8;
+    if (m < 0) return -2;
+    if (k < 0) return -3;
+    return rlhip::cholqrq_defer(c, m, k, A, lda, R, info_host, deferred_host);
+}
+extern "C" int rlhip_deferred_gemm_f64(rlhip_ctx* c, char ta, char tb, int64_t m, int64_t n, int64_t k, double alpha, const double* A, int64_t lda,
+                                       const double* B, int64_t ldb, double beta, double* C, int64_t ldc) {
+    if (!c) return -1;
+    const int fa = (ta == 'N' || ta == 'n') ? 0 : 1, fb = (tb == 'N' || tb == 'n') ? 0 : 1;
+    return rlhip::deferred_gemm(c, fa, fb, m, n, k, alpha, A, lda, B, ldb, beta, C, ldc);
+}
+extern "C" int rlhip_deferred_materialise(rlhip_ctx* c) { return c ? rlhip::deferred_materialise(c) : -1; }
+extern "C" int rlhip_deferred_clear(rlhip_ctx* c) {
+    if (!c) return -1;
+    c->defer.pending = 0;
+    return 0;
+}
 extern "C" int rlhip_path_note(rlhip_ctx* c, int which, int64_t delta) {
     if (!c || which < 0 || which >= RLHIP_NPATH) return -1;
     c->path_count[which] += delta;
diff --git a/randlapack_amd/csrc/rlhip_internal.h b/randlapack_amd/csrc/rlhip_internal.h
--- a/randlapack_amd/csrc/rlhip_internal.h
+++ b/randlapack_amd/csrc/rlhip_internal.h
@@ -110,7 +110,7 @@
     unsigned long sync_epoch = 0;
     int avoid_persistent = 0;
     int qrcp_cols_per_wg = 0;
-    int64_t opt[RLHIP_OPT_COUNT] = {-1, -1, -1, -1, -1, -1, -1, -1, -1, -1, -1, -1, -1, -1, -1};
+    int64_t opt[RLHIP_OPT_COUNT] = {-1, -1, -1, -1, -1, -1, -1, -1, -1, -1, -1, -1, -1, -1, -1, -1};
     rlhip_ctx* side_ctx = nullptr;
     hipStream_t side = nullptr;
     void* comm = nullptr;
@@ -127,7 +127,19 @@
     int64_t rbf_split_count = 0;
     int64_t var_path_count[2] = {};
     int64_t lu_path_count[7] = {};
-    int64_t tri_path_count[7] = {};
+    int64_t tri_path_count[8] = {};
+    struct Deferred {
+        const void* Y = nullptr;
+        int64_t m = 0, k = 0, ld = 0;
+        int pending = 0;
+        double* buf = nullptr;
+        size_t buf_elems = 0;
+        double* R() const { return buf; }
+        double* Rinv() const { return buf + k * k; }
+        double* Upk() const { return buf + 2 * k * k; }
+        double* Dinv() const { return buf + 3 * k * k; }
+        double* ssq() const { return buf + 4 * k * k; }
+    } defer;
     int var_fused = 0;
     int64_t grad_path_count[2] = {};
     int grad_fused = 0;
@@ -249,6 +261,10 @@
 
 template <typename T>
 int cholqrq(rlhip_ctx* c, int64_t m, int64_t k, T* A, int64_t lda, T* R, int reduce_gram, int* info_host);
+int cholqrq_defer(rlhip_ctx* c, int64_t m, int64_t k, double* A, int64_t lda, double* R, int* info_host, int* deferred_host);
+int deferred_gemm(rlhip_ctx* c, int transA, int transB, int64_t m, int64_t n, int64_t k, double alpha, const double* A, int64_t lda,
+                  const double* B, int64_t ldb, double beta, double* C, int64_t ldc);
+int deferred_materialise(rlhip_ctx* c);
 
 template <typename T>
 int jacobi_enqueue_rt(rlhip_ctx* c, int n, const T* R, int64_t ldr, int trans_upper, float norm_ratio_lim, const int* skip_dev, int* out_dev,
diff --git a/randlapack_amd/csrc/tri.hip b/randlapack_amd/csrc/tri.hip
--- a/randlapack_amd/csrc/tri.hip
+++ b/randlapack_amd/csrc/tri.hip
@@ -639,6 +639,46 @@
     return xasm ? tf_launch_one<T, 8, OOP, true>(c, a) : tf_launch_one<T, 8, OOP, false>(c, a);
 }
 
+constexpr double DEFER_KAPPA2_LIMIT = 1.0e6;
+__global__ __launch_bounds__(256) void defer_prep_kernel(int64_t k, const double* __restrict__ R, double* __restrict__ Rsave, double* __restrict__ Rinv) {
+    const int64_t e = (int64_t)blockIdx.x * 256 + threadIdx.x;
+    if (e >= k * k) return;
+    Rsave[e] = R[e];
+    Rinv[e] = (e % k == e / k) ? 1.0 : 0.0;
+}
+constexpr int DEFER_SSQ_BLOCKS = 64;
+__global__ __launch_bounds__(256) void defer_ssq_kernel(int64_t k, const double* __restrict__ R, const double* __restrict__ Rinv, double* __restrict__ part) {
+    __shared__ double s_r[4], s_i[4];
+    double nr = 0, ni = 0;
+    for (int64_t e = (int64_t)blockIdx.x * 256 + threadIdx.x; e < k * k; e += (int64_t)DEFER_SSQ_BLOCKS * 256) {
+        const double r = R[e], x = Rinv[e];
+        nr += r * r;
+        ni += x * x;
+    }
+    for (int o = 32; o > 0; o >>= 1) { nr += __shfl_down(nr, o); ni += __shfl_down(ni, o); }
+    if ((threadIdx.x & 63) == 0) { s_r[threadIdx.x >> 6] = nr; s_i[threadIdx.x >> 6] = ni; }
+    __syncthreads();
+    if (threadIdx.x == 0) {
+        part[blockIdx.x] = (s_r[0] + s_r[1]) + (s_r[2] + s_r[3]);
+        part[DEFER_SSQ_BLOCKS + blockIdx.x] = (s_i[0] + s_i[1]) + (s_i[2] + s_i[3]);
+    }
+}
+__global__ __launch_bounds__(64) void defer_gate_kernel(const double* __restrict__ part, int* __restrict__ words, int ngate, double limit2) {
+    static_assert(DEFER_SSQ_BLOCKS == 64, "one share per lane");
+    double a = part[threadIdx.x], b = part[DEFER_SSQ_BLOCKS + threadIdx.x];
+    for (int o = 32; o > 0; o >>= 1) { a += __shfl_down(a, o); b += __shfl_down(b, o); }
+    if (threadIdx.x == 0) {
+        int closed = 0;
+        for (int i = 0; i < ngate; ++i) closed |= words[i];
+        words[ngate] = (!closed && a * b < limit2) ? 1 : 0;
+    }
+}
+inline hipError_t defer_enqueue_blk_solve(rlhip_ctx* c, int64_t rows, const double* Upk, const double* Dinv, double* X, int64_t ldx) {
+    if (rows >= 65536) hipLaunchKernelGGL((trsm_blk_kernel<double, 2>), dim3((unsigned)((rows + 127) / 128)), dim3(256), 0, c->stream, rows, BW, 1.0, Upk, Dinv, X, ldx, 0, 0);
+    else hipLaunchKernelGGL((trsm_blk_kernel<double, 1>), dim3((unsigned)((rows + 63) / 64)), dim3(256), 0, c->stream, rows, BW, 1.0, Upk, Dinv, X, ldx, 0, 0);
+    return hipGetLastError();
+}
+
 }
 
 namespace rlhip {
@@ -885,12 +925,29 @@
 template int trmm_left_upper<float>(rlhip_ctx*, int, int, int64_t, int64_t, float, const float*, int64_t, float*, int64_t);
 
 template <typename T>
-int cholqrq(rlhip_ctx* c, int64_t m, int64_t k, T* A, int64_t lda, T* R, int reduce_gram, int* info_host) {
+static int cholqrq_core(rlhip_ctx* c, int64_t m, int64_t k, T* A, int64_t lda, T* R, int reduce_gram, int* info_host, int* deferred_host) {
+    if (deferred_host) *deferred_host = 0;
     const int64_t nblk = (k + BW - 1) / BW;
     if (c->opt[RLHIP_OPT_CHOLQRQ_ONE_STREAM] == 0 || k < BW || k % BW != 0 || k > 448 || nblk > TF_MAX_BLOCKS - 1 || lda < (m > 1 ? m : 1)) return 1;
     bool local_ok = m >= TF_MIN_ROWS && tf_offsets_fit(lda, m);
     if (!reduce_gram && !local_ok) return 1;
     *info_host = 0;
+    bool defer = false;
+    if constexpr (sizeof(T) == 8) {
+        defer = deferred_host && !reduce_gram && local_ok && k == BW && c->opt[RLHIP_OPT_RSVD_DEFER_SOLVE] != 0;
+        if (defer) {
+            auto& d = c->defer;
+            d.pending = 0;
+            const size_t need = (size_t)4 * k * k + 2 * DEFER_SSQ_BLOCKS;
+            if (d.buf_elems < need) {
+                if (d.buf) { RLHIP_CHECK(rlhip_stream_sync(c)); RLHIP_CHECK(hipFree(d.buf)); d.buf = nullptr; d.buf_elems = 0; }
+                if (hipMalloc((void**)&d.buf, need * sizeof(double)) != hipSuccess) { (void)hipGetLastError(); d.buf = nullptr; defer = false; }
+                else d.buf_elems = need;
+            }
+            if (defer) d.k = k;
+        }
+    }
+    const int ngate = 1 + (int)nblk;
     hipError_t e1 = hipSuccess;
     {
         ws_scope ws(c);
@@ -898,8 +955,13 @@
         if (!words) return reduce_gram ? RLHIP_ERR_HIP(hipErrorOutOfMemory) : 1;
         T *Upk_all = nullptr, *Dinv_all = nullptr, *Uneg = nullptr, *fdump = nullptr;
         if (local_ok) {
-            Upk_all = ws.alloc<T>((size_t)nblk * BW * BW);
-            Dinv_all = ws.alloc<T>((size_t)nblk * (BW / 32) * 1024);
+            if constexpr (sizeof(T) == 8) {
+                if (defer) { Upk_all = c->defer.Upk(); Dinv_all = c->defer.Dinv(); }
+            }
+            if (!Upk_all) {
+                Upk_all = ws.alloc<T>((size_t)nblk * BW * BW);
+                Dinv_all = ws.alloc<T>((size_t)nblk * (BW / 32) * 1024);
+            }
             Uneg = ws.alloc<T>((size_t)k * k);
             fdump = ws.alloc<T>(512 + 64);
             if (!Upk_all || !Dinv_all || !Uneg || !fdump) {
@@ -934,8 +996,19 @@
         if (local_ok) {
             RLHIP_CHECK(tf_enqueue_blk_pack<T>(c, k, nblk, (int)NonUnit, R, k, Upk_all, Dinv_all, words + 1));
             RLHIP_CHECK(tf_enqueue_neg_pack<T>(c, k, k, R, k, Uneg));
+            if constexpr (sizeof(T) == 8) {
+                if (defer) {
+                    auto& d = c->defer;
+                    hipLaunchKernelGGL(defer_prep_kernel, dim3((unsigned)((k * k + 255) / 256)), dim3(256), 0, c->stream, k, R, d.R(), d.Rinv());
+                    RLHIP_LAUNCH_CHECK();
+                    RLHIP_CHECK(defer_enqueue_blk_solve(c, k, d.Upk(), d.Dinv(), d.Rinv(), k));
+                    hipLaunchKernelGGL(defer_ssq_kernel, dim3(DEFER_SSQ_BLOCKS), dim3(256), 0, c->stream, k, d.R(), d.Rinv(), d.ssq());
+                    hipLaunchKernelGGL(defer_gate_kernel, dim3(1), dim3(64), 0, c->stream, d.ssq(), words, ngate, DEFER_KAPPA2_LIMIT);
+                    RLHIP_LAUNCH_CHECK();
+                }
+            }
             TfArgs<T> a{m, k, k, T(1), Uneg, Dinv_all, A, lda, 0, (int)nblk, 0, fdump};
-            a.gate = words; a.ngate = 1 + (int)nblk;
+            a.gate = words; a.ngate = ngate + (defer ? 1 : 0);
             rc = tf_launch<T, 0>(c, a);
             if (rc) return rc;
         }
@@ -946,6 +1019,14 @@
     const int* w = (const int*)(c->h_mail + MAIL_CHOLQRQ);
     *info_host = w[0];
     if (w[0] != 0) return 0;
+    if (defer && w[ngate] != 0) {
+        auto& d = c->defer;
+        d.Y = A; d.m = m; d.ld = lda; d.pending = 1;
+        *deferred_host = 1;
+        c->path_count[11]++;
+        c->tri_path_count[7]++;
+        return 0;
+    }
     bool guard = !local_ok;
     for (int64_t b = 0; b < nblk; ++b) guard = guard || (w[1 + b] != 0);
     if (guard) return trsm_right_upper<T>(c, NonUnit, m, k, T(1), R, k, A, lda);
@@ -953,8 +1034,77 @@
     c->path_count[11]++;
     return 0;
 }
+template <typename T>
+int cholqrq(rlhip_ctx* c, int64_t m, int64_t k, T* A, int64_t lda, T* R, int reduce_gram, int* info_host) {
+    return cholqrq_core<T>(c, m, k, A, lda, R, reduce_gram, info_host, nullptr);
+}
 template int cholqrq<double>(rlhip_ctx*, int64_t, int64_t, double*, int64_t, double*, int, int*);
 template int cholqrq<float>(rlhip_ctx*, int64_t, int64_t, float*, int64_t, float*, int, int*);
+
+int cholqrq_defer(rlhip_ctx* c, int64_t m, int64_t k, double* A, int64_t lda, double* R, int* info_host, int* deferred_host) {
+    return cholqrq_core<double>(c, m, k, A, lda, R, 0, info_host, deferred_host);
+}
+
+int deferred_gemm(rlhip_ctx* c, int transA, int transB, int64_t m, int64_t n, int64_t k, double alpha, const double* A, int64_t lda,
+                  const double* B, int64_t ldb, double beta, double* C, int64_t ldc) {
+    auto& d = c->defer;
+    if (!d.pending) return 1;
+    const int64_t kk = d.k;
+    if (transA && !transB && (const void*)B == d.Y && k == d.m && n == kk && ldb == d.ld) {
+        if (beta != 0.0) return 1;
+        if (m <= 0) return 0;
+        if (ldc < m) return -13;
+        int rc = gemm_impl<double>(c, 1, 0, m, n, k, alpha, A, lda, B, ldb, 0.0, C, ldc, 0);
+        if (rc) return rc;
+        RLHIP_CHECK(defer_enqueue_blk_solve(c, m, d.Upk(), d.Dinv(), C, ldc));
+        return 0;
+    }
+    if (!transA && transB && (const void*)A == d.Y && m == d.m && k == kk && lda == d.ld) {
+        if (n <= 0) { d.pending = 0; return 0; }
+        ws_scope ws(c);
+        double* M = ws.alloc<double>((size_t)kk * n);
+        if (!M) return RLHIP_ERR_HIP(hipErrorOutOfMemory);
+        int rc = gemm_impl<double>(c, 0, 1, n, kk, kk, 1.0, B, ldb, d.Rinv(), kk, 0.0, M, n, 0);
+        if (!rc) rc = gemm_impl<double>(c, 0, 1, m, n, kk, alpha, A, lda, M, n, beta, C, ldc, 0);
+        if (!rc) d.pending = 0;
+        return rc;
+    }
+    return 1;
+}
+
+int deferred_materialise(rlhip_ctx* c) {
+    auto& d = c->defer;
+    if (!d.pending) return 0;
+    d.pending = 0;
+    const int64_t m = d.m, k = d.k, lda = d.ld, nblk = k / BW;
+    double* A = (double*)const_cast<void*>(d.Y);
+    hipError_t e1 = hipSuccess;
+    {
+        ws_scope ws(c);
+        int* words = ws.alloc<int>(TF_VERDICT_ALLOC);
+        double* Upk_all = ws.alloc<double>((size_t)nblk * BW * BW);
+        double* Dinv_all = ws.alloc<double>((size_t)nblk * (BW / 32) * 1024);
+        double* Uneg = ws.alloc<double>((size_t)k * k);
+        double* fdump = ws.alloc<double>(512 + 64);
+        if (!words || !Upk_all || !Dinv_all || !Uneg || !fdump) return RLHIP_ERR_HIP(hipErrorOutOfMemory);
+        RLHIP_CHECK(hipMemsetAsync(words, 0, TF_VERDICT_ALLOC * sizeof(int), c->stream));
+        RLHIP_CHECK(tf_enqueue_blk_pack<double>(c, k, nblk, (int)NonUnit, d.R(), k, Upk_all, Dinv_all, words + 1));
+        RLHIP_CHECK(tf_enqueue_neg_pack<double>(c, k, k, d.R(), k, Uneg));
+        TfArgs<double> a{m, k, k, 1.0, Uneg, Dinv_all, A, lda, 0, (int)nblk, 0, fdump};
+        a.gate = words; a.ngate = 1 + (int)nblk;
+        const int rc = tf_launch<double, 0>(c, a);
+        if (rc) return rc;
+        e1 = hipMemcpyAsync(c->h_mail + MAIL_CHOLQRQ, words, TF_VERDICT_ALLOC * sizeof(int), hipMemcpyDeviceToHost, c->stream);
+        if (e1 == hipSuccess) e1 = rlhip_stream_sync(c);
+    }
+    if (e1 != hipSuccess) return RLHIP_ERR_HIP(e1);
+    const int* w = (const int*)(c->h_mail + MAIL_CHOLQRQ);
+    bool guard = false;
+    for (int64_t b = 0; b < nblk; ++b) guard = guard || (w[1 + b] != 0);
+    if (guard) return trsm_right_upper<double>(c, NonUnit, m, k, 1.0, d.R(), k, A, lda);
+    c->path_count[2]++;
+    return 0;
+}
 
 template int trsm_right_upper<double>(rlhip_ctx*, int, int64_t, int64_t, double, const double*, int64_t, double*, int64_t);
 template int trsm_right_upper_oop<double>(rlhip_ctx*, int, int64_t, int64_t, double, const double*, int64_t, const double*, int64_t, const int64_t*, double*, int64_t);
diff --git a/randlapack_amd/device.py b/randlapack_amd/device.py
--- a/randlapack_amd/device.py
+++ b/randlapack_amd/device.py
@@ -229,12 +229,16 @@
     OPT = dict(cholqrq_one_stream=0, gesdd_gram=1, jacobi_persist=2, trsm_xasm=3, saso_mode=4, hqrrp_tall_panel=5,
                bqrrp_lookahead_min_elems=6, bqrrp_cholqr_fallback=7, cqrrpt_fold_pivoting=8, cqrrpt_split_qrcp=9, sparse_sketch_densify=10, jacobi_clock_holders=11,
                lsq_normal_fused=12, spmv_lanes=13, rbf_fused=14)
+    OPT_LATER = dict(rsvd_defer_solve=15)
+
+    def _opt_index(self, name: str) -> int:
+        return self.OPT[name] if name in self.OPT else self.OPT_LATER[name]
 
     def set_option(self, name: str, value: int) -> None:
-        _lib.check(self.lib.rlhip_set_option(self.h, self.OPT[name], int(value)), "set_option")
+        _lib.check(self.lib.rlhip_set_option(self.h, self._opt_index(name), int(value)), "set_option")
 
     def get_option(self, name: str) -> int:
-        return int(self.lib.rlhip_get_option(self.h, self.OPT[name]))
+        return int(self.lib.rlhip_get_option(self.h, self._opt_index(name)))
 
     def options(self, **kw):
         import contextlib
```

Result: no change. 65370 GFLOP/s (median of 6 runs) (+0.3%).
